# raulmur/ORB_SLAM

Hardware: AMD Instinct MI355X
Metric: frames/s ORB extract+match @640x480, 1000 kp (higher is better)
Workload: dtype u8; 1 GPU; vga: 640x480 grayscale stream, 8 levels, nFeatures 1000, S-blocks frames, extract + Hamming top-2 match vs previous frame (BASELINE.json configs[1] + the frame-to-frame match of the metric); resident_frames_per_gpu=2048, lanes=4, parity_checked_frames=0, parity_mismatches=0, library_build_id=6b2c39ae018c2573, lane_placement=2

## Files before the change

include/orbx.h:

```cpp
#ifndef ORBX_H
#define ORBX_H

#include <stddef.h>
#include <stdint.h>

#ifdef __cplusplus
extern "C" {
#endif

#define ORBX_OK             0
#define ORBX_EMPTY          1
#define ORBX_ERR_ARG       -1
#define ORBX_ERR_DEVICE    -2
#define ORBX_ERR_CAPACITY  -3
#define ORBX_ERR_GEOMETRY  -4

#define ORBX_HARRIS_SCORE 0
#define ORBX_FAST_SCORE   1

#define ORBX_BLUR_X86_SSE2 0
#define ORBX_BLUR_HALF_UP  1

#define ORBX_FP_ISO          0
#define ORBX_FP_GCC_CONTRACT 1

typedef struct orbx_keypoint {
    float x, y;
    float size;
    float angle;
    float response;
    int32_t octave;
    int32_t class_id;
} orbx_keypoint;

typedef struct orbx_params {
    int32_t nfeatures;
    float   scale_factor;
    int32_t nlevels;
    int32_t score_type;
    int32_t fast_th;
    int32_t device;
    int32_t max_batch;
    int32_t blur_rounding;
    int32_t fp_contract;
    int32_t reserved[7];
} orbx_params;

typedef struct orbx_extractor orbx_extractor;

void  orbx_default_params(orbx_params* p);
int   orbx_create(const orbx_params* p, orbx_extractor** out);
void  orbx_destroy(orbx_extractor* h);
int   orbx_get_levels(const orbx_extractor* h);
float orbx_get_scale_factor(const orbx_extractor* h);
int   orbx_max_keypoints(const orbx_extractor* h);
const char* orbx_last_error(const orbx_extractor* h);
const char* orbx_build_id(void);

int orbx_extract(orbx_extractor* h, const uint8_t* img, int w, int hgt, ptrdiff_t stride,
                 orbx_keypoint* kps, uint8_t* desc, int cap, int* n_out);

int orbx_extract_batch_device(orbx_extractor* h, const uint8_t* d_imgs, int nframes, int w, int hgt,
                              ptrdiff_t row_stride, ptrdiff_t frame_stride,
                              orbx_keypoint* d_kps, uint8_t* d_desc, int32_t* d_n, int cap,
                              int32_t* d_status, void* stream);

#define ORBX_PHASE_PYRAMID  1
#define ORBX_PHASE_DETECT   2
#define ORBX_PHASE_DESCRIBE 4
#define ORBX_PHASE_ALL      7
int orbx_extract_batch_device_phases(orbx_extractor* h, const uint8_t* d_imgs, int nframes, int w, int hgt,
                                     ptrdiff_t row_stride, ptrdiff_t frame_stride,
                                     orbx_keypoint* d_kps, uint8_t* d_desc, int32_t* d_n, int cap,
                                     int32_t* d_status, void* stream, int phases);

#define ORBX_FRAMES_ON_DEVICE 0
#define ORBX_FRAMES_ON_HOST   1
int orbx_extract_batch(orbx_extractor* h, const uint8_t* const* imgs, const ptrdiff_t* row_strides, int nframes, int w, int hgt,
                       int where, orbx_keypoint* d_kps, uint8_t* d_desc, int32_t* d_n, int cap,
                       int32_t* d_status, void* stream);

#define ORBX_PIX_GRAY8  0
#define ORBX_PIX_RGB8   1
#define ORBX_PIX_BGR8   2
#define ORBX_PIX_RGBA8  3
#define ORBX_PIX_BGRA8  4

int orbx_to_gray_device(const uint8_t* d_src, int nframes, int w, int hgt, ptrdiff_t src_row_stride, ptrdiff_t src_frame_stride, int fmt,
                        uint8_t* d_gray, ptrdiff_t gray_row_stride, ptrdiff_t gray_frame_stride, void* stream);

int orbx_extract_color(orbx_extractor* h, const uint8_t* img, int w, int hgt, ptrdiff_t stride, int fmt,
                       orbx_keypoint* kps, uint8_t* desc, int cap, int* n_out, uint8_t* gray_out);

int orbx_extract_batch_device_color(orbx_extractor* h, const uint8_t* d_imgs, int nframes, int w, int hgt,
                                    ptrdiff_t row_stride, ptrdiff_t frame_stride, int fmt,
                                    orbx_keypoint* d_kps, uint8_t* d_desc, int32_t* d_n, int cap, int32_t* d_status,
                                    uint8_t* d_gray, ptrdiff_t gray_row_stride, ptrdiff_t gray_frame_stride, void* stream);

int orbx_extract_batch_color(orbx_extractor* h, const uint8_t* const* imgs, const ptrdiff_t* row_strides, int nframes, int w, int hgt,
                             int where, int fmt, orbx_keypoint* d_kps, uint8_t* d_desc, int32_t* d_n, int cap,
                             int32_t* d_status, void* stream);

int orbm_hamming256(const uint8_t* a, const uint8_t* b);

int orbm_match_top2(const uint8_t* Q, int nq, const uint8_t* T, int nt,
                    int32_t* best_idx, int32_t* best, int32_t* second, int device);
int orbm_match_top2_device(const uint8_t* dQ, int nq, const uint8_t* dT, int nt,
                           int32_t* d_best_idx, int32_t* d_best, int32_t* d_second, void* stream);
int orbm_match_top2_masked(const uint8_t* Q, int nq, const uint8_t* T, int nt, const uint8_t* t_valid,
                           int32_t* best_idx, int32_t* best, int32_t* second, int device);
int orbm_match_top2_masked_device(const uint8_t* dQ, int nq, const uint8_t* dT, int nt, const uint8_t* d_t_valid,
                                  int32_t* d_best_idx, int32_t* d_best, int32_t* d_second, void* stream);
int orbm_match_top2_batch_device(const uint8_t* dQ, const int32_t* d_nq, const uint8_t* dT, const int32_t* d_nt,
                                 int nbatch, int cap, int32_t* d_best_idx, int32_t* d_best, int32_t* d_second,
                                 void* stream);
int orbm_match_top2_segments(const uint8_t* Q, int nq, const uint8_t* T, int nt, const int32_t* seg_off, const int32_t* cand,
                             int32_t* best_idx, int32_t* best, int32_t* second, int device);
int orbm_match_top2_segments_device(const uint8_t* dQ, int nq, const uint8_t* dT, int nt, const int32_t* d_seg_off,
                                    const int32_t* d_cand, int32_t* d_best_idx, int32_t* d_best, int32_t* d_second, void* stream);
int orbm_count_accepted(const int32_t* best, const int32_t* second, int nq, int th, float ratio);
int orbm_debug_set_match_path(int path);
int orbm_debug_get_match_path(void);

int orbx_device_alloc(int device, size_t bytes, void** d_ptr);
int orbx_device_free(int device, void* d_ptr);
int orbx_device_upload(int device, void* d_dst, const void* src, size_t bytes);
int orbx_device_download(int device, void* dst, const void* d_src, size_t bytes);

int orbx_stream_create(int device, void** stream);
int orbx_stream_create_priority(int device, int priority, void** stream);
int orbx_stream_destroy(int device, void* stream);
int orbx_stream_synchronize(int device, void* stream);
int orbx_event_create(int device, void** event);
int orbx_event_destroy(int device, void* event);
int orbx_event_record(void* event, void* stream);
int orbx_stream_wait_event(void* stream, void* event);
int orbx_device_copy_async(void* d_dst, const void* d_src, size_t bytes, void* stream);
int orbx_host_alloc(int device, size_t bytes, void** h_ptr);
int orbx_host_free(int device, void* h_ptr);
int orbx_device_upload_async(void* d_dst, const void* h_src, size_t bytes, void* stream);
int orbx_device_download_async(void* h_dst, const void* d_src, size_t bytes, void* stream);

int orbm_distinctive(const uint8_t* desc, const int32_t* seg_off, int npoints, int32_t* best_idx, int32_t* best_median, int device);
int orbm_distinctive_device(const uint8_t* d_desc, const int32_t* d_seg_off, int npoints, int32_t* d_best_idx,
                            int32_t* d_best_median, void* stream);

#define ORBX_DBG_PLANE      0
#define ORBX_DBG_BLUR       1
#define ORBX_DBG_NMS        2
#define ORBX_DBG_LEVEL_KPS  3
#define ORBX_DBG_BANDS      4
int orbx_debug_set_stop_after(orbx_extractor* h, int stage);
int orbx_debug_set_blur_on_demand(orbx_extractor* h, int mode);
int orbx_debug_stage_timing(orbx_extractor* h, int enable);
int orbx_debug_stage_time(orbx_extractor* h, int stage, double* total_ms, long* launches);
int orbx_debug_level_size(const orbx_extractor* h, int level, int* w, int* hgt);
int orbx_debug_resize_form(const orbx_extractor* h, int level, int* form, int* rows_out);
#define ORBX_VS_COLOR        0
#define ORBX_VS_INGEST       1
#define ORBX_VS_PYRAMID      2
#define ORBX_VS_FAST         3
#define ORBX_VS_QUOTA        4
#define ORBX_VS_CELL_SELECT  5
#define ORBX_VS_LEVEL_SELECT 6
#define ORBX_VS_BLUR         7
#define ORBX_VS_DESCRIBE     8
#define ORBX_VS_COUNT        9
#define ORBX_VF_LDS_OVER_64K  1u
#define ORBX_VF_FUSE_BLUR     2u
#define ORBX_VF_OVERLAP       4u
#define ORBX_VF_ON_DEMAND     8u
#define ORBX_VF_XCD_AFFINITY 16u
typedef struct orbx_stage_variant {
    int32_t id;
    uint32_t flags;
    uint64_t mask;
} orbx_stage_variant;
int orbx_debug_launch_variant(const orbx_extractor* h, int stage, orbx_stage_variant* out, char* name, int name_cap);
int orbx_debug_variant_count(int stage);
const char* orbx_debug_variant_name(int stage, int id);
typedef struct orbx_plan_args {
    int32_t w, h, nframes;
    int32_t gather, xcd_affinity, on_demand, od_min_frames, stop_after;
    int64_t row_stride, frame_stride;
    uint32_t base_bits;
    int32_t color_fmt, color_gather;
    uint32_t color_bits;
    int32_t one_frame, side_stream;
    int64_t one_frame_bytes;
} orbx_plan_args;
int orbx_debug_plan(const orbx_params* p, const orbx_plan_args* a, orbx_stage_variant* out);
long orbx_debug_fetch(orbx_extractor* h, int what, int frame, int level, void* host_out, long cap_bytes);
int orbx_debug_geometry(const orbx_params* p, int w, int hgt, int32_t* out, int cap_levels);
int orbx_debug_nth_element(const float* resp, int n, int nth, int32_t* out_perm, int device);
int orbx_debug_eval_math(int kind, const float* in0, const float* in1, float* out0, float* out1, int n, int device);
int orbx_debug_eval_compass(const uint32_t* c, const uint32_t* e, const uint32_t* w, const uint32_t* nn, const uint32_t* ss, uint32_t* out, int n, int t, int device);
int orbx_debug_eval_blur_window(const uint8_t* windows, uint8_t* out, int n, int rounding, int general, int device);

#ifdef __cplusplus
}
#endif
#endif
```

orb_slam_amd/capi.py:

```python
import ctypes
import os
import numpy as np

_HERE = os.path.dirname(os.path.abspath(__file__))
LIB_PATH = os.environ.get("ORBX_LIB") or os.path.join(_HERE, "liborbx.so")

ORBX_OK, ORBX_EMPTY = 0, 1
ORBX_ERR_ARG, ORBX_ERR_DEVICE, ORBX_ERR_CAPACITY, ORBX_ERR_GEOMETRY = -1, -2, -3, -4
HARRIS_SCORE, FAST_SCORE = 0, 1
BLUR_X86_SSE2, BLUR_HALF_UP = 0, 1
DBG_PLANE, DBG_BLUR, DBG_NMS, DBG_LEVEL_KPS, DBG_BANDS = 0, 1, 2, 3, 4
(ST_PYRAMID, ST_FAST_CELLS, ST_QUOTA, ST_CELL_SELECT, ST_LEVEL_SELECT, ST_BLUR, ST_DESCRIBE) = range(7)

KP_DTYPE = np.dtype([("x", "<f4"), ("y", "<f4"), ("size", "<f4"), ("angle", "<f4"),
                     ("response", "<f4"), ("octave", "<i4"), ("class_id", "<i4")])

EXPORTS = [
    "orbx_default_params", "orbx_create", "orbx_destroy", "orbx_get_levels", "orbx_get_scale_factor",
    "orbx_max_keypoints", "orbx_last_error", "orbx_build_id", "orbx_extract", "orbx_extract_batch_device", "orbx_extract_batch_device_phases", "orbx_extract_batch",
    "orbx_to_gray_device", "orbx_extract_color", "orbx_extract_batch_device_color", "orbx_extract_batch_color",
    "orbm_hamming256", "orbm_match_top2", "orbm_match_top2_device", "orbm_match_top2_batch_device", "orbm_match_top2_masked", "orbm_match_top2_masked_device",
    "orbm_count_accepted", "orbm_match_top2_segments", "orbm_match_top2_segments_device", "orbm_distinctive", "orbm_distinctive_device",
    "orbx_device_alloc", "orbx_device_free", "orbx_device_upload", "orbx_device_download",
    "orbx_stream_create", "orbx_stream_create_priority", "orbx_stream_destroy", "orbx_stream_synchronize", "orbx_event_create", "orbx_event_destroy", "orbx_event_record",
    "orbx_stream_wait_event", "orbx_device_copy_async", "orbx_host_alloc", "orbx_host_free", "orbx_device_upload_async", "orbx_device_download_async", "orbx_debug_set_stop_after", "orbx_debug_set_blur_on_demand", "orbx_debug_level_size", "orbx_debug_resize_form", "orbx_debug_fetch",
    "orbx_debug_launch_variant", "orbx_debug_variant_count", "orbx_debug_variant_name", "orbx_debug_plan",
    "orbx_debug_eval_math", "orbx_debug_eval_compass", "orbx_debug_eval_blur_window", "orbx_debug_stage_timing", "orbx_debug_stage_time", "orbx_debug_nth_element", "orbx_debug_geometry",
    "orbm_debug_set_match_path",
    "orbm_debug_get_match_path",
]
EXPORTS_F = [
    "orbf_image_bounds", "orbf_undistort_grid", "orbf_undistort_grid_batch_device", "orbf_features_in_area",
    "orbf_features_in_area_device",
]
EXPORTS_S = ["orbs_lds_bytes", "orbs_debug_set_buckets", "orbs_debug_set_wide_max", "orbs_three_maxima", "orbs_window_search_batch_device", "orbs_list_search_batch_device",
             "orbs_bow_ranges_batch_device", "orbs_triangulation_search_batch_device", "orbs_epipolar_bound", "orbs_agreement_batch_device",
             "orbs_bow_rows_search_batch_device", "orbs_bow_rows_search", "orbs_tri_rows_search_batch_device", "orbs_tri_rows_search"]
PHASE_PYRAMID, PHASE_DETECT, PHASE_DESCRIBE, PHASE_ALL = 1, 2, 4, 7
RULE_MAPPOINTS, RULE_WINDOW, RULE_BEST, RULE_INIT, RULE_BOW, RULE_FREE, RULE_TRIANGULATION = 0, 1, 2, 3, 4, 5, 6
TH_HIGH, TH_LOW = 100, 50
EXPORTS_V = [
    "orbv_create", "orbv_load_text", "orbv_destroy", "orbv_info", "orbv_descend", "orbv_descend_device",
    "orbv_transform", "orbv_transform_batch_device", "orbv_score",
]
EXPORTS_D = ["orbd_create", "orbd_destroy", "orbd_size", "orbd_add", "orbd_add_batch_device", "orbd_erase", "orbd_clear",
             "orbd_query_batch_device", "orbd_query"]
EXPORTS_P = ["orbp_create", "orbp_destroy", "orbp_capacity", "orbp_size", "orbp_clear", "orbp_put", "orbp_put_device", "orbp_erase", "orbp_get",
             "orbp_project_batch_device", "orbp_track_batch_device", "orbp_track", "orbp_project_source_batch_device",
             "orbp_track_source_batch_device", "orbp_track_source", "orbp_refresh_batch_device", "orbp_refresh", "orbp_fuse_batch_device",
             "orbp_fuse", "orbp_view_from_sim3", "orbp_loop_project_batch_device", "orbp_loop_search_batch_device", "orbp_loop_search",
             "orbp_sim3_from_pair", "orbp_sim3_search_batch_device", "orbp_sim3_search", "orbp_local_votes_batch_device", "orbp_local_votes",
             "orbp_local_points_batch_device", "orbp_local_points", "orbp_rows_purge_device", "orbp_cull_batch_device", "orbp_cull"]
LOCAL_MAX_PROBLEMS, LOCAL_MAX_ROWS = 64, 65535
CULL_MAX_CANDIDATES = 4096
EXPORTS_T = ["orbt_triangulate_batch_device", "orbt_triangulate", "orbt_new_points_rows_device", "orbt_new_points_rows"]
(T_NONE, T_ACCEPTED, T_PARALLAX, T_W_ZERO, T_DEPTH1, T_DEPTH2, T_REPROJ1, T_REPROJ2, T_ZERO_DIST, T_SCALE, T_SKIP_INDEX, T_SKIP_OCTAVE) = range(12)
EXPORTS_I = ["orbi_normalize", "orbi_pose_from_rt", "orbi_models_batch_device", "orbi_models", "orbi_check_rt_batch_device", "orbi_check_rt"]
INIT_MAX_PROBLEMS, INIT_MAX_MATCHES, INIT_MAX_ITERS, INIT_MAX_HYP = 32, 16384, 1024, 8
(RT_NONE, RT_GOOD, RT_COUNTED, RT_NONFINITE, RT_DEPTH1, RT_DEPTH2, RT_REPROJ1, RT_REPROJ2, RT_SKIP_INDEX) = range(9)
EXPORTS_E = ["orbe_ransac_parameters", "orbe_hypotheses_batch_device", "orbe_hypotheses", "orbe_refine_batch_device", "orbe_refine",
             "orbe_refit_batch_device", "orbe_refit", "orbe_select_batch_device", "orbe_select", "orbe_iterate", "orbe_iterate_batch"]
EXPORTS_H = ["orbh_ransac_parameters", "orbh_max_errors", "orbh_hypotheses_batch_device", "orbh_hypotheses", "orbh_select_batch_device", "orbh_select",
             "orbh_iterate", "orbh_iterate_batch"]
MODE_FRAME, MODE_LAST_FRAME, MODE_KEYFRAME, MODE_FUSE, MODE_LOOP, MODE_SIM3 = 0, 1, 2, 3, 4, 5
(FUSE_FUSED, FUSE_SKIPPED, FUSE_DEPTH, FUSE_IMAGE, FUSE_DISTANCE, FUSE_ANGLE, FUSE_EMPTY, FUSE_FAR) = range(8)
LOOP_QUERY = 8
REFRESH_NORMAL_DEPTH, REFRESH_DESCRIPTOR = 1, 2
(REFRESH_OK, REFRESH_SKIPPED, REFRESH_EMPTY, REFRESH_BAD_INDEX, REFRESH_BAD_OCTAVE, REFRESH_NONFINITE) = range(6)


class OrbxError(RuntimeError):
    def __init__(self, code, msg=""):
        super().__init__("orbx error %d %s" % (code, msg))
        self.code = code


class Params(ctypes.Structure):
    _fields_ = [("nfeatures", ctypes.c_int32), ("scale_factor", ctypes.c_float), ("nlevels", ctypes.c_int32),
                ("score_type", ctypes.c_int32), ("fast_th", ctypes.c_int32), ("device", ctypes.c_int32),
                ("max_batch", ctypes.c_int32), ("blur_rounding", ctypes.c_int32), ("fp_contract", ctypes.c_int32), ("reserved", ctypes.c_int32 * 7)]


class StageVariant(ctypes.Structure):
    _fields_ = [("id", ctypes.c_int32), ("flags", ctypes.c_uint32), ("mask", ctypes.c_uint64)]


class PlanArgs(ctypes.Structure):
    _fields_ = [("w", ctypes.c_int32), ("h", ctypes.c_int32), ("nframes", ctypes.c_int32), ("gather", ctypes.c_int32),
                ("xcd_affinity", ctypes.c_int32), ("on_demand", ctypes.c_int32), ("od_min_frames", ctypes.c_int32), ("stop_after", ctypes.c_int32),
                ("row_stride", ctypes.c_int64), ("frame_stride", ctypes.c_int64), ("base_bits", ctypes.c_uint32), ("color_fmt", ctypes.c_int32),
                ("color_gather", ctypes.c_int32), ("color_bits", ctypes.c_uint32), ("one_frame", ctypes.c_int32), ("side_stream", ctypes.c_int32),
                ("one_frame_bytes", ctypes.c_int64)]


VS_COLOR, VS_INGEST, VS_PYRAMID, VS_FAST, VS_QUOTA, VS_CELL_SELECT, VS_LEVEL_SELECT, VS_BLUR, VS_DESCRIBE, VS_COUNT = range(10)
VS_NAMES = ["color", "ingest", "pyramid", "fast", "quota", "cell_select", "level_select", "blur", "describe"]
VF_LDS_OVER_64K, VF_FUSE_BLUR, VF_OVERLAP, VF_ON_DEMAND, VF_XCD_AFFINITY = 1, 2, 4, 8, 16
XCD_AFFINITY_MIN_FRAMES = 64
OD_MIN_FRAMES_DEFAULT = 32


class Camera(ctypes.Structure):
    _fields_ = [("K", ctypes.c_float * 9), ("dist", ctypes.c_float * 8), ("ndist", ctypes.c_int32),
                ("width", ctypes.c_int32), ("height", ctypes.c_int32)]

    @classmethod
    def make(cls, fx, fy, cx, cy, dist, width, height):
        c = cls()
        for i, v in enumerate((fx, 0, cx, 0, fy, cy, 0, 0, 1)):
            c.K[i] = v
        for i, v in enumerate(dist):
            c.dist[i] = v
        c.ndist, c.width, c.height = len(dist), width, height
        return c


class Bounds(ctypes.Structure):
    _fields_ = [("min_x", ctypes.c_int32), ("max_x", ctypes.c_int32), ("min_y", ctypes.c_int32), ("max_y", ctypes.c_int32),
                ("inv_w", ctypes.c_float), ("inv_h", ctypes.c_float)]

    def astuple(self):
        return (self.min_x, self.max_x, self.min_y, self.max_y, self.inv_w, self.inv_h)


class SearchParams(ctypes.Structure):
    _fields_ = [("rule", ctypes.c_int32), ("th", ctypes.c_int32), ("ratio", ctypes.c_float), ("check_orientation", ctypes.c_int32)]


class View(ctypes.Structure):
    _fields_ = [("Rcw", ctypes.c_float * 9), ("tcw", ctypes.c_float * 3), ("Ow", ctypes.c_float * 3),
                ("fx", ctypes.c_float), ("fy", ctypes.c_float), ("cx", ctypes.c_float), ("cy", ctypes.c_float),
                ("min_x", ctypes.c_int32), ("max_x", ctypes.c_int32), ("min_y", ctypes.c_int32), ("max_y", ctypes.c_int32),
                ("view_cos_limit", ctypes.c_float), ("th", ctypes.c_float), ("mode", ctypes.c_int32), ("reserved", ctypes.c_int32)]

    @classmethod
    def make(cls, Rcw, tcw, Ow, fx, fy, cx, cy, min_x, max_x, min_y, max_y, view_cos_limit=0.5, th=1.0):
        v = cls()
        v.Rcw[:] = [float(x) for x in np.asarray(Rcw, np.float32).reshape(9)]
        v.tcw[:] = [float(x) for x in np.asarray(tcw, np.float32).reshape(3)]
        v.Ow[:] = [float(x) for x in np.asarray(Ow, np.float32).reshape(3)]
        v.fx, v.fy, v.cx, v.cy = float(fx), float(fy), float(cx), float(cy)
        v.min_x, v.max_x, v.min_y, v.max_y = int(min_x), int(max_x), int(min_y), int(max_y)
        v.view_cos_limit, v.th, v.mode, v.reserved = float(view_cos_limit), float(th), 0, 0
        return v


def view_from_sim3(Scw, view):
    S = np.ascontiguousarray(np.asarray(Scw, dtype=np.float32).reshape(-1)[:12])
    assert S.size == 12
    if isinstance(view, np.ndarray):
        assert view.dtype == VIEW_DTYPE and view.size == 1 and view.flags.c_contiguous
        ptr = view.ctypes.data
    else:
        ptr = ctypes.addressof(view)
    rc = lib().orbp_view_from_sim3(S.ctypes.data, ptr)
    if rc != ORBX_OK:
        raise OrbxError(rc, "orbp_view_from_sim3")
    return view


def sim3_from_pair(s12, R12, t12, R1w, t1w, R2w, t2w, fx, fy, cx, cy, bounds, th):
    a = lambda x, n: np.ascontiguousarray(np.asarray(x, dtype=np.float32).reshape(n))
    R12, t12, R1w, t1w, R2w, t2w = a(R12, 9), a(t12, 3), a(R1w, 9), a(t1w, 3), a(R2w, 9), a(t2w, 3)
    dirs = np.zeros(2, SIM3_DIR_DTYPE)
    rc = lib().orbp_sim3_from_pair(float(s12), R12.ctypes.data, t12.ctypes.data, R1w.ctypes.data, t1w.ctypes.data, R2w.ctypes.data, t2w.ctypes.data,
                                   float(fx), float(fy), float(cx), float(cy), ctypes.addressof(bounds), float(th), dirs.ctypes.data)
    if rc != ORBX_OK:
        raise OrbxError(rc, "orbp_sim3_from_pair")
    return dirs


class TriCamera(ctypes.Structure):
    _fields_ = [("Rcw", ctypes.c_float * 9), ("tcw", ctypes.c_float * 3), ("Ow", ctypes.c_float * 3),
                ("fx", ctypes.c_float), ("fy", ctypes.c_float), ("cx", ctypes.c_float), ("cy", ctypes.c_float)]


class TriPair(ctypes.Structure):
    _fields_ = [("kf1", TriCamera), ("kf2", TriCamera), ("scale_factor", ctypes.c_float), ("reserved", ctypes.c_int32)]


TRI_CAMERA_DTYPE = np.dtype([("Rcw", np.float32, 9), ("tcw", np.float32, 3), ("Ow", np.float32, 3), ("fx", np.float32), ("fy", np.float32),
                             ("cx", np.float32), ("cy", np.float32)])
TRI_PAIR_DTYPE = np.dtype([("kf1", TRI_CAMERA_DTYPE), ("kf2", TRI_CAMERA_DTYPE), ("scale_factor", np.float32), ("reserved", np.int32)])
assert TRI_PAIR_DTYPE.itemsize == ctypes.sizeof(TriPair) == 160

INIT_PROBLEM_DTYPE = np.dtype([("norm1", np.float32, 4), ("norm2", np.float32, 4), ("sigma", np.float32), ("n1", np.int32), ("n2", np.int32),
                               ("nmatches", np.int32), ("iters", np.int32), ("reserved", np.int32)])
INIT_POSE_DTYPE = np.dtype([("R", np.float32, 9), ("t", np.float32, 3), ("P2", np.float32, 12), ("O2", np.float32, 3)])
assert INIT_PROBLEM_DTYPE.itemsize == 56 and INIT_POSE_DTYPE.itemsize == 108
PNP_PROBLEM_DTYPE = np.dtype([("fu", np.float32), ("fv", np.float32), ("uc", np.float32), ("vc", np.float32), ("n", np.int32), ("iters", np.int32),
                              ("min_inliers", np.int32), ("max_its", np.int32)])
PNP_STATE_DTYPE = np.dtype([("iterations", np.int32), ("best_inliers", np.int32), ("refine_ok", np.int32), ("refined_inliers", np.int32),
                            ("best_tcw", np.float32, 12), ("refined_tcw", np.float32, 12)])
PNP_RESULT_DTYPE = np.dtype([("kind", np.int32), ("stop", np.int32), ("no_more", np.int32), ("ninliers", np.int32), ("tcw", np.float32, 12)])
assert PNP_PROBLEM_DTYPE.itemsize == 32 and PNP_STATE_DTYPE.itemsize == 112 and PNP_RESULT_DTYPE.itemsize == 64
PNP_KIND_NONE, PNP_KIND_BEST, PNP_KIND_REFINED = 0, 1, 2
PNP_MAX_PROBLEMS, PNP_MAX_POINTS, PNP_MAX_ITERS = 32, 8192, 1024
SIM3SOLVER_PROBLEM_DTYPE = np.dtype([("fx1", np.float32), ("fy1", np.float32), ("cx1", np.float32), ("cy1", np.float32), ("fx2", np.float32),
                                     ("fy2", np.float32), ("cx2", np.float32), ("cy2", np.float32), ("n", np.int32), ("iters", np.int32),
                                     ("min_inliers", np.int32), ("max_its", np.int32)])
SIM3SOLVER_HYP_DTYPE = np.dtype([("q", np.float64, 4), ("R", np.float32, 9), ("t", np.float32, 3), ("s", np.float32), ("T12", np.float32, 16),
                                 ("T21", np.float32, 16), ("count", np.int32)])
SIM3SOLVER_STATE_DTYPE = np.dtype([("iterations", np.int32), ("best_inliers", np.int32), ("best_T12", np.float32, 16), ("best_R", np.float32, 9),
                                   ("best_t", np.float32, 3), ("best_s", np.float32)])
SIM3SOLVER_RESULT_DTYPE = np.dtype([("found", np.int32), ("stop", np.int32), ("no_more", np.int32), ("ninliers", np.int32), ("T12", np.float32, 16)])
assert SIM3SOLVER_PROBLEM_DTYPE.itemsize == 48 and SIM3SOLVER_HYP_DTYPE.itemsize == 216 and SIM3SOLVER_STATE_DTYPE.itemsize == 124 and \
    SIM3SOLVER_RESULT_DTYPE.itemsize == 80
SIM3SOLVER_MAX_PROBLEMS, SIM3SOLVER_MAX_POINTS, SIM3SOLVER_MAX_ITERS, SIM3SOLVER_POINT_ROWS = 32, 8192, 1024, 12

VIEW_DTYPE = np.dtype([("Rcw", np.float32, 9), ("tcw", np.float32, 3), ("Ow", np.float32, 3), ("fx", np.float32), ("fy", np.float32),
                       ("cx", np.float32), ("cy", np.float32), ("min_x", np.int32), ("max_x", np.int32), ("min_y", np.int32),
                       ("max_y", np.int32), ("view_cos_limit", np.float32), ("th", np.float32), ("mode", np.int32), ("reserved", np.int32)])
RECORD_DTYPE = np.dtype([("in_view", np.uint8), ("pad", np.uint8, 3), ("u", np.float32), ("v", np.float32), ("view_cos", np.float32),
                         ("level", np.int32)])
assert VIEW_DTYPE.itemsize == ctypes.sizeof(View) == 108 and RECORD_DTYPE.itemsize == 20
REFRESHED_DTYPE = np.dtype([("normal", np.float32, 3), ("min_dist", np.float32), ("max_dist", np.float32), ("best_obs", np.int32),
                            ("best_median", np.int32), ("status", np.int32)])
assert REFRESHED_DTYPE.itemsize == 32
FUSED_DTYPE = np.dtype([("u", np.float32), ("v", np.float32), ("level", np.int32), ("status", np.int32)])
assert FUSED_DTYPE.itemsize == 16
SIM3_DIR_DTYPE = np.dtype([("Raw", np.float32, 9), ("taw", np.float32, 3), ("S", np.float32, 9), ("t", np.float32, 3), ("fx", np.float32),
                           ("fy", np.float32), ("cx", np.float32), ("cy", np.float32), ("min_x", np.int32), ("max_x", np.int32), ("min_y", np.int32),
                           ("max_y", np.int32), ("th", np.float32), ("mode", np.int32), ("reserved", np.int32, 2)])
assert SIM3_DIR_DTYPE.itemsize == 144

GRID_COLS, GRID_ROWS = 64, 48
GRID_CELLS = GRID_COLS * GRID_ROWS

_LIB = None


def lib():
    global _LIB
    if _LIB is None:
        if not os.path.exists(LIB_PATH):
            raise OrbxError(ORBX_ERR_DEVICE, "liborbx.so not built: run `make` / __graft_entry__.build()")
        try:
            import torch
        except ImportError:
            pass
        L = ctypes.CDLL(LIB_PATH)
        vp, ci, cl, cf = ctypes.c_void_p, ctypes.c_int, ctypes.c_long, ctypes.c_float
        pd = ctypes.c_ssize_t
        L.orbx_default_params.argtypes = [ctypes.POINTER(Params)]
        L.orbx_default_params.restype = None
        L.orbx_create.argtypes = [ctypes.POINTER(Params), ctypes.POINTER(vp)]
        L.orbx_destroy.argtypes = [vp]
        L.orbx_destroy.restype = None
        L.orbx_get_levels.argtypes = [vp]
        L.orbx_get_scale_factor.argtypes = [vp]
        L.orbx_get_scale_factor.restype = cf
        L.orbx_max_keypoints.argtypes = [vp]
        L.orbx_last_error.argtypes = [vp]
        L.orbx_last_error.restype = ctypes.c_char_p
        L.orbx_build_id.argtypes = []
        L.orbx_build_id.restype = ctypes.c_char_p
        L.orbx_extract.argtypes = [vp, vp, ci, ci, pd, vp, vp, ci, ctypes.POINTER(ci)]
        L.orbx_extract_batch_device.argtypes = [vp, vp, ci, ci, ci, pd, pd, vp, vp, vp, ci, vp, vp]
        L.orbx_extract_batch_device_phases.argtypes = [vp, vp, ci, ci, ci, pd, pd, vp, vp, vp, ci, vp, vp, ci]
        L.orbx_extract_batch.argtypes = [vp, vp, vp, ci, ci, ci, ci, vp, vp, vp, ci, vp, vp]
        L.orbx_to_gray_device.argtypes = [vp, ci, ci, ci, pd, pd, ci, vp, pd, pd, vp]
        L.orbx_extract_color.argtypes = [vp, vp, ci, ci, pd, ci, vp, vp, ci, ctypes.POINTER(ci), vp]
        L.orbx_extract_batch_device_color.argtypes = [vp, vp, ci, ci, ci, pd, pd, ci, vp, vp, vp, ci, vp, vp, pd, pd, vp]
        L.orbx_extract_batch_color.argtypes = [vp, vp, vp, ci, ci, ci, ci, ci, vp, vp, vp, ci, vp, vp]
        L.orbm_hamming256.argtypes = [vp, vp]
        L.orbm_match_top2.argtypes = [vp, ci, vp, ci, vp, vp, vp, ci]
        L.orbm_match_top2_device.argtypes = [vp, ci, vp, ci, vp, vp, vp, vp]
        L.orbm_match_top2_batch_device.argtypes = [vp, vp, vp, vp, ci, ci, vp, vp, vp, vp]
        L.orbm_match_top2_masked.argtypes = [vp, ci, vp, ci, vp, vp, vp, vp, ci]
        L.orbm_match_top2_masked_device.argtypes = [vp, ci, vp, ci, vp, vp, vp, vp, vp]
        L.orbm_count_accepted.argtypes = [vp, vp, ci, ci, cf]
        L.orbm_debug_set_match_path.argtypes = [ci]
        L.orbm_debug_get_match_path.argtypes = []
        L.orbs_debug_set_buckets.argtypes = [ci]
        L.orbs_debug_set_wide_max.argtypes = [ci]
        L.orbm_match_top2_segments.argtypes = [vp, ci, vp, ci, vp, vp, vp, vp, vp, ci]
        L.orbm_match_top2_segments_device.argtypes = [vp, ci, vp, ci, vp, vp, vp, vp, vp, vp]
        L.orbx_device_alloc.argtypes = [ci, ctypes.c_size_t, ctypes.POINTER(vp)]
        L.orbx_device_free.argtypes = [ci, vp]
        L.orbx_device_upload.argtypes = [ci, vp, vp, ctypes.c_size_t]
        L.orbx_device_download.argtypes = [ci, vp, vp, ctypes.c_size_t]
        L.orbm_distinctive.argtypes = [vp, vp, ci, vp, vp, ci]
        L.orbm_distinctive_device.argtypes = [vp, vp, ci, vp, vp, vp]
        L.orbx_debug_set_stop_after.argtypes = [vp, ci]
        L.orbx_debug_set_blur_on_demand.argtypes = [vp, ci]
        L.orbx_debug_level_size.argtypes = [vp, ci, ctypes.POINTER(ci), ctypes.POINTER(ci)]
        if hasattr(L, "orbx_debug_resize_form"):
            L.orbx_debug_resize_form.argtypes = [vp, ci, ctypes.POINTER(ci), ctypes.POINTER(ci)]
        if hasattr(L, "orbx_debug_launch_variant"):
            L.orbx_debug_launch_variant.argtypes = [vp, ci, ctypes.POINTER(StageVariant), ctypes.c_char_p, ci]
            L.orbx_debug_variant_count.argtypes = [ci]
            L.orbx_debug_variant_name.argtypes = [ci, ci]
            L.orbx_debug_variant_name.restype = ctypes.c_char_p
            L.orbx_debug_plan.argtypes = [ctypes.POINTER(Params), ctypes.POINTER(PlanArgs), ctypes.POINTER(StageVariant)]
        L.orbx_debug_fetch.argtypes = [vp, ci, ci, ci, vp, cl]
        L.orbx_debug_fetch.restype = cl
        L.orbx_debug_eval_math.argtypes = [ci, vp, vp, vp, vp, ci, ci]
        L.orbx_debug_eval_compass.argtypes = [vp, vp, vp, vp, vp, vp, ci, ci, ci]
        L.orbx_debug_eval_blur_window.argtypes = [vp, vp, ci, ci, ci, ci]
        L.orbx_debug_nth_element.argtypes = [vp, ci, ci, vp, ci]
        L.orbx_debug_geometry.argtypes = [ctypes.POINTER(Params), ci, ci, vp, ci]
        L.orbx_debug_stage_timing.argtypes = [vp, ci]
        L.orbx_debug_stage_time.argtypes = [vp, ci, ctypes.POINTER(ctypes.c_double), ctypes.POINTER(cl)]
        L.orbf_image_bounds.argtypes = [ctypes.POINTER(Camera), ctypes.POINTER(Bounds)]
        L.orbf_undistort_grid.argtypes = [ctypes.POINTER(Camera), ctypes.POINTER(Bounds), vp, ci, vp, vp, vp, ci]
        L.orbf_undistort_grid_batch_device.argtypes = [ctypes.POINTER(Camera), ctypes.POINTER(Bounds), vp, vp, ci, ci, vp, vp, vp, vp]
        L.orbf_features_in_area.argtypes = [ctypes.POINTER(Bounds), vp, ci, vp, vp, vp, vp, ci, vp, vp, ci, ci]
        L.orbf_features_in_area_device.argtypes = [ctypes.POINTER(Bounds), vp, ci, vp, vp, vp, vp, ci, vp, vp, ci, vp, vp]
        L.orbs_lds_bytes.argtypes = [ci, ci]
        L.orbs_lds_bytes.restype = ctypes.c_size_t
        L.orbs_three_maxima.argtypes = [vp, ci, vp]
        L.orbs_three_maxima.restype = None
        L.orbs_window_search_batch_device.argtypes = [ctypes.POINTER(Bounds), ctypes.POINTER(SearchParams), vp, vp, vp, vp, vp, ci, vp,
                                                      vp, vp, vp, vp, vp, vp, ci, ci, vp, vp, vp, vp, vp, vp]
        L.orbs_list_search_batch_device.argtypes = [ctypes.POINTER(SearchParams), vp, vp, vp, vp, vp, ci, vp, vp, vp, vp, vp, vp, vp, ci, ci,
                                                    vp, vp, vp, vp, vp, vp]
        L.orbs_bow_ranges_batch_device.argtypes = [vp, vp, vp, vp, vp, vp, ci, ci, vp, vp, vp]
        L.orbs_triangulation_search_batch_device.argtypes = [ctypes.POINTER(SearchParams), vp, vp, ci, vp, vp, vp, vp, vp, ci, vp, vp, vp,
                                                             vp, vp, vp, vp, ci, ci, vp, vp, vp, vp, vp, vp]
        L.orbs_epipolar_bound.argtypes = [ctypes.c_float]
        L.orbs_epipolar_bound.restype = ctypes.c_float
        L.orbs_agreement_batch_device.argtypes = [vp, vp, ci, vp, vp, ci, ci, vp, vp, vp]
        L.orbs_bow_rows_search_batch_device.argtypes = [ctypes.POINTER(SearchParams), vp, ci, vp, vp, vp, vp, vp, vp, vp, ci, ci, vp, vp, vp, vp, vp, vp, vp, vp]
        L.orbs_bow_rows_search.argtypes = [ctypes.POINTER(SearchParams), vp, ci, vp, vp, vp, vp, vp, vp, vp, ci, ci, ci, vp, vp, vp, vp, vp, vp, vp, vp]
        L.orbs_tri_rows_search_batch_device.argtypes = [ctypes.POINTER(SearchParams), vp, ci, vp, vp, ci, vp, vp, vp, vp, vp, vp, vp, ci, ci, vp, ci, vp, vp, vp, vp, vp,
                                                        vp, vp]
        L.orbs_tri_rows_search.argtypes = [ctypes.POINTER(SearchParams), vp, ci, vp, vp, ci, vp, vp, vp, vp, vp, vp, vp, ci, ci, ci, vp, ci, vp, vp, vp, vp, vp, vp, vp]
        L.orbv_create.argtypes = [ci, ci, ci, ci, ci, vp, vp, vp, vp, ci, ctypes.POINTER(vp)]
        L.orbv_load_text.argtypes = [ctypes.c_char_p, ci, ctypes.POINTER(vp)]
        L.orbv_destroy.argtypes = [vp]
        L.orbv_destroy.restype = None
        L.orbv_info.argtypes = [vp] + [ctypes.POINTER(ci)] * 6
        L.orbv_descend.argtypes = [vp, vp, ci, ci, vp, vp, vp]
        L.orbv_descend_device.argtypes = [vp, vp, ci, ci, vp, vp, vp, vp]
        L.orbv_transform.argtypes = [vp, vp, ci, ci, vp, vp, ctypes.POINTER(ci), vp, vp, vp, ctypes.POINTER(ci)]
        L.orbv_transform_batch_device.argtypes = [vp, vp, vp, ci, ci, ci, vp, vp, vp, vp, vp, vp, vp, vp]
        L.orbv_score.argtypes = [vp, vp, vp, ci, vp, vp, ci]
        L.orbv_score.restype = ctypes.c_double
        L.orbd_create.argtypes = [vp, ci, ci, ctypes.POINTER(vp)]
        L.orbd_destroy.argtypes = [vp]
        L.orbd_destroy.restype = None
        L.orbd_size.argtypes = [vp]
        L.orbd_add.argtypes = [vp, ci, vp, vp, ci]
        L.orbd_add_batch_device.argtypes = [vp, vp, ci, vp, vp, vp, ci, vp, vp]
        L.orbd_erase.argtypes = [vp, ci]
        L.orbd_clear.argtypes = [vp]
        L.orbd_query_batch_device.argtypes = [vp, ci, vp, vp, vp, ci, vp, vp, vp, vp, vp, vp, ci, vp, vp, vp, vp]
        L.orbd_query.argtypes = [vp, vp, vp, ci, vp, ci, vp, vp, vp, vp, ci, ctypes.POINTER(ci), ctypes.POINTER(ci), vp]
        L.orbp_create.argtypes = [ci, ci, ctypes.POINTER(vp)]
        L.orbp_destroy.argtypes = [vp]
        L.orbp_destroy.restype = None
        L.orbp_capacity.argtypes = [vp]
        L.orbp_size.argtypes = [vp]
        L.orbp_clear.argtypes = [vp]
        L.orbp_put.argtypes = [vp, vp, ci, vp, vp, vp, vp, vp]
        L.orbp_put_device.argtypes = [vp, vp, ci, vp, vp, vp, vp, vp, vp]
        L.orbp_erase.argtypes = [vp, vp, ci]
        L.orbp_get.argtypes = [vp, ci, ctypes.POINTER(ci), vp, vp, vp, vp, vp]
        L.orbp_project_batch_device.argtypes = [vp, vp, ci, vp, ci, vp, vp, ci, vp, vp, vp, vp, vp, vp, vp, vp, ci, vp]
        L.orbp_track_batch_device.argtypes = [vp, vp, ci, vp, ci, vp, vp, ci, vp, ctypes.POINTER(Bounds), cf, vp, vp, vp, vp, vp, ci, vp, ci,
                                              vp, vp, vp, vp, vp, vp]
        L.orbp_track.argtypes = [vp, ctypes.POINTER(View), vp, ci, vp, ci, vp, ctypes.POINTER(Bounds), cf, vp, vp, vp, vp, vp, ci, ci, ci,
                                 vp, vp, ctypes.POINTER(ci), ctypes.POINTER(ci), vp]
        L.orbp_refresh_batch_device.argtypes = [vp, vp, ci, vp, vp, vp, vp, vp, vp, vp, vp, vp, ci, ci, vp, ci, ci, vp, vp]
        L.orbp_refresh.argtypes = [vp, vp, ci, vp, vp, vp, vp, vp, vp, vp, vp, vp, ci, ci, ci, vp, ci, ci, vp, vp]
        L.orbp_fuse_batch_device.argtypes = [vp, vp, ci, vp, ci, vp, vp, ci, vp, vp, ci, vp, vp, vp, vp, vp, ci, ci, vp, vp, vp, vp, vp]
        L.orbp_fuse.argtypes = [vp, vp, ci, vp, ci, vp, vp, ci, vp, vp, ci, vp, vp, vp, vp, vp, ci, ci, ci, vp, vp, vp, vp, vp]
        L.orbp_view_from_sim3.argtypes = [vp, vp]
        cf = ctypes.c_float
        L.orbp_sim3_from_pair.argtypes = [cf, vp, vp, vp, vp, vp, vp, cf, cf, cf, cf, vp, cf, vp]
        L.orbp_sim3_search_batch_device.argtypes = [vp, vp, ci, vp, ci, vp, vp, ci, vp, vp, vp, vp, vp, vp, vp, ci, ci, vp, ci, vp, vp, vp, vp, vp, vp]
        L.orbp_sim3_search.argtypes = [vp, vp, ci, vp, ci, vp, vp, ci, vp, vp, vp, vp, vp, vp, vp, ci, ci, ci, vp, ci, vp, vp, vp, vp, vp, vp]
        L.orbp_loop_project_batch_device.argtypes = [vp, vp, ci, vp, ci, vp, vp, ci, vp, vp, vp, vp, vp, vp, vp, vp, ci, vp]
        L.orbp_loop_search_batch_device.argtypes = [vp, vp, ci, vp, ci, vp, vp, ci, vp, vp, ci, vp, vp, vp, vp, vp, ci, ci, vp, vp, ci, vp, vp, vp, vp, vp, vp, vp]
        L.orbp_loop_search.argtypes = [vp, vp, vp, ci, vp, ci, vp, vp, ci, vp, vp, vp, vp, vp, ci, ci, ci, vp, vp, vp, ctypes.POINTER(ci), ctypes.POINTER(ci), vp]
        L.orbp_local_votes_batch_device.argtypes = [vp, vp, vp, ci, ci, vp, vp, ci, ci, vp, vp]
        L.orbp_local_votes.argtypes = [vp, vp, vp, ci, ci, vp, vp, ci, ci, ci, vp, vp]
        L.orbp_local_points_batch_device.argtypes = [vp, vp, vp, ci, ci, vp, vp, ci, vp, vp, ci, ci, vp, vp, vp, vp, ci, vp]
        L.orbp_local_points.argtypes = [vp, vp, vp, ci, ci, vp, vp, ci, vp, vp, ci, ci, ci, vp, vp, vp, vp, ci, vp]
        L.orbp_rows_purge_device.argtypes = [vp, vp, ci, vp, ci, ci, vp]
        L.orbp_cull_batch_device.argtypes = [vp, vp, ci, vp, vp, vp, ci, ci, ci, vp, vp, vp, vp]
        L.orbp_cull.argtypes = [vp, vp, ci, vp, vp, vp, ci, ci, ci, ci, vp, vp, vp, vp]
        L.orbp_project_source_batch_device.argtypes = [vp, vp, ci, vp, ci, vp, vp, ci, vp, vp, vp, vp, vp, vp, vp, vp, vp, vp, ci, vp]
        L.orbp_track_source_batch_device.argtypes = [vp, vp, ci, vp, ci, vp, vp, ci, vp, vp, vp, ctypes.POINTER(Bounds), ctypes.POINTER(SearchParams),
                                                     vp, vp, vp, vp, vp, ci, vp, ci, vp, vp, vp, vp, vp, vp]
        L.orbp_track_source.argtypes = [vp, ctypes.POINTER(View), vp, ci, vp, ci, vp, vp, vp, ci, ctypes.POINTER(Bounds), ctypes.POINTER(SearchParams),
                                        vp, vp, vp, vp, vp, ci, ci, ci, vp, vp, ctypes.POINTER(ci), ctypes.POINTER(ci), vp]
        L.orbt_triangulate_batch_device.argtypes = [vp, ci, vp, vp, vp, vp, ci, vp, vp, ci, ci, vp, vp, ci, vp, vp, vp, ci, vp, vp, vp, vp, vp, vp, vp, vp,
                                                    ci, vp, vp, vp]
        L.orbt_triangulate.argtypes = [vp, vp, vp, vp, vp, ci, vp, ci, vp, ci, vp, vp, vp, vp, vp, vp, ci, ctypes.POINTER(ci), ci]
        L.orbt_new_points_rows_device.argtypes = [ctypes.POINTER(SearchParams), vp, ci, vp, vp, vp, vp, vp, vp, ci, vp, vp, vp, vp, vp, vp, vp, ci, ci, vp, vp, vp, vp,
                                                  vp, vp, vp, vp, vp, vp, vp, vp, vp, ci, vp]
        L.orbt_new_points_rows.argtypes = [ctypes.POINTER(SearchParams), vp, ci, vp, vp, vp, vp, vp, vp, ci, vp, vp, vp, vp, vp, vp, vp, ci, ci, ci, vp, vp, vp, vp,
                                           vp, vp, vp, vp, vp, vp, vp, vp, vp, ci, vp]
        pnp_bind(L)
        sim3solver_bind(L)
        L.orbi_normalize.argtypes = [vp, ci, vp]
        L.orbi_pose_from_rt.argtypes = [cf, cf, cf, cf, vp, vp, vp]
        L.orbi_models_batch_device.argtypes = [vp, ci, vp, ci, vp, ci, vp, ci, vp, ci, vp, vp, vp, vp, vp, vp, vp, vp, vp, vp, vp, vp]
        L.orbi_models.argtypes = [vp, vp, vp, vp, vp, vp, vp, vp, vp, vp, vp, vp, vp, vp, vp, vp, ci]
        L.orbi_check_rt_batch_device.argtypes = [cf, cf, cf, cf, vp, ci, ci, vp, vp, vp, vp, ci, vp, ci, vp, ci, vp, cf, vp, vp, vp, vp, vp, vp, vp]
        L.orbi_check_rt.argtypes = [cf, cf, cf, cf, vp, ci, vp, ci, vp, ci, vp, ci, vp, cf, vp, vp, vp, vp, vp, vp, vp, ci]
        _LIB = L
    return _LIB


FRAMES_ON_DEVICE, FRAMES_ON_HOST = 0, 1


def frame_table(frames):
    frames = list(frames)
    if not frames:
        raise ValueError("no frames")
    on_dev = [bool(getattr(f, "is_cuda", False)) for f in frames]
    if any(on_dev) and not all(on_dev):
        raise ValueError("frames mix device and host memory")
    ptrs, strides, keep, shape = [], [], [], None
    for f in frames:
        if hasattr(f, "data_ptr"):
            import torch
            if f.dtype != torch.uint8 or f.dim() != 2:
                raise ValueError("frames must be 2-D uint8")
            if f.stride(1) != 1 or f.stride(0) < f.shape[1]:
                if f.is_cuda:
                    raise ValueError("device frame rows must be contiguous (stride(1) == 1)")
                f = f.contiguous()
            hw, p, rs = tuple(f.shape), f.data_ptr(), f.stride(0)
        else:
            a = np.asarray(f)
            if a.dtype != np.uint8 or a.ndim != 2:
                raise ValueError("frames must be 2-D uint8")
            if a.strides[1] != 1 or a.strides[0] < a.shape[1]:
                a = np.ascontiguousarray(a)
            hw, p, rs = a.shape, a.ctypes.data, a.strides[0]
            f = a
        if shape is None:
            shape = hw
        elif hw != shape:
            raise ValueError("frames differ in size: %s vs %s" % (hw, shape))
        keep.append(f)
        ptrs.append(p)
# ... 59 lines not shown
        raise OrbxError(rc, "orbx_to_gray_device")


def to_gray(frames, fmt, stream=0):
    import torch
    one = frames.dim() == 3
    x = frames.unsqueeze(0) if one else frames
    ch = pix_channels(fmt)
    if not x.is_cuda or x.dtype != torch.uint8 or x.dim() != 4 or x.shape[3] != ch or x.stride(3) != 1 or x.stride(2) != ch:
        raise ValueError("to_gray wants a CUDA uint8 (F, H, W, %d) tensor with packed pixels" % ch)
    F, h, w = x.shape[:3]
    out = torch.empty((F, h, w), dtype=torch.uint8, device=x.device)
    to_gray_device(x.data_ptr(), F, w, h, x.stride(1), x.stride(0), fmt, out.data_ptr(), w, w * h, stream)
    return out[0] if one else out


class ORBextractor:

    def __init__(self, nfeatures=1000, scaleFactor=1.2, nlevels=8, scoreType=FAST_SCORE, fastTh=20,
                 device=0, max_batch=1, blur_rounding=BLUR_X86_SSE2, fp_contract=None):
        L = lib()
        p = Params()
        L.orbx_default_params(ctypes.byref(p))
        p.nfeatures, p.scale_factor, p.nlevels, p.score_type, p.fast_th = nfeatures, scaleFactor, nlevels, scoreType, fastTh
        p.device, p.max_batch, p.blur_rounding = device, max_batch, blur_rounding
        if fp_contract is not None:
            p.fp_contract = 1 if fp_contract else 0
        h = ctypes.c_void_p()
        rc = L.orbx_create(ctypes.byref(p), ctypes.byref(h))
        if rc != ORBX_OK:
            raise OrbxError(rc, "orbx_create (is a gfx950 GPU visible?)")
        self.h = h
        self.L = L
        self.max_keypoints = L.orbx_max_keypoints(h)

    def close(self):
        if getattr(self, "h", None):
            self.L.orbx_destroy(self.h)
            self.h = None

    def __del__(self):
        self.close()

    def GetLevels(self):
        return self.L.orbx_get_levels(self.h)

    def GetScaleFactor(self):
        return self.L.orbx_get_scale_factor(self.h)

    def _err(self, rc):
        return OrbxError(rc, self.L.orbx_last_error(self.h).decode())

    def __call__(self, image):
        img = np.asarray(image)
        if img.size == 0:
            return None
        assert img.dtype == np.uint8 and img.ndim == 2
        if img.strides[1] != 1:
            img = np.ascontiguousarray(img)
        hh, w = img.shape
        cap = self.max_keypoints
        kps = np.zeros(cap, dtype=KP_DTYPE)
        desc = np.zeros((cap, 32), dtype=np.uint8)
        n = ctypes.c_int(0)
        rc = self.L.orbx_extract(self.h, img.ctypes.data, w, hh, img.strides[0], kps.ctypes.data, desc.ctypes.data, cap, ctypes.byref(n))
        if rc != ORBX_OK:
            raise self._err(rc)
        return kps[:n.value].copy(), desc[:n.value].copy()

    def extract_batch_device(self, d_imgs, nframes, w, h, row_stride, frame_stride, d_kps, d_desc, d_n, cap, d_status=0, stream=0, phases=PHASE_ALL):
        rc = self.L.orbx_extract_batch_device_phases(self.h, d_imgs, nframes, w, h, row_stride, frame_stride, d_kps, d_desc, d_n, cap,
                                                     d_status or None, stream or None, phases)
        if rc != ORBX_OK:
            raise self._err(rc)

    def extract_batch(self, frames, d_kps, d_desc, d_n, cap, d_status=0, stream=0):
        where, ptrs, strides, w, h, keep = frame_table(frames)
        rc = self.L.orbx_extract_batch(self.h, ptrs.ctypes.data, strides.ctypes.data, len(ptrs), w, h, where, d_kps, d_desc, d_n, cap,
                                       d_status or None, stream or None)
        del keep
        if rc != ORBX_OK:
            raise self._err(rc)

    def extract_color(self, image, fmt, want_gray=False):
        ptr, w, hh, rs, on_dev, keep = color_layout(image, fmt)
        if on_dev:
            raise ValueError("extract_color takes a host frame")
        if w == 0 or hh == 0:
            return None
        cap = self.max_keypoints
        kps = np.zeros(cap, dtype=KP_DTYPE)
        desc = np.zeros((cap, 32), dtype=np.uint8)
        gray = np.empty((hh, w), dtype=np.uint8) if want_gray else None
        n = ctypes.c_int(0)
        rc = self.L.orbx_extract_color(self.h, ptr, w, hh, rs, fmt, kps.ctypes.data, desc.ctypes.data, cap, ctypes.byref(n),
                                       gray.ctypes.data if want_gray else None)
        del keep
        if rc != ORBX_OK:
            raise self._err(rc)
        res = (kps[:n.value].copy(), desc[:n.value].copy())
        return res + (gray,) if want_gray else res

    def extract_batch_device_color(self, d_imgs, nframes, w, h, row_stride, frame_stride, fmt, d_kps, d_desc, d_n, cap, d_status=0, d_gray=0,
                                   gray_row_stride=0, gray_frame_stride=0, stream=0):
        pix_channels(fmt)
        rc = self.L.orbx_extract_batch_device_color(self.h, d_imgs, nframes, w, h, row_stride, frame_stride, fmt, d_kps, d_desc, d_n, cap,
                                                    d_status or None, d_gray or None, gray_row_stride, gray_frame_stride, stream or None)
        if rc != ORBX_OK:
            raise self._err(rc)

    def extract_batch_color(self, frames, fmt, d_kps, d_desc, d_n, cap, d_status=0, stream=0):
        where, ptrs, strides, w, h, keep = color_frame_table(frames, fmt)
        rc = self.L.orbx_extract_batch_color(self.h, ptrs.ctypes.data, strides.ctypes.data, len(ptrs), w, h, where, fmt, d_kps, d_desc, d_n,
                                             cap, d_status or None, stream or None)
        del keep
        if rc != ORBX_OK:
            raise self._err(rc)

    def set_stop_after(self, stage):
        self.L.orbx_debug_set_stop_after(self.h, stage)

    def set_blur_on_demand(self, mode):
        rc = self.L.orbx_debug_set_blur_on_demand(self.h, int(mode))
        if rc != ORBX_OK:
            raise OrbxError(rc, "orbx_debug_set_blur_on_demand")

    STAGE_NAMES = ["pyramid", "fast_cells", "quota", "cell_select", "level_select", "blur", "describe"]

    def stage_timing(self, enable):
        self.L.orbx_debug_stage_timing(self.h, enable)

    def stage_times(self):
        res = {}
        for i, name in enumerate(self.STAGE_NAMES):
            ms, n = ctypes.c_double(), ctypes.c_long()
            self.L.orbx_debug_stage_time(self.h, i, ctypes.byref(ms), ctypes.byref(n))
            res[name] = (ms.value, n.value)
        return res

    def level_size(self, level):
        w, hh = ctypes.c_int(), ctypes.c_int()
        rc = self.L.orbx_debug_level_size(self.h, level, ctypes.byref(w), ctypes.byref(hh))
        if rc != ORBX_OK:
            raise self._err(rc)
        return w.value, hh.value

    def resize_form(self, level):
        form, rows = ctypes.c_int(), ctypes.c_int()
        rc = self.L.orbx_debug_resize_form(self.h, level, ctypes.byref(form), ctypes.byref(rows))
        if rc != ORBX_OK:
            raise OrbxError(rc, "orbx_debug_resize_form")
        return form.value, rows.value

    def launch_variant(self, stage):
        v, name = StageVariant(), ctypes.create_string_buffer(96)
        rc = self.L.orbx_debug_launch_variant(self.h, stage, ctypes.byref(v), name, len(name))
        if rc != ORBX_OK:
            raise OrbxError(rc, "orbx_debug_launch_variant")
        return v.id, v.flags, v.mask, name.value.decode()

    def fetch_plane(self, what, level, frame=0):
        w, hh = self.level_size(level)
        out = np.empty((hh, w), dtype=np.uint8)
        rc = self.L.orbx_debug_fetch(self.h, what, frame, level, out.ctypes.data, out.nbytes)
        if rc < 0:
            raise self._err(rc)
        return out

    def fetch_bands(self, level, frame=0):
        out = np.zeros((16384, 8), dtype=np.int32)
        rc = self.L.orbx_debug_fetch(self.h, DBG_BANDS, frame, level, out.ctypes.data, out.nbytes)
        if rc < 0:
            raise self._err(rc)
        return out[:rc // 32].copy()

    def fetch_level_keypoints(self, level, frame=0):
        out = np.zeros((4 * self.max_keypoints + 64, 3), dtype=np.int32)
        rc = self.L.orbx_debug_fetch(self.h, DBG_LEVEL_KPS, frame, level, out.ctypes.data, out.nbytes)
        if rc < 0:
            raise self._err(rc)
        n = rc // 12
        xy = out[:n, :2].copy()
        resp = out[:n, 2].copy().view(np.float32)
        return xy, resp


def hamming256(a, b):
    a = np.ascontiguousarray(a, dtype=np.uint8)
    b = np.ascontiguousarray(b, dtype=np.uint8)
    assert a.size == 32 and b.size == 32
    return lib().orbm_hamming256(a.ctypes.data, b.ctypes.data)


def match_top2(Q, T, device=0):
    Q = np.ascontiguousarray(Q, dtype=np.uint8).reshape(-1, 32)
    T = np.ascontiguousarray(T, dtype=np.uint8).reshape(-1, 32)
    nq, nt = len(Q), len(T)
    idx = np.empty(nq, np.int32)
    best = np.empty(nq, np.int32)
    sec = np.empty(nq, np.int32)
    rc = lib().orbm_match_top2(Q.ctypes.data, nq, T.ctypes.data, nt, idx.ctypes.data, best.ctypes.data, sec.ctypes.data, device)
    if rc != ORBX_OK:
        raise OrbxError(rc, "orbm_match_top2")
    return idx, best, sec


def match_top2_masked(Q, T, t_valid, device=0):
    Q = np.ascontiguousarray(Q, dtype=np.uint8).reshape(-1, 32)
    T = np.ascontiguousarray(T, dtype=np.uint8).reshape(-1, 32)
    v = np.ascontiguousarray(t_valid, dtype=np.uint8)
    nq, nt = len(Q), len(T)
    assert len(v) == nt
    idx = np.empty(nq, np.int32); best = np.empty(nq, np.int32); sec = np.empty(nq, np.int32)
    rc = lib().orbm_match_top2_masked(Q.ctypes.data, nq, T.ctypes.data, nt, v.ctypes.data if nt else None, idx.ctypes.data, best.ctypes.data, sec.ctypes.data, device)
    if rc != ORBX_OK:
        raise OrbxError(rc, "orbm_match_top2_masked")
    return idx, best, sec


def match_top2_segments(Q, T, seg_off, cand, device=0):
    Q = np.ascontiguousarray(Q, dtype=np.uint8).reshape(-1, 32)
    T = np.ascontiguousarray(T, dtype=np.uint8).reshape(-1, 32)
    seg = np.ascontiguousarray(seg_off, dtype=np.int32)
    cd = np.ascontiguousarray(cand, dtype=np.int32)
    nq = len(Q)
    assert len(seg) == nq + 1
    idx = np.empty(nq, np.int32); best = np.empty(nq, np.int32); sec = np.empty(nq, np.int32)
    rc = lib().orbm_match_top2_segments(Q.ctypes.data, nq, T.ctypes.data, len(T), seg.ctypes.data, cd.ctypes.data if len(cd) else None,
                                        idx.ctypes.data, best.ctypes.data, sec.ctypes.data, device)
    if rc != ORBX_OK:
        raise OrbxError(rc, "orbm_match_top2_segments")
    return idx, best, sec


def build_id():
    return lib().orbx_build_id().decode()


def match_top2_device(dQ, nq, dT, nt, d_idx, d_best, d_second, stream=0):
    rc = lib().orbm_match_top2_device(dQ, nq, dT, nt, d_idx, d_best, d_second, stream or None)
    if rc != ORBX_OK:
        raise OrbxError(rc, "orbm_match_top2_device")


def match_top2_batch_device(dQ, d_nq, dT, d_nt, nbatch, cap, d_idx, d_best, d_second, stream=0):
    rc = lib().orbm_match_top2_batch_device(dQ, d_nq, dT, d_nt, nbatch, cap, d_idx, d_best, d_second, stream or None)
    if rc != ORBX_OK:
        raise OrbxError(rc, "orbm_match_top2_batch_device")


def get_match_path():
    return int(lib().orbm_debug_get_match_path())


def set_match_path(path):
    rc = lib().orbm_debug_set_match_path(path)
    if rc != ORBX_OK:
        raise OrbxError(rc, "orbm_debug_set_match_path")


def set_search_buckets(mode):
    rc = lib().orbs_debug_set_buckets(mode)
    if rc != ORBX_OK:
        raise OrbxError(rc, "orbs_debug_set_buckets")


def set_search_wide_max(nproblems):
    rc = lib().orbs_debug_set_wide_max(nproblems)
    if rc != ORBX_OK:
        raise OrbxError(rc, "orbs_debug_set_wide_max")


def count_accepted(best, second, th=50, ratio=0.6):
    best = np.ascontiguousarray(best, dtype=np.int32)
    second = np.ascontiguousarray(second, dtype=np.int32)
    return lib().orbm_count_accepted(best.ctypes.data, second.ctypes.data, len(best), th, ratio)


def geometry(w, h, nfeatures=1000, scaleFactor=1.2, nlevels=8, scoreType=FAST_SCORE, fastTh=20):
    L = lib()
    p = Params()
    L.orbx_default_params(ctypes.byref(p))
    p.nfeatures, p.scale_factor, p.nlevels, p.score_type, p.fast_th = nfeatures, scaleFactor, nlevels, scoreType, fastTh
    out = np.zeros((16, 8), np.int32)
    rc = L.orbx_debug_geometry(ctypes.byref(p), w, h, out.ctypes.data, 16)
    if rc < 0:
        raise OrbxError(rc, "orbx_debug_geometry")
    keys = ("w", "h", "quota", "grid_cols", "grid_rows", "cell_w", "cell_h", "n_bands")
    return [dict(zip(keys, map(int, out[l]))) for l in range(rc)]


def variant_count(stage):
    return lib().orbx_debug_variant_count(stage)


def variant_name(stage, vid):
    return lib().orbx_debug_variant_name(stage, vid).decode()


def plan(w, h, nframes, row_stride=None, frame_stride=None, base_bits=0, gather=False, xcd_affinity=None, on_demand=1, od_min_frames=OD_MIN_FRAMES_DEFAULT,
         stop_after=-1, color_fmt=-1, color_gather=False, color_bits=0, one_frame=False, one_frame_bytes=0, side_stream=True,
         nfeatures=1000, scaleFactor=1.2, nlevels=8, scoreType=FAST_SCORE, fastTh=20, fp_contract=False):
    L = lib()
    p = Params()
    L.orbx_default_params(ctypes.byref(p))
    p.nfeatures, p.scale_factor, p.nlevels, p.score_type, p.fast_th, p.fp_contract = nfeatures, scaleFactor, nlevels, scoreType, fastTh, 1 if fp_contract else 0
# ... 1422 lines not shown
```

orb_slam_amd/csrc/k_pyramid.hip:

```cpp
#include <algorithm>
#include <type_traits>

#include "k_resize_strip.h"
#include "orbx_device.h"
#include "orbx_launch.h"

namespace orbx {


template <bool ALIGNED, bool WINDOW, bool GATHER>
__device__ __forceinline__ void k_resize_body(Batch b, int level) {
    extern __shared__ __attribute__((aligned(16))) uint8_t s_src[];
    const DevGeom& g = b.g;
    const LevelGeom& L = g.lv[level];
    const int RZ_SRC_W = L.rz_pitch;
    const LevelGeom& P = g.lv[level - 1];
    const int tiles_x = (L.w + 255) / 256, tiles_y = (L.h + RZ_ROWS - 1) / RZ_ROWS;
    int frame, tile;
    if (!frame_item(b, blockIdx.x, tiles_x * tiles_y, frame, tile)) return;
    const int tile_y = tile / tiles_x, tile_x = tile - tile_y * tiles_x;
    const int tid = threadIdx.x, lane = tid & 63, wave = wave_id();
    const int bx0 = tile_x * 256, by0 = tile_y * RZ_ROWS;
    const int bx1 = min(bx0 + 255, L.w - 1), by1 = min(by0 + RZ_ROWS - 1, L.h - 1);
    long long sstride;
    const uint8_t* src = plain_plane<GATHER>(b, P, level - 1, frame, sstride);
    const ResizeX* tx = b.tabx + L.tabx_off;
    const ResizeY* ty = b.taby + L.taby_off;
    const int dx0 = bx0 + lane * 4;
    ResizeX rx[4];
#pragma unroll
    for (int k = 0; k < 4; k++) rx[k] = tx[min(dx0 + k, L.w - 1)];
    constexpr int RPW = RZ_ROWS / 4;
    const uint2 ryl = *reinterpret_cast<const uint2*>(ty + min(by0 + wave * RPW + min(lane, RPW - 1), L.h - 1));
    const int r0 = ty[by0].sy0, r1 = ty[by1].sy1;
    const int c0 = tx[bx0].sx & ~3, c1 = tx[bx1].sx1;
    const int nd = ((c1 - c0) >> 2) + 1, nr = r1 - r0 + 1;
    if (ALIGNED) {
        typedef const void __attribute__((address_space(1))) * gptr_t;
        typedef void __attribute__((address_space(3))) * lptr_t;
        const uint8_t* base = src + (long long)r0 * sstride + c0;
        for (int p0 = 0; p0 < nd; p0 += 64) {
            const bool on = p0 + lane < nd;
            for (int r = wave; r < nr; r += 4) {
                const uint8_t* grow = base + (long long)r * sstride + 4 * p0;
                if (on) __builtin_amdgcn_global_load_lds((gptr_t)(grow + 4 * lane), (lptr_t)(s_src + r * RZ_SRC_W + 4 * p0), 4, 0, 0);
            }
        }
        asm volatile("s_waitcnt vmcnt(0)" ::: "memory");
    } else {
        const int total = nr * nd;
        const float inv_nd = 1.0f / (float)nd;
        const uint8_t* base = src + (long long)r0 * sstride + c0;
        const int xm = P.w - 1 - c0;
        for (int i0 = 0; i0 < total; i0 += 256 * 8) {
            uint32_t v4[8];
            int off[8];
#pragma unroll
            for (int k = 0; k < 8; k++) {
                const int i = i0 + k * 256 + tid;
                v4[k] = 0;
                off[k] = -1;
                if (i < total) {
                    int r, d;
                    split_px(i, nd, inv_nd, r, d);
                    const uint8_t* row = base + (long long)r * sstride;
                    off[k] = r * RZ_SRC_W + 4 * d;
                    if (ALIGNED) v4[k] = *reinterpret_cast<const uint32_t*>(row + 4 * d);
                    else v4[k] = (uint32_t)row[min(4 * d, xm)] | (uint32_t)row[min(4 * d + 1, xm)] << 8 | (uint32_t)row[min(4 * d + 2, xm)] << 16 |
                                 (uint32_t)row[min(4 * d + 3, xm)] << 24;
                }
            }
#pragma unroll
            for (int k = 0; k < 8; k++)
                if (off[k] >= 0) *reinterpret_cast<uint32_t*>(s_src + off[k]) = v4[k];
        }
    }
    __syncthreads();
    if (dx0 >= L.w) return;
    uint8_t* dplane = b.pyr + (long long)frame * g.frame_plane_bytes + L.plane_off;
    if (WINDOW) {
        const int w0 = rx[0].sx - c0;
        const int wa = w0 & ~3, sh = w0 & 3;
        uint32_t sel[4], apair[4];
#pragma unroll
        for (int k = 0; k < 4; k++) {
            sel[k] = (uint32_t)(rx[k].sx - c0 - w0) | 0x0C000C00u | ((uint32_t)(rx[k].sx1 - c0 - w0) << 16);
            apair[k] = (uint32_t)(uint16_t)rx[k].a0 | ((uint32_t)(uint16_t)rx[k].a1 << 16);
        }
        auto hrow = [&](int sy, uint32_t (&d)[4]) {
            const uint32_t* p = reinterpret_cast<const uint32_t*>(s_src + (sy - r0) * RZ_SRC_W + wa);
            const uint32_t d0 = p[0], d1 = p[1], d2 = p[2];
            const uint32_t lo = __builtin_amdgcn_alignbyte(d1, d0, (uint32_t)sh), hi = __builtin_amdgcn_alignbyte(d2, d1, (uint32_t)sh);
#pragma unroll
            for (int k = 0; k < 4; k++) d[k] = __builtin_amdgcn_udot2(as_us2v(__builtin_amdgcn_perm(hi, lo, sel[k])), as_us2v(apair[k]), 0u, false) >> 4;
        };
        int have = -1;
        uint32_t dprev[4] = {0, 0, 0, 0};
#pragma unroll
        for (int j = 0; j < RPW; j++) {
            const int dy = by0 + wave * RPW + j;
            if (dy >= L.h) break;
            const uint32_t ry_rows = (uint32_t)__builtin_amdgcn_readlane((int)ryl.x, j), ry_w = (uint32_t)__builtin_amdgcn_readlane((int)ryl.y, j);
            const int sy0 = (int16_t)(ry_rows & 0xffffu), sy1 = (int16_t)(ry_rows >> 16);
            const uint32_t b0s = ry_w << 16, b1s = ry_w & 0xffff0000u;
            uint32_t da[4], db[4];
            if (sy0 == have) {
#pragma unroll
                for (int k = 0; k < 4; k++) da[k] = dprev[k];
            } else hrow(sy0, da);
            if (sy1 == sy0) {
#pragma unroll
                for (int k = 0; k < 4; k++) db[k] = da[k];
            } else hrow(sy1, db);
            have = sy1;
            uint32_t packed = 0;
#pragma unroll
            for (int k = 0; k < 4; k++) {
                dprev[k] = db[k];
                const uint32_t px = (__umulhi(da[k], b0s) + __umulhi(db[k], b1s) + 2u) >> 2;
                packed |= px << (8 * k);
            }
            *reinterpret_cast<uint32_t*>(dplane + (long long)dy * L.stride + dx0) = packed;
        }
        return;
    }
#pragma unroll
    for (int j = 0; j < RZ_ROWS / 4; j++) {
        const int dy = by0 + wave + 4 * j;
        if (dy >= L.h) break;
        const ResizeY ry = ty[dy];
        const uint8_t* q0 = s_src + (ry.sy0 - r0) * RZ_SRC_W - c0;
        const uint8_t* q1 = s_src + (ry.sy1 - r0) * RZ_SRC_W - c0;
        uint32_t packed = 0;
#pragma unroll
        for (int k = 0; k < 4; k++) {
            const int px = resize_px(q0[rx[k].sx], q0[rx[k].sx1], q1[rx[k].sx], q1[rx[k].sx1], rx[k].a0, rx[k].a1, ry.b0, ry.b1);
            packed |= (uint32_t)(px & 255) << (8 * k);
        }
        *reinterpret_cast<uint32_t*>(dplane + (long long)dy * L.stride + dx0) = packed;
    }
}
template <bool ALIGNED, bool WINDOW>
__global__ __launch_bounds__(256) void k_resize(Batch b, int level) { k_resize_body<ALIGNED, WINDOW, false>(b, level); }
template <bool ALIGNED, bool WINDOW>
__global__ __launch_bounds__(256) void k_resize_gather(Batch b, int level) { k_resize_body<ALIGNED, WINDOW, true>(b, level); }

struct RzsCols {
    uint32_t sel[4], apair[4];
    int wa, sh;
};
__device__ __forceinline__ void rzs_load_cols(const ResizeX* tx, int w, int dcol, RzsCols& c) {
    ResizeX rx[4];
#pragma unroll
    for (int k = 0; k < 4; k++) rx[k] = tx[min(4 * dcol + k, w - 1)];
    const int w0 = rx[0].sx;
    c.wa = w0 & ~3;
    c.sh = w0 & 3;
#pragma unroll
    for (int k = 0; k < 4; k++) {
        c.sel[k] = (uint32_t)(rx[k].sx - w0) | 0x0C000C00u | ((uint32_t)(rx[k].sx1 - w0) << 16);
        c.apair[k] = (uint32_t)(uint16_t)rx[k].a0 | ((uint32_t)(uint16_t)rx[k].a1 << 16);
    }
}
__device__ __forceinline__ void rzs_hrow(const uint8_t* s_src, int off, const RzsCols& c, uint32_t (&d)[4]) {
    const uint32_t* p = reinterpret_cast<const uint32_t*>(s_src + off);
    const uint32_t d0 = p[0], d1 = p[1], d2 = p[2];
    const uint32_t lo = __builtin_amdgcn_alignbyte(d1, d0, (uint32_t)c.sh), hi = __builtin_amdgcn_alignbyte(d2, d1, (uint32_t)c.sh);
#pragma unroll
    for (int k = 0; k < 4; k++) d[k] = __builtin_amdgcn_udot2(as_us2v(__builtin_amdgcn_perm(hi, lo, c.sel[k])), as_us2v(c.apair[k]), 0u, false) >> 4;
}
__device__ __forceinline__ uint32_t rzs_vpack(const uint32_t (&da)[4], const uint32_t (&db)[4], uint32_t b0s, uint32_t b1s) {
    uint32_t packed = 0;
#pragma unroll
    for (int k = 0; k < 4; k++) packed |= ((__umulhi(da[k], b0s) + __umulhi(db[k], b1s) + 2u) >> 2) << (8 * k);
    return packed;
}

template <bool GATHER, int NG>
__device__ __forceinline__ void k_resize_strip_body(Batch b, int level, int rows_out, int nstrips, unsigned magic) {
    extern __shared__ __attribute__((aligned(16))) uint8_t s_src[];
    const DevGeom& g = b.g;
    const LevelGeom& L = g.lv[level];
    const LevelGeom& P = g.lv[level - 1];
    int frame, strip;
    if (!frame_item_magic(b, blockIdx.x, (unsigned)nstrips, magic, frame, strip)) return;
    const int tid = threadIdx.x, lane = tid & 63, wave = wave_id();
    long long sstride64;
    const uint8_t* src = plain_plane<GATHER>(b, P, level - 1, frame, sstride64);
    const int sstride = (int)sstride64;
    const ResizeX* tx = b.tabx + L.tabx_off;
    const ResizeY* ty = b.taby + L.taby_off;
    const int RPW = rows_out >> 2;
    const int row0 = strip * rows_out + wave * RPW;
    const uint2 ryl = *reinterpret_cast<const uint2*>(ty + min(row0 + min(lane, RPW - 1), L.h - 1));
    const int ngroups = NG ? NG : rzs_groups(L.w);
    const int rem = rzs_rem_cols(L.w);
    const bool rowpar = rem <= RZS_ROWPAR_MAX;
    const int shift = rzs_rowpar_shift(rem);
    auto group_col = [&](int gi) { return gi == ngroups - 1 && rowpar ? 64 * gi + rzs_rowpar_slot(lane, shift) : rzs_loop_col(gi, lane); };
    RzsCols cols[NG ? NG : 1];
    if (NG) {
#pragma unroll
        for (int gi = 0; gi < NG; gi++) rzs_load_cols(tx, L.w, group_col(gi), cols[gi]);
    }
    __builtin_amdgcn_sched_barrier(0);
    const StripSpan sp = rzs_span(ty, L.h, rows_out, strip, sstride64, rzs_readable(level == 1, sstride64, P.w));
    const int r0 = sp.r0, nchunks = (int)sp.chunks;
    {
        typedef const void __attribute__((address_space(1))) * gptr_t;
        typedef void __attribute__((address_space(3))) * lptr_t;
        const uint8_t* base = src + (long long)r0 * sstride64;
        if (tid < sp.tail_dwords)
            *reinterpret_cast<uint32_t*>(s_src + 16 * nchunks + 4 * tid) = *reinterpret_cast<const uint32_t*>(base + 16 * (long long)nchunks + 4 * tid);
        for (int q0 = 64 * wave; q0 < nchunks; q0 += 256)
            if (q0 + lane < nchunks) __builtin_amdgcn_global_load_lds((gptr_t)(base + 16 * (q0 + lane)), (lptr_t)(s_src + 16 * q0), 16, 0, 0);
        asm volatile("s_waitcnt vmcnt(0)" ::: "memory");
    }
    __syncthreads();
    uint8_t* dplane = b.pyr + (long long)frame * g.frame_plane_bytes + L.plane_off;
    const unsigned dstride = (unsigned)L.stride;
    const int nrows = min(RPW, L.h - row0);
    auto process = [&](int gi, const RzsCols& c) {
        const int dcol = group_col(gi);
        if (gi == ngroups - 1 && rowpar) {
            const int slot = rzs_rowpar_slot(lane, shift);
            for (int pass = 0; pass * (64 >> shift) < RPW; pass++) {
                const int j = rzs_rowpar_row(lane, shift, pass);
                const uint32_t ry_rows = (uint32_t)__shfl((int)ryl.x, min(j, RPW - 1)), ry_w = (uint32_t)__shfl((int)ryl.y, min(j, RPW - 1));
                const int dy = row0 + j;
                if (slot < rem && j < RPW && dy < L.h) {
                    const int sy0 = (int16_t)(ry_rows & 0xffffu), sy1 = (int16_t)(ry_rows >> 16);
                    uint32_t da[4], db[4];
                    rzs_hrow(s_src, (sy0 - r0) * sstride + c.wa, c, da);
                    rzs_hrow(s_src, (sy1 - r0) * sstride + c.wa, c, db);
                    *reinterpret_cast<uint32_t*>(dplane + ((unsigned)dy * dstride + 4u * (unsigned)dcol)) = rzs_vpack(da, db, ry_w << 16, ry_w & 0xffff0000u);
                }
            }
        } else if (4 * dcol < L.w) {
            int have = -1;
            uint32_t cur[4] = {0, 0, 0, 0};
            for (int j = 0; j < nrows; j++) {
                const int dy = row0 + j;
                const uint32_t ry_rows = (uint32_t)__builtin_amdgcn_readlane((int)ryl.x, j), ry_w = (uint32_t)__builtin_amdgcn_readlane((int)ryl.y, j);
                const int sy0 = (int16_t)(ry_rows & 0xffffu), sy1 = (int16_t)(ry_rows >> 16);
                const uint32_t b0s = ry_w << 16, b1s = ry_w & 0xffff0000u;
                if (sy0 != have) rzs_hrow(s_src, (sy0 - r0) * sstride + c.wa, c, cur);
                uint32_t t[4];
#pragma unroll
                for (int k = 0; k < 4; k++) t[k] = __umulhi(cur[k], b0s);
                asm volatile("" : "+v"(t[0]), "+v"(t[1]), "+v"(t[2]), "+v"(t[3]));
                if (sy1 != sy0) rzs_hrow(s_src, (sy1 - r0) * sstride + c.wa, c, cur);
                have = sy1;
                uint32_t packed = 0;
#pragma unroll
                for (int k = 0; k < 4; k++) packed |= ((t[k] + __umulhi(cur[k], b1s) + 2u) >> 2) << (8 * k);
                *reinterpret_cast<uint32_t*>(dplane + ((unsigned)dy * dstride + 4u * (unsigned)dcol)) = packed;
            }
        }
    };
    if constexpr (NG != 0) {
#pragma unroll
        for (int gi = 0; gi < NG; gi++) process(gi, cols[gi]);
    } else {
        for (int gi = 0; gi < ngroups; gi++) {
            rzs_load_cols(tx, L.w, group_col(gi), cols[0]);
            process(gi, cols[0]);
        }
    }
}
typedef void (*resize_strip_fn)(Batch, int, int, int, unsigned);
template <int NG>
__global__ __launch_bounds__(256) void k_resize(Batch b, int level, int rows_out, int nstrips, unsigned magic) { k_resize_strip_body<false, NG>(b, level, rows_out, nstrips, magic); }
template <int NG>
__global__ __launch_bounds__(256) void k_resize_gather(Batch b, int level, int rows_out, int nstrips, unsigned magic) { k_resize_strip_body<true, NG>(b, level, rows_out, nstrips, magic); }

template <bool ALIGNED, bool GATHER>
__global__ __launch_bounds__(256) void k_pyramid(Batch b, int group) {
    extern __shared__ __attribute__((aligned(16))) uint8_t s_lv[];
    const DevGeom& g = b.g;
    const PyrGroup& pg = g.pyr[group];
    const int frame = blockIdx.z, ix = blockIdx.x, iy = blockIdx.y;
    const int tid = threadIdx.x;
    const int l0 = pg.l0, depth = pg.depth;
    if (group == 0 && ix == 0 && iy == 0 && tid == 0) b.status[frame] = ORBX_OK;
    const int* xt = b.pyr_tab + pg.xtab;
    const int* yt = b.pyr_tab + pg.ytab;
    auto xr = [&](int k, int i, int e) { return xt[(k * (pg.ntx + 1) + i) * 2 + e]; };
    auto yr = [&](int k, int i, int e) { return yt[(k * (pg.nty + 1) + i) * 2 + e]; };
    {
        const LevelGeom& P = g.lv[l0];
        const int xs = xr(0, ix, 0), xe = xr(0, ix, 1), ys = yr(0, iy, 0), ye = yr(0, iy, 1);
        const int nd = ((xe - xs) >> 2) + 1, nr = ye - ys + 1;
        long long sstride;
        const uint8_t* src = plain_plane<GATHER>(b, P, l0, frame, sstride);
        const uint8_t* base = src + (long long)ys * sstride + xs;
        const int xm = P.w - 1 - xs;
        const int total = nr * nd;
        const float inv_nd = 1.0f / (float)nd;
        const int pitch = pg.pitch[0];
        for (int i0 = 0; i0 < total; i0 += 256 * 8) {
            uint32_t v4[8];
            int off[8];
#pragma unroll
            for (int k = 0; k < 8; k++) {
                const int i = i0 + k * 256 + tid;
                v4[k] = 0;
                off[k] = -1;
                if (i < total) {
                    int r, d;
                    split_px(i, nd, inv_nd, r, d);
                    const uint8_t* row = base + (long long)r * sstride;
                    off[k] = r * pitch + 4 * d;
                    if (ALIGNED) v4[k] = *reinterpret_cast<const uint32_t*>(row + 4 * d);
                    else v4[k] = (uint32_t)row[min(4 * d, xm)] | (uint32_t)row[min(4 * d + 1, xm)] << 8 | (uint32_t)row[min(4 * d + 2, xm)] << 16 |
                                 (uint32_t)row[min(4 * d + 3, xm)] << 24;
                }
            }
#pragma unroll
            for (int k = 0; k < 8; k++)
                if (off[k] >= 0) *reinterpret_cast<uint32_t*>(s_lv + pg.lds_off[0] + off[k]) = v4[k];
        }
    }
    __syncthreads();
    for (int k = 1; k <= depth; k++) {
        const int level = l0 + k;
        const LevelGeom& L = g.lv[level];
        const ResizeX* tx = b.tabx + L.tabx_off;
        const ResizeY* ty = b.taby + L.taby_off;
        const int xs = xr(k, ix, 0), xe = xr(k, ix, 1), ys = yr(k, iy, 0), ye = yr(k, iy, 1);
        const int own_x1 = xr(k, ix + 1, 0), own_y1 = yr(k, iy + 1, 0);
        const int sxs = xr(k - 1, ix, 0), sys = yr(k - 1, iy, 0);
        const uint8_t* sbuf = s_lv + pg.lds_off[k - 1];
        const int spitch = pg.pitch[k - 1];
        uint8_t* dbuf = k < depth ? s_lv + pg.lds_off[k] : nullptr;
        const int dpitch = k < depth ? pg.pitch[k] : 0;
        uint8_t* dplane = b.pyr + (long long)frame * g.frame_plane_bytes + L.plane_off;
        const int ngroups = ((xe - xs) >> 2) + 1;
        const int lc = ngroups > 16 ? 5 : ngroups > 8 ? 4 : 3;
        const int gx = tid & ((1 << lc) - 1), gy = tid >> lc, ystep = 256 >> lc;
        for (int G0 = 0; G0 < ngroups; G0 += 1 << lc) {
            const int G = G0 + gx;
            if (G >= ngroups) continue;
            const int X = xs + 4 * G;
            ResizeX rx[4];
#pragma unroll
            for (int j = 0; j < 4; j++) rx[j] = tx[min(X + j, L.w - 1)];
            for (int y = ys + gy; y <= ye; y += ystep) {
                const ResizeY ry = ty[y];
                const uint8_t* q0 = sbuf + (ry.sy0 - sys) * spitch - sxs;
                const uint8_t* q1 = sbuf + (ry.sy1 - sys) * spitch - sxs;
                uint32_t packed = 0;
#pragma unroll
                for (int j = 0; j < 4; j++) {
                    const int px = resize_px(q0[rx[j].sx], q0[rx[j].sx1], q1[rx[j].sx], q1[rx[j].sx1], rx[j].a0, rx[j].a1, ry.b0, ry.b1);
                    packed |= (uint32_t)(px & 255) << (8 * j);
                }
                if (dbuf) *reinterpret_cast<uint32_t*>(dbuf + (y - ys) * dpitch + 4 * G) = packed;
                if (X < own_x1 && y < own_y1) *reinterpret_cast<uint32_t*>(dplane + (long long)y * L.stride + X) = packed;
            }
        }
        __syncthreads();
    }
}


int resize_form(const Batch& b, const HostGeom& hg, int level, StripChoice& sc) {
    const DevGeom& g = hg.g;
    sc = StripChoice{0, 0};
    if (level < 1 || level >= g.nlevels) return RZ_FORM_TILED;
    if (g.npyr_groups > 0 && b.nframes < PYR_FUSED_MAX_FRAMES) return RZ_FORM_FUSED;
    const LevelGeom& L = g.lv[level];
    if (level >= 2 || (level0_max_stride(b) == g.lv[0].w && (level0_bits(b) & 3) == 0)) sc = StripChoice{L.rs_rows, L.rs_lds};
    else sc = resize_strip_choice(hg, level, level0_max_stride(b), level0_bits(b));
    return sc.rows_out ? RZ_FORM_STRIP : RZ_FORM_TILED;
}

template <int NG>
static void launch_resize_strip(const Batch& b, int l, const StripChoice& sc, bool gather, hipStream_t stream) {
    const LevelGeom& L = b.g.lv[l];
    const int nstrips = rzs_strips(L.h, sc.rows_out);
    const unsigned magic = frame_item_magic_of(nstrips);
    dim3 grid(frame_item_blocks(b, nstrips));
    const resize_strip_fn fn = gather ? static_cast<resize_strip_fn>(&k_resize_gather<NG>) : static_cast<resize_strip_fn>(&k_resize<NG>);
    hipLaunchKernelGGL(fn, grid, dim3(256), (size_t)sc.lds_bytes, stream, b, l, sc.rows_out, nstrips, magic);
}

PyramidPlan plan_pyramid(const Batch& b, const HostGeom& hg) {
    const DevGeom& g = hg.g;
    const bool al0 = (level0_bits(b) & 3) == 0;
    PyramidPlan p;
    StripChoice sc;
    if (g.nlevels > 1 && resize_form(b, hg, 1, sc) == RZ_FORM_FUSED) {
        for (int gi = 0; gi < g.npyr_groups; gi++) {
            const bool first = g.pyr[gi].l0 == 0;
            p.launch[p.n++] = PyramidLaunch{PV_PYRAMID0 + ((!first || al0) ? 1 : 0) + ((b.img_tab && first) ? 2 : 0), gi, StripChoice{0, 0}};
        }
        return p;
    }
    for (int l = 1; l < g.nlevels; l++) {
        const LevelGeom& L = g.lv[l];
        const bool gather = b.img_tab && l == 1;
        if (resize_form(b, hg, l, sc) == RZ_FORM_STRIP) {
            const int ng = rzs_groups(L.w);
            p.launch[p.n++] = PyramidLaunch{(gather ? PV_STRIP_GATHER0 : PV_STRIP0) + (ng <= 4 ? ng : 0), l, sc};
        } else
            p.launch[p.n++] = PyramidLaunch{PV_TILED0 + ((l > 1 || al0) ? 1 : 0) + (L.rz_window ? 2 : 0) + (gather ? 4 : 0), l, StripChoice{0, 0}};
    }
    return p;
}
const char* pyramid_variant_name(int id) {
    static const char* const names[PV_COUNT] = {
        "k_pyramid<false, false>", "k_pyramid<true, false>", "k_pyramid<false, true>", "k_pyramid<true, true>",
        "k_resize<false, false>", "k_resize<true, false>", "k_resize<false, true>", "k_resize<true, true>",
        "k_resize_gather<false, false>", "k_resize_gather<true, false>", "k_resize_gather<false, true>", "k_resize_gather<true, true>",
        "k_resize<0>", "k_resize<1>", "k_resize<2>", "k_resize<3>", "k_resize<4>",
        "k_resize_gather<0>", "k_resize_gather<1>", "k_resize_gather<2>", "k_resize_gather<3>", "k_resize_gather<4>"};
    return id >= 0 && id < PV_COUNT ? names[id] : "?";
}

int launch_pyramid(const Batch& b, const PyramidPlan& plan, hipStream_t stream) {
    const DevGeom& g = b.g;
    for (int i = 0; i < plan.n; i++) {
        const PyramidLaunch& pl = plan.launch[i];
        if (pl.variant < PV_TILED0) {
            const PyrGroup& pg = g.pyr[pl.index];
            const dim3 grid(pg.ntx, pg.nty, b.nframes);
            const size_t lds = (size_t)pg.lds_bytes;
            switch (pl.variant - PV_PYRAMID0) {
                case 0: hipLaunchKernelGGL((k_pyramid<false, false>), grid, dim3(256), lds, stream, b, pl.index); break;
                case 1: hipLaunchKernelGGL((k_pyramid<true, false>), grid, dim3(256), lds, stream, b, pl.index); break;
                case 2: hipLaunchKernelGGL((k_pyramid<false, true>), grid, dim3(256), lds, stream, b, pl.index); break;
                default: hipLaunchKernelGGL((k_pyramid<true, true>), grid, dim3(256), lds, stream, b, pl.index); break;
            }
        } else if (pl.variant < PV_STRIP0) {
            const int l = pl.index;
            const LevelGeom& L = g.lv[l];
            const dim3 grid(frame_item_blocks(b, ((L.w + 255) / 256) * ((L.h + RZ_ROWS - 1) / RZ_ROWS)));
            const size_t lds = (size_t)L.rz_pitch * L.rz_rows;
            switch (pl.variant - PV_TILED0) {
                case 0: hipLaunchKernelGGL((k_resize<false, false>), grid, dim3(256), lds, stream, b, l); break;
                case 1: hipLaunchKernelGGL((k_resize<true, false>), grid, dim3(256), lds, stream, b, l); break;
                case 2: hipLaunchKernelGGL((k_resize<false, true>), grid, dim3(256), lds, stream, b, l); break;
                case 3: hipLaunchKernelGGL((k_resize<true, true>), grid, dim3(256), lds, stream, b, l); break;
                case 4: hipLaunchKernelGGL((k_resize_gather<false, false>), grid, dim3(256), lds, stream, b, l); break;
                case 5: hipLaunchKernelGGL((k_resize_gather<true, false>), grid, dim3(256), lds, stream, b, l); break;
                case 6: hipLaunchKernelGGL((k_resize_gather<false, true>), grid, dim3(256), lds, stream, b, l); break;
                default: hipLaunchKernelGGL((k_resize_gather<true, true>), grid, dim3(256), lds, stream, b, l); break;
            }
        } else {
            const bool gather = pl.variant >= PV_STRIP_GATHER0;
            switch (pl.variant - (gather ? PV_STRIP_GATHER0 : PV_STRIP0)) {
                case 1: launch_resize_strip<1>(b, pl.index, pl.sc, gather, stream); break;
                case 2: launch_resize_strip<2>(b, pl.index, pl.sc, gather, stream); break;
                case 3: launch_resize_strip<3>(b, pl.index, pl.sc, gather, stream); break;
                case 4: launch_resize_strip<4>(b, pl.index, pl.sc, gather, stream); break;
                default: launch_resize_strip<0>(b, pl.index, pl.sc, gather, stream); break;
            }
        }
        ORBX_LAUNCH_CHECK();
    }
    return ORBX_OK;
}

}
```

orb_slam_amd/csrc/k_resize_strip.h:

```cpp
#pragma once
#include <stdint.h>

#include "orb_math.h"

namespace orbx {

constexpr int RZS_WG_PER_CU = 8;
constexpr int RZS_LDS_BUDGET = 160 * 1024 / RZS_WG_PER_CU;
constexpr int RZS_ROWS_MIN = 12, RZS_ROWS_CAP = 48;
constexpr int RZS_SLACK = 16;
constexpr int RZS_ROWPAR_MAX = 32;

enum { RZ_FORM_TILED = 0, RZ_FORM_STRIP = 1, RZ_FORM_FUSED = 2 };

ORBX_HD long long rzs_readable(bool src_is_level0, long long stride, int src_w) {
    if (!src_is_level0) return stride;
    const long long w16 = (long long)((src_w + 15) & ~15);
    return stride < w16 ? stride : w16;
}

struct StripSpan {
    int by0, by1;
    int r0, r1;
    long long bytes;
    long long chunks;
    int tail_dwords;
    long long lds_bytes;
};

template <class RY>
ORBX_HD StripSpan rzs_span(const RY* ty, int h, int rows_out, int strip, long long stride, long long readable) {
    StripSpan s;
    s.by0 = strip * rows_out;
    s.by1 = imin(s.by0 + rows_out - 1, h - 1);
    s.r0 = ty[s.by0].sy0;
    s.r1 = ty[s.by1].sy1;
    s.bytes = (long long)(s.r1 - s.r0) * stride + readable;
    s.chunks = s.bytes >> 4;
    s.tail_dwords = (int)(s.bytes & 15) >> 2;
    s.lds_bytes = ((s.bytes + 15) & ~15ll) + RZS_SLACK;
    return s;
}

ORBX_HD int rzs_strips(int h, int rows_out) { return (h + rows_out - 1) / rows_out; }

template <class RY>
inline long long rzs_lds_bytes(const RY* ty, int h, int rows_out, long long stride, long long readable) {
    long long m = 0;
    for (int s = 0; s < rzs_strips(h, rows_out); s++) {
        const long long v = rzs_span(ty, h, rows_out, s, stride, readable).lds_bytes;
        m = v > m ? v : m;
    }
    return m;
}

template <class RY>
inline int rzs_pick_rows(const RY* ty, int h, long long stride, long long readable, int budget = RZS_LDS_BUDGET, int cap = RZS_ROWS_CAP) {
    for (int r = cap & ~3; r >= RZS_ROWS_MIN; r -= 4)
        if (rzs_lds_bytes(ty, h, r, stride, readable) <= (long long)budget) return r;
    return 0;
}

ORBX_HD int rzs_dword_cols(int w) { return (w + 3) >> 2; }
ORBX_HD int rzs_groups(int w) { return (rzs_dword_cols(w) + 63) >> 6; }
ORBX_HD int rzs_rem_cols(int w) { return rzs_dword_cols(w) - 64 * (rzs_groups(w) - 1); }
ORBX_HD bool rzs_rowpar(int w) { return rzs_rem_cols(w) <= RZS_ROWPAR_MAX; }
ORBX_HD int rzs_rowpar_shift(int rem) {
    int s = 0;
    while ((1 << s) < rem) s++;
    return s;
}
ORBX_HD int rzs_loop_col(int g, int lane) { return 64 * g + lane; }
ORBX_HD int rzs_rowpar_slot(int lane, int shift) { return lane & ((1 << shift) - 1); }
ORBX_HD int rzs_rowpar_row(int lane, int shift, int pass) { return pass * (64 >> shift) + (lane >> shift); }
ORBX_HD long long rzs_window_off(int sy, int r0, long long stride, int sx0) { return (long long)(sy - r0) * stride + (sx0 & ~3); }

}
```

orb_slam_amd/csrc/orb_math.h:

```cpp
#pragma once
#include <math.h>
#include <stdint.h>

#if defined(__HIPCC__)
#define ORBX_HD __host__ __device__ inline
#else
#define ORBX_HD inline
#endif

namespace orbx {

ORBX_HD int cv_round_f(float v) { return (int)rintf(v); }

ORBX_HD int imin(int a, int b) { return a < b ? a : b; }
ORBX_HD int imax(int a, int b) { return a > b ? a : b; }
ORBX_HD int imin3(int a, int b, int c) { return imin(imin(a, b), c); }
ORBX_HD int imax3(int a, int b, int c) { return imax(imax(a, b), c); }

ORBX_HD int reflect101(int p, int len) {
    if ((unsigned)p < (unsigned)len) return p;
    if (len == 1) return 0;
    do {
        p = p < 0 ? -p : 2 * len - 2 - p;
    } while ((unsigned)p >= (unsigned)len);
    return p;
}

ORBX_HD float fast_atan2_deg(float y, float x) {
    const float k = (float)(180 / 3.14159265358979323846);
    const float p1 = 0.9997878412794807f * k, p3 = -0.3258083974640975f * k;
    const float p5 = 0.1555786518463281f * k, p7 = -0.04432655554792128f * k;
    const float eps = 2.2204460492503131e-16f;
    float ax = fabsf(x), ay = fabsf(y);
    float a, c, c2;
    if (ax >= ay) {
        c = ay / (ax + eps);
        c2 = c * c;
        a = (((p7 * c2 + p5) * c2 + p3) * c2 + p1) * c;
    } else {
        c = ax / (ay + eps);
        c2 = c * c;
        a = 90.f - (((p7 * c2 + p5) * c2 + p3) * c2 + p1) * c;
    }
    if (x < 0) a = 180.f - a;
    if (y < 0) a = 360.f - a;
    return a;
}

ORBX_HD void sincosf_orb(float y, float* sinp, float* cosp) {
    const double hpi_inv = 0x1.45F306DC9C883p+23;
    const double hpi = 0x1.921FB54442D18p0;
    const double c0 = 0x1p0, c1 = -0x1.ffffffd0c621cp-2, c2 = 0x1.55553e1068f19p-5;
    const double c3 = -0x1.6c087e89a359dp-10, c4 = 0x1.99343027bf8c3p-16;
    const double s1 = -0x1.555545995a603p-3, s2 = 0x1.1107605230bc4p-7, s3 = -0x1.994eb3774cf24p-13;
    double x = (double)y;
    int n = 0;
    const float ay = fabsf(y);
    if (!(ay < 0x1.921fb6p-1f)) {
        double r = x * hpi_inv;
        n = ((int32_t)r + 0x800000) >> 24;
        x = x - (double)n * hpi;
    }
    const double x2 = x * x;
    double ps, pc;
    {
        double x3 = x * x2;
        double t1 = s2 + x2 * s3;
        double x7 = x3 * x2;
        double s = x + x3 * s1;
        ps = s + x7 * t1;
    }
    {
        double x4 = x2 * x2;
        double t2 = c3 + x2 * c4;
        double t1 = c0 + x2 * c1;
        double x6 = x4 * x2;
        double c = t1 + x4 * c2;
        pc = c + x6 * t2;
    }
    double sv = (n & 1) ? pc : ps;
    double cv = (n & 1) ? ps : pc;
    if (n & 2) sv = -sv;
    if ((n + 1) & 2) cv = -cv;
    if (n == 0 && ay < 0x1p-12f) sv = (double)y;
    *sinp = (float)sv;
    *cosp = (float)cv;
}

ORBX_HD int fast9_score(const int d[16], int tmin) {
    int lo3[16], hi3[16];
#pragma unroll
    for (int k = 0; k < 16; k++) {
        lo3[k] = imin3(d[k], d[(k + 1) & 15], d[(k + 2) & 15]);
        hi3[k] = imax3(d[k], d[(k + 1) & 15], d[(k + 2) & 15]);
    }
    int dark = -1000, bright = 1000;
#pragma unroll
    for (int k = 0; k < 16; k++) {
        int lo9 = imin3(lo3[k], lo3[(k + 3) & 15], lo3[(k + 6) & 15]);
        int hi9 = imax3(hi3[k], hi3[(k + 3) & 15], hi3[(k + 6) & 15]);
        dark = imax(dark, lo9);
        bright = imin(bright, hi9);
    }
    int s = imax(dark, -bright) - 1;
    return s >= tmin ? s : 0;
}

ORBX_HD int avg_u8(int a, int b, int c) { return (a + b + (c & 1)) >> 1; }
ORBX_HD int compass_t(int t) { return t < 0 ? 0 : t > 254 ? 254 : t; }
ORBX_HD int compass_r(int t) { return compass_t(t) & 1; }
ORBX_HD int compass_kb(int t) { return 128 - (compass_t(t) + compass_r(t)) / 2; }
ORBX_HD int compass_kd(int t) { return 255 - (254 + compass_r(t) - compass_t(t)) / 2; }
ORBX_HD uint32_t avg4_u8(uint32_t a, uint32_t b, uint32_t c) {
    uint32_t o = 0;
    for (int j = 0; j < 4; j++) o |= (uint32_t)avg_u8((int)((a >> (8 * j)) & 255u), (int)((b >> (8 * j)) & 255u), (int)((c >> (8 * j)) & 1u)) << (8 * j);
    return o;
}
ORBX_HD uint32_t compass4_flags(uint32_t C, uint32_t E, uint32_t W, uint32_t N, uint32_t S, int t) {
    const uint32_t R = (uint32_t)compass_r(t) * 0x01010101u, KB = (uint32_t)compass_kb(t) * 0x01010101u, KD = (uint32_t)compass_kd(t) * 0x01010101u;
    const uint32_t nc = ~C;
    const uint32_t hN = avg4_u8(N, nc, R), hS = avg4_u8(S, nc, R), hE = avg4_u8(E, nc, R), hW = avg4_u8(W, nc, R);
    const uint32_t br = (avg4_u8(hN, KB, 0) | avg4_u8(hS, KB, 0)) & (avg4_u8(hE, KB, 0) | avg4_u8(hW, KB, 0));
    const uint32_t dk = (avg4_u8(hN, KD, 0) & avg4_u8(hS, KD, 0)) | (avg4_u8(hE, KD, 0) & avg4_u8(hW, KD, 0));
    return (br | ~dk) & 0x80808080u;
}

ORBX_HD int resize_px(int s00, int s01, int s10, int s11, int a0, int a1, int b0, int b1) {
    int d0 = s00 * a0 + s01 * a1;
    int d1 = s10 * a0 + s11 * a1;
    return (((b0 * (d0 >> 4)) >> 16) + ((b1 * (d1 >> 4)) >> 16) + 2) >> 2;
}

#define ORBX_G0 18
#define ORBX_G1 34
#define ORBX_G2 49
#define ORBX_G3 55
ORBX_HD int blur_taps7(int a, int b, int c, int d, int e, int f, int g) {
    return ORBX_G0 * (a + g) + ORBX_G1 * (b + f) + ORBX_G2 * (c + e) + ORBX_G3 * d;
}
ORBX_HD int blur_round(int sum, int ties_even) {
    int q = (sum + 0x7FFF + (ties_even ? ((sum >> 16) & 1) : 1)) >> 16;
    return q > 255 ? 255 : q;
}

ORBX_HD constexpr int blur_tap(int t) { return t == 0 || t == 6 ? ORBX_G0 : t == 1 || t == 5 ? ORBX_G1 : t == 2 || t == 4 ? ORBX_G2 : t == 3 ? ORBX_G3 : 0; }
ORBX_HD constexpr int blur_tap_sum() { return blur_tap(0) + blur_tap(1) + blur_tap(2) + blur_tap(3) + blur_tap(4) + blur_tap(5) + blur_tap(6); }
ORBX_HD constexpr int blurf_lo_bias() { return 1024; }
ORBX_HD constexpr int blurf_hi(int mid) { return mid >> 8; }
ORBX_HD constexpr int blurf_lo(int mid) { return blurf_lo_bias() + (mid & 255); }
ORBX_HD constexpr float blurf_tap_hi(int t) { return (float)blur_tap(t) / 256.f; }
ORBX_HD constexpr float blurf_tap_lo(int t) { return (float)blur_tap(t) / 65536.f; }
ORBX_HD constexpr float blurf_start() { return -(float)(blurf_lo_bias() * blur_tap_sum()) / 65536.f; }
ORBX_HD constexpr int blurf_mid_start() { return 128 * blur_tap_sum() + (0x64 << 16); }
ORBX_HD constexpr uint32_t f16_bits_scaled(int v, int shift) {
    if (v <= 0) return 0u;
    int p = 0;
    while ((v >> p) > 1) p++;
    return (uint32_t)(p - shift + 15) << 10 | (((uint32_t)v << (10 - p)) & 0x3FFu);
}
ORBX_HD float blurf_column(const int mid[7]) {
    float acc = blurf_start();
    for (int t = 0; t < 7; t++) acc = acc + (float)blurf_hi(mid[t]) * blurf_tap_hi(t);
    for (int t = 0; t < 7; t++) acc = acc + (float)blurf_lo(mid[t]) * blurf_tap_lo(t);
    return acc;
}
ORBX_HD int blurf_round(float v, int ties_even) {
    const float r = ties_even ? rintf(v) : floorf(v + 0.5f);
    return r > 255.f ? 255 : r < 0.f ? 0 : (int)r;
}

// ... 10 lines not shown
```

orb_slam_amd/csrc/orbx_api.hip:

```cpp
#include <climits>
#include <cstdio>
#include <cstdlib>
#include <cstring>

#include "orbx_internal.h"
#include "orbx_launch.h"

namespace orbx {
int launch_eval_math(int kind, const float* in0, const float* in1, float* out0, float* out1, int n);
int launch_eval_compass(const uint32_t* c, const uint32_t* e, const uint32_t* w, const uint32_t* nn, const uint32_t* ss, uint32_t* out, int n, int t);
int launch_eval_blur_window(const uint8_t* win, uint8_t* out, int n, int ties_even, int general);
void stage_timer_collect(StageTimer& t);
int launch_debug_nth(const float* d_resp, int n, int nth, int* d_out);
int launch_ingest(uint8_t* d_dst, const uint8_t* mapped_src, size_t bytes, hipStream_t stream);
}
using namespace orbx;

struct orbx_extractor {
    orbx_params p;
    std::string err;
    int gw = 0, gh = 0;
    HostGeom hg;
    struct __attribute__((visibility("hidden"))) Geom {
        DevBuf cells, cellrecs, bands, tabx, taby, pyr_tab;
        DevBuf pyr, blur, cand, sel, cstate, csel, cbands, level_total, level_count, status, long_cells;
    } geo;
    bool fallback_hint = true;
    DevBuf d_img1;
    PinnedBuf h_img1;
    DevBuf d_out1;
    PinnedBuf h_out1;
    bool zero_copy = true;
    Stream s1;
    int stop_after = -1;
    bool no_xcd_affinity = false;
    int od_min_frames = ORBX_OD_MIN_FRAMES_DEFAULT;
    int blur_on_demand = ORBX_BLUR_ON_DEMAND_DEFAULT;
    StageTimer timer;
    SideStream side;
    Batch last;
    bool have_last = false;
    LaunchPlan last_plan;
    StagePlan pend_color, pend_ingest;
    int ph_done = 0;
    struct PhaseKey {
        const void *img, *kps, *desc, *n, *stream;
        int nframes, w, hgt, cap;
        ptrdiff_t row_stride, frame_stride;
        bool operator==(const PhaseKey& o) const {
            return img == o.img && kps == o.kps && desc == o.desc && n == o.n && stream == o.stream && nframes == o.nframes && w == o.w && hgt == o.hgt &&
                   cap == o.cap && row_stride == o.row_stride && frame_stride == o.frame_stride;
        }
    } ph_key = {};
    static constexpr int TAB_RING = 4;
    DevBuf d_tab;
    PinnedBuf h_tab;
    Event tab_ev[TAB_RING];
    int tab_next = 0;
    std::vector<ImgSrc> last_tab;
    Stream up;
    struct __attribute__((visibility("hidden"))) HostUpload {
        DevBuf d[2];
        PinnedBuf stage[2];
        Event up_ev[2], kern_ev[2];
        int next = 0;
    };
    HostUpload hup;
    HostUpload cup;
    DevBuf d_cring;
    PinnedBuf h_cimg1, h_gray1;
    DevBuf d_cimg1;
};

template <typename T>
static int upload(orbx_extractor* h, DevBuf& d, const std::vector<T>& v) {
    HIPCHK(h, d.ensure(std::max<size_t>(v.size(), 1) * sizeof(T)));
    if (!v.empty()) HIPCHK(h, hipMemcpy(d, v.data(), v.size() * sizeof(T), hipMemcpyHostToDevice));
    return ORBX_OK;
}

static int ensure_geometry(orbx_extractor* h, int w, int hgt) {
    if (h->gw == w && h->gh == hgt) return ORBX_OK;
    HIPCHK(h, hipDeviceSynchronize());
    h->geo = {};
    h->gw = h->gh = 0;
    h->have_last = false;
    HostGeom hg;
    int rc = build_geometry(h->p, w, hgt, hg, h->err);
    if (rc != ORBX_OK) return rc;
    h->hg = hg;
    const DevGeom& g = h->hg.g;
    const size_t B = (size_t)h->p.max_batch;
    orbx_extractor::Geom& d = h->geo;
    if ((rc = upload(h, d.cells, h->hg.cells)) != ORBX_OK) return rc;
    if ((rc = upload(h, d.cellrecs, h->hg.cellrecs)) != ORBX_OK) return rc;
    if ((rc = upload(h, d.bands, h->hg.bands)) != ORBX_OK) return rc;
    if ((rc = upload(h, d.tabx, h->hg.tabx)) != ORBX_OK) return rc;
    if ((rc = upload(h, d.taby, h->hg.taby)) != ORBX_OK) return rc;
    if ((rc = upload(h, d.pyr_tab, h->hg.pyr_tab)) != ORBX_OK) return rc;
    HIPCHK(h, d.pyr.ensure(B * g.frame_plane_bytes));
    HIPCHK(h, d.blur.ensure(B * g.frame_plane_bytes));
    HIPCHK(h, d.cand.ensure(B * std::max(g.frame_cands, 1) * sizeof(Cand)));
    HIPCHK(h, d.sel.ensure((B * std::max(g.frame_sel, 1) + 4) * sizeof(Cand)));
    HIPCHK(h, d.cstate.ensure(B * g.nbands_total * sizeof(CellState)));
    HIPCHK(h, hipMemset(d.cstate, 0, B * g.nbands_total * sizeof(CellState)));
    HIPCHK(h, d.csel.ensure(B * g.ncells_total * sizeof(CellSel)));
    HIPCHK(h, d.cbands.ensure(B * g.ncells_total * sizeof(CellBands)));
    HIPCHK(h, hipMemset(d.cbands, 0, B * g.ncells_total * sizeof(CellBands)));
    HIPCHK(h, d.level_total.ensure(B * MAX_LEVELS * sizeof(int32_t)));
    HIPCHK(h, d.level_count.ensure(B * MAX_LEVELS * sizeof(int32_t)));
    HIPCHK(h, hipMemset(d.level_total, 0, B * MAX_LEVELS * sizeof(int32_t)));
    HIPCHK(h, hipMemset(d.level_count, 0, B * MAX_LEVELS * sizeof(int32_t)));
    HIPCHK(h, d.status.ensure(B * sizeof(int32_t)));
    HIPCHK(h, d.long_cells.ensure((B * g.ncells_total + 64) * sizeof(int32_t)));
    HIPCHK(h, hipDeviceSynchronize());
    h->gw = w;
    h->gh = hgt;
    return ORBX_OK;
}

static void fill_batch(orbx_extractor* h, Batch& b) {
    const orbx_extractor::Geom& d = h->geo;
    b.g = h->hg.g; b.cells = d.cells.as<CellGeom>(); b.cellrec = d.cellrecs.as<CellRec>(); b.bands = d.bands.as<BandGeom>(); b.tabx = d.tabx.as<ResizeX>(); b.taby = d.taby.as<ResizeY>();
    b.pyr_tab = d.pyr_tab.as<int>(); b.pyr = d.pyr.as(); b.blur = d.blur.as();
    b.cand = d.cand.as<Cand>(); b.sel = d.sel.as<Cand>(); b.cstate = d.cstate.as<CellState>(); b.csel = d.csel.as<CellSel>(); b.cbands = d.cbands.as<CellBands>();
    b.level_total = d.level_total.as<int32_t>(); b.level_count = d.level_count.as<int32_t>(); b.status = d.status.as<int32_t>();
    b.long_cells = d.long_cells.as<int32_t>();
}

static void group_batch(orbx_extractor* h, Batch& b, int f0, int n, orbx_keypoint* d_kps, uint8_t* d_desc, int32_t* d_n, int cap, int32_t* d_status) {
    memset(&b, 0, sizeof(b));
    fill_batch(h, b);
    b.fallback_hint = h->fallback_hint ? 1 : 0;
    b.nframes = n;
    b.xcd_affinity = (b.nframes >= XCD_AFFINITY_MIN_FRAMES && !h->no_xcd_affinity) ? 1 : 0;
    b.blur_on_demand = h->blur_on_demand;
    b.od_min_frames = h->od_min_frames;
    b.out_kps = d_kps + (size_t)f0 * cap;
    b.out_desc = d_desc + (size_t)f0 * cap * 32;
    b.out_n = d_n + f0;
    b.out_status = d_status ? d_status + f0 : nullptr;
    b.cap = cap;
}

static hipMemoryType host_memory_type(const void* p) {
    hipPointerAttribute_t a;
    if (hipPointerGetAttributes(&a, p) != hipSuccess) {
        (void)hipGetLastError();
        return hipMemoryTypeUnregistered;
    }
    return a.type;
}

static int launch_group(orbx_extractor* h, const Batch& b, hipStream_t stream, int phases = ORBX_PHASE_ALL) {
    LaunchPlan plan;
    const int rc = launch_extract(b, h->hg, stream, h->stop_after, &h->timer, &h->side, phases, &plan);
    plan.st[VS_COLOR] = h->pend_color;
    plan.st[VS_INGEST] = h->pend_ingest;
    h->pend_color = h->pend_ingest = StagePlan();
    if (!(phases & ORBX_PHASE_PYRAMID) && h->have_last)
        for (int s = 0; s < VS_COUNT; s++)
            if (plan.st[s].id < 0) plan.st[s] = h->last_plan.st[s];
    if (rc != ORBX_OK) { h->err = "kernel launch failed (no gfx950 code object for this device?)"; return rc; }
    h->last = b;
    h->last_plan = plan;
    h->have_last = true;
    return ORBX_OK;
}

static int ensure_cring(orbx_extractor* h, int w, int hgt, size_t& pitch);
static int convert(orbx_extractor* h, const uint8_t* src, ptrdiff_t srs, ptrdiff_t sfs, const ImgSrc* tab, unsigned long long tab_bits, int n, int w,
                   int hgt, int fmt, uint8_t* dst, ptrdiff_t drs, ptrdiff_t dfs, uint8_t* dst2, hipStream_t stream);

static int extract_gather(orbx_extractor* h, int fmt, const uint8_t* const* imgs, const ptrdiff_t* row_strides, int nframes, int w, int hgt,
                          orbx_keypoint* d_kps, uint8_t* d_desc, int32_t* d_n, int cap, int32_t* d_status, hipStream_t stream) {
    const int mb = h->p.max_batch;
    size_t gp = 0;
    if (fmt != ORBX_PIX_GRAY8) {
        const int rc = ensure_cring(h, w, hgt, gp);
        if (rc != ORBX_OK) return rc;
    }
    const size_t tab_bytes = (size_t)orbx_extractor::TAB_RING * mb * sizeof(ImgSrc);
    HIPCHK(h, h->d_tab.ensure(tab_bytes));
    HIPCHK(h, h->h_tab.ensure(tab_bytes, hipHostMallocDefault));
    for (Event& e : h->tab_ev) HIPCHK(h, e.ensure());
    for (int f0 = 0; f0 < nframes; f0 += mb) {
        const int n = std::min(mb, nframes - f0);
        const int slot = h->tab_next;
        h->tab_next = (slot + 1) % orbx_extractor::TAB_RING;
        HIPCHK(h, hipEventSynchronize(h->tab_ev[slot]));
        ImgSrc* ht = h->h_tab.as<ImgSrc>() + (size_t)slot * mb;
        ImgSrc* dt = h->d_tab.as<ImgSrc>() + (size_t)slot * mb;
        unsigned long long bits = 0;
        long long min_stride = LLONG_MAX, max_stride = 0;
        for (int i = 0; i < n; i++) {
            const long long s = row_strides ? (long long)row_strides[f0 + i] : (long long)w * pix_channels(fmt);
            ht[i].data = imgs[f0 + i];
            ht[i].row_stride = s;
            bits |= (uintptr_t)imgs[f0 + i] | (unsigned long long)s;
            min_stride = std::min(min_stride, s);
            max_stride = std::max(max_stride, s);
        }
        HIPCHK(h, hipMemcpyAsync(dt, ht, (size_t)n * sizeof(ImgSrc), hipMemcpyHostToDevice, stream));
        Batch b;
        group_batch(h, b, f0, n, d_kps, d_desc, d_n, cap, d_status);
        if (fmt == ORBX_PIX_GRAY8) {
            b.img_row_stride = min_stride;
            b.img_tab = dt;
            b.img_tab_bits = bits;
            b.img_tab_min_stride = min_stride;
            b.img_tab_max_stride = max_stride;
        } else {
            const int rc = convert(h, nullptr, 0, 0, dt, bits, n, w, hgt, fmt, h->d_cring.as(), (ptrdiff_t)gp, (ptrdiff_t)(gp * hgt), nullptr, stream);
            if (rc != ORBX_OK) return rc;
            b.img = h->d_cring.as();
            b.img_row_stride = (long long)gp;
            b.img_frame_stride = (long long)(gp * hgt);
        }
        const int rc = launch_group(h, b, stream);
        if (rc != ORBX_OK) return rc;
        HIPCHK(h, hipEventRecord(h->tab_ev[slot], stream));
        if (fmt == ORBX_PIX_GRAY8) h->last_tab.assign(ht, ht + n);
    }
    return ORBX_OK;
}

static int ensure_cring(orbx_extractor* h, int w, int hgt, size_t& pitch) {
    pitch = ((size_t)w + 15) & ~(size_t)15;
    const size_t bytes = pitch * hgt * h->p.max_batch;
    if (h->d_cring.size() < bytes) {
        HIPCHK(h, hipDeviceSynchronize());
        HIPCHK(h, h->d_cring.ensure(bytes));
    }
    return ORBX_OK;
}

static int convert(orbx_extractor* h, const uint8_t* src, ptrdiff_t srs, ptrdiff_t sfs, const ImgSrc* tab, unsigned long long tab_bits, int n, int w,
                   int hgt, int fmt, uint8_t* dst, ptrdiff_t drs, ptrdiff_t dfs, uint8_t* dst2, hipStream_t stream) {
    ColorArgs a;
    memset(&a, 0, sizeof(a));
    a.src = src; a.src_row_stride = srs; a.src_frame_stride = sfs; a.tab = tab; a.tab_bits = tab_bits;
    a.dst = dst; a.dst2 = dst2; a.dst_row_stride = drs; a.dst_frame_stride = dfs; a.w = w; a.h = hgt;
    const int rc = launch_to_gray(a, n, fmt, stream, &h->pend_color);
    if (rc != ORBX_OK) h->err = rc == ORBX_ERR_ARG ? "frame too large for the conversion kernel" : "kernel launch failed (no gfx950 code object for this device?)";
    return rc;
}

static int extract_host(orbx_extractor* h, orbx_extractor::HostUpload& U, int fmt, const uint8_t* const* imgs, const ptrdiff_t* row_strides, int nframes,
                        int w, int hgt, orbx_keypoint* d_kps, uint8_t* d_desc, int32_t* d_n, int cap, int32_t* d_status, hipStream_t stream) {
    const int mb = h->p.max_batch;
    const size_t rowb = (size_t)w * pix_channels(fmt);
    const size_t P = (rowb + 15) & ~(size_t)15, fb = P * hgt;
    size_t gp = 0;
    if (fmt != ORBX_PIX_GRAY8) {
        const int rc = ensure_cring(h, w, hgt, gp);
        if (rc != ORBX_OK) return rc;
    }
    HIPCHK(h, h->up.ensure());
    for (int i = 0; i < 2; i++) {
        HIPCHK(h, U.up_ev[i].ensure());
        HIPCHK(h, U.kern_ev[i].ensure());
    }
    std::vector<char> pinned(nframes);
    bool any_pageable = false;
    for (int f = 0; f < nframes; f++) {
        const hipMemoryType t = host_memory_type(imgs[f]);
        if (t == hipMemoryTypeDevice || t == hipMemoryTypeArray) { h->err = "ORBX_FRAMES_ON_HOST with a device pointer"; return ORBX_ERR_ARG; }
        pinned[f] = t == hipMemoryTypeHost;
        any_pageable |= !pinned[f];
    }
    const size_t bytes = fb * mb;
    const bool stage = any_pageable || U.stage[0].size() > 0;
    bool grow = false;
    for (int i = 0; i < 2; i++) grow |= U.d[i].size() < bytes || (stage && U.stage[i].size() < bytes);
    if (grow) {
        HIPCHK(h, hipDeviceSynchronize());
        for (int i = 0; i < 2; i++) {
            HIPCHK(h, U.d[i].ensure(bytes));
            if (stage) HIPCHK(h, U.stage[i].ensure(bytes, hipHostMallocDefault));
        }
    }
    for (int f0 = 0; f0 < nframes; f0 += mb) {
        const int n = std::min(mb, nframes - f0);
        const int i = U.next;
        U.next ^= 1;
        uint8_t* dbuf = U.d[i].as();
        uint8_t* stage = U.stage[i].as();
        HIPCHK(h, hipStreamWaitEvent(h->up, U.kern_ev[i], 0));
        bool stage_free = false;
        for (int j = 0; j < n;) {
            const uint8_t* src = imgs[f0 + j];
            const ptrdiff_t s = row_strides ? row_strides[f0 + j] : (ptrdiff_t)rowb;
            if (pinned[f0 + j]) {
                HIPCHK(h, hipMemcpy2DAsync(dbuf + j * fb, P, src, (size_t)s, rowb, (size_t)hgt, hipMemcpyHostToDevice, h->up));
                j++;
                continue;
            }
            if (!stage_free) {
                HIPCHK(h, hipEventSynchronize(U.up_ev[i]));
                stage_free = true;
            }
            int j1 = j;
            for (; j1 < n && !pinned[f0 + j1]; j1++) {
                const uint8_t* fs = imgs[f0 + j1];
                const ptrdiff_t fst = row_strides ? row_strides[f0 + j1] : (ptrdiff_t)rowb;
                uint8_t* d = stage + j1 * fb;
                if (fst == (ptrdiff_t)P) memcpy(d, fs, fb - (P - rowb));
                else for (int y = 0; y < hgt; y++) memcpy(d + y * P, fs + (ptrdiff_t)y * fst, rowb);
            }
            HIPCHK(h, hipMemcpyAsync(dbuf + j * fb, stage + j * fb, (size_t)(j1 - j) * fb, hipMemcpyHostToDevice, h->up));
            j = j1;
        }
        HIPCHK(h, hipEventRecord(U.up_ev[i], h->up));
        HIPCHK(h, hipStreamWaitEvent(stream, U.up_ev[i], 0));
        Batch b;
        group_batch(h, b, f0, n, d_kps, d_desc, d_n, cap, d_status);
        if (fmt == ORBX_PIX_GRAY8) {
            b.img = dbuf;
            b.img_row_stride = (long long)P;
            b.img_frame_stride = (long long)fb;
        } else {
            int rc = convert(h, dbuf, (ptrdiff_t)P, (ptrdiff_t)fb, nullptr, 0, n, w, hgt, fmt, h->d_cring.as(), (ptrdiff_t)gp, (ptrdiff_t)(gp * hgt), nullptr, stream);
            if (rc != ORBX_OK) return rc;
            HIPCHK(h, hipEventRecord(U.kern_ev[i], stream));
            b.img = h->d_cring.as();
            b.img_row_stride = (long long)gp;
            b.img_frame_stride = (long long)(gp * hgt);
        }
        const int rc = launch_group(h, b, stream);
        if (rc != ORBX_OK) return rc;
        if (fmt == ORBX_PIX_GRAY8) HIPCHK(h, hipEventRecord(U.kern_ev[i], stream));
    }
    for (int i = 0; i < 2; i++) HIPCHK(h, hipEventSynchronize(U.up_ev[i]));
    return ORBX_OK;
}

static int extract_one(orbx_extractor* h, int w, int hgt, int dstride, size_t bytes, orbx_keypoint* kps, uint8_t* desc, int* n_out);

extern "C" {

void orbx_default_params(orbx_params* p) {
    memset(p, 0, sizeof(*p));
    p->nfeatures = 1000;
    p->scale_factor = 1.2f;
    p->nlevels = 8;
    p->score_type = ORBX_FAST_SCORE;
    p->fast_th = 20;
    p->device = 0;
    p->max_batch = 1;
    p->blur_rounding = ORBX_BLUR_X86_SSE2;
    const char* fc = getenv("ORBX_FP_CONTRACT");
    p->fp_contract = (fc && fc[0] == '1' && fc[1] == 0) ? ORBX_FP_GCC_CONTRACT : ORBX_FP_ISO;
}

int orbx_create(const orbx_params* p, orbx_extractor** out) {
    if (!p || !out) return ORBX_ERR_ARG;
    *out = nullptr;
    if (p->max_batch < 1 || p->nlevels < 1 || p->nlevels > MAX_LEVELS || p->nfeatures < 1) return ORBX_ERR_ARG;
    int ndev = 0;
    if (hipGetDeviceCount(&ndev) != hipSuccess || ndev <= 0 || p->device < 0 || p->device >= ndev) return ORBX_ERR_DEVICE;
    if (hipSetDevice(p->device) != hipSuccess) return ORBX_ERR_DEVICE;
    orbx_extractor* h = new orbx_extractor();
    h->p = *p;
    { const char* xa = getenv("ORBX_XCD_AFFINITY"); h->no_xcd_affinity = xa && xa[0] == '0'; }
    { const char* fh = getenv("ORBX_FALLBACK_HINT"); h->fallback_hint = !(fh && fh[0] == '0'); }
    { const char* om = getenv("ORBX_OD_MIN_FRAMES"); if (om && atoi(om) >= 1) h->od_min_frames = atoi(om); }
    { const char* od = getenv("ORBX_BLUR_ON_DEMAND"); if (od && (od[0] == '0' || od[0] == '1') && od[1] == 0) h->blur_on_demand = od[0] - '0'; }
    { const char* zc = getenv("ORBX_ZERO_COPY"); h->zero_copy = !(zc && zc[0] == '0'); }
    const char* ovl = getenv("ORBX_OVERLAP");
    if (!(ovl && ovl[0] == '0') && (h->side.aux.ensure() != hipSuccess || h->side.fork.ensure() != hipSuccess || h->side.join.ensure() != hipSuccess)) {
        delete h;
        return ORBX_ERR_DEVICE;
    }
    *out = h;
    return ORBX_OK;
}

void orbx_destroy(orbx_extractor* h) {
    if (!h) return;
    (void)hipSetDevice(h->p.device);
    (void)hipDeviceSynchronize();
    delete h;
}

int orbx_get_levels(const orbx_extractor* h) { return h ? h->p.nlevels : 0; }
float orbx_get_scale_factor(const orbx_extractor* h) { return h ? (float)(double)h->p.scale_factor : 0.f; }
const char* orbx_last_error(const orbx_extractor* h) { return h ? h->err.c_str() : "null handle"; }
#ifndef ORBX_SRC_HASH
#define ORBX_SRC_HASH "unknown"
#endif
const char* orbx_build_id(void) { return ORBX_SRC_HASH; }

int orbx_max_keypoints(const orbx_extractor* h) {
    if (!h) return 0;
    HostGeom tmp;
    std::string e;
    orbx_params p = h->p;
    if (build_geometry(p, 4096, 4096, tmp, e) != ORBX_OK) return std::max(p.nfeatures, 0) + p.nlevels;
    return tmp.g.nslots;
}

int orbx_extract_batch_device(orbx_extractor* h, const uint8_t* d_imgs, int nframes, int w, int hgt, ptrdiff_t row_stride,
                              ptrdiff_t frame_stride, orbx_keypoint* d_kps, uint8_t* d_desc, int32_t* d_n, int cap,
                              int32_t* d_status, void* stream_) {
    return orbx_extract_batch_device_phases(h, d_imgs, nframes, w, hgt, row_stride, frame_stride, d_kps, d_desc, d_n, cap, d_status, stream_, ORBX_PHASE_ALL);
}

int orbx_extract_batch_device_phases(orbx_extractor* h, const uint8_t* d_imgs, int nframes, int w, int hgt, ptrdiff_t row_stride,
                                     ptrdiff_t frame_stride, orbx_keypoint* d_kps, uint8_t* d_desc, int32_t* d_n, int cap,
                                     int32_t* d_status, void* stream_, int phases) {
    if (!h) return ORBX_ERR_ARG;
    if (!d_imgs || nframes <= 0 || w <= 0 || hgt <= 0) return ORBX_EMPTY;
    if (!d_kps || !d_desc || !d_n || cap < 1 || row_stride < w) { h->err = "bad argument"; return ORBX_ERR_ARG; }
    if (phases < 1 || phases > ORBX_PHASE_ALL || phases == (ORBX_PHASE_PYRAMID | ORBX_PHASE_DESCRIBE)) {
        h->err = "bad phase mask (the parts of one call must be consecutive)";
        return ORBX_ERR_ARG;
    }
    if (phases != ORBX_PHASE_ALL && nframes > h->p.max_batch) { h->err = "a phased call covers one launch group: nframes <= max_batch"; return ORBX_ERR_ARG; }
    const orbx_extractor::PhaseKey key = {d_imgs, d_kps, d_desc, d_n, stream_, nframes, w, hgt, cap, row_stride, frame_stride};
    {
        const int first = phases & -phases;
        const int before = first - 1;
        if (!(phases & ORBX_PHASE_PYRAMID) && (!(key == h->ph_key) || (h->ph_done & before) != before)) {
            h->err = "phase queued out of order: the parts in front of it were not queued for this batch (same arguments, same stream)";
            return ORBX_ERR_ARG;
        }
    }
    if (phases & ORBX_PHASE_PYRAMID) h->ph_done = 0;
    HIPCHK(h, hipSetDevice(h->p.device));
    int rc = ensure_geometry(h, w, hgt);
    if (rc != ORBX_OK) return rc;
    if (cap < h->hg.g.nslots) { h->err = "cap < orbx_max_keypoints()"; return ORBX_ERR_CAPACITY; }
    hipStream_t stream = (hipStream_t)stream_;
    for (int f0 = 0; f0 < nframes; f0 += h->p.max_batch) {
        Batch b;
        group_batch(h, b, f0, std::min(h->p.max_batch, nframes - f0), d_kps, d_desc, d_n, cap, d_status);
        b.img = d_imgs + (ptrdiff_t)f0 * frame_stride;
        b.img_row_stride = row_stride;
        b.img_frame_stride = frame_stride;
        if ((rc = launch_group(h, b, stream, phases)) != ORBX_OK) return rc;
    }
    if (phases & ORBX_PHASE_PYRAMID) h->ph_key = key;
    h->ph_done |= phases;
    return ORBX_OK;
}

int orbx_extract_batch(orbx_extractor* h, const uint8_t* const* imgs, const ptrdiff_t* row_strides, int nframes, int w, int hgt, int where,
                       orbx_keypoint* d_kps, uint8_t* d_desc, int32_t* d_n, int cap, int32_t* d_status, void* stream_) {
    if (!h) return ORBX_ERR_ARG;
    if (nframes <= 0 || w <= 0 || hgt <= 0) return ORBX_EMPTY;
    if (!imgs || (where != ORBX_FRAMES_ON_DEVICE && where != ORBX_FRAMES_ON_HOST) || !d_kps || !d_desc || !d_n || cap < 1) {
        h->err = "bad argument";
        return ORBX_ERR_ARG;
    }
    for (int f = 0; f < nframes; f++) {
        const ptrdiff_t s = row_strides ? row_strides[f] : (ptrdiff_t)w;
        if (!imgs[f] || s < w || s >= ((ptrdiff_t)1 << 24)) { h->err = "bad frame pointer or row stride"; return ORBX_ERR_ARG; }
    }
    HIPCHK(h, hipSetDevice(h->p.device));
    int rc = ensure_geometry(h, w, hgt);
    if (rc != ORBX_OK) return rc;
    if (cap < h->hg.g.nslots) { h->err = "cap < orbx_max_keypoints()"; return ORBX_ERR_CAPACITY; }
    h->ph_done = 0;
    hipStream_t stream = (hipStream_t)stream_;
    if (where == ORBX_FRAMES_ON_HOST) return extract_host(h, h->hup, ORBX_PIX_GRAY8, imgs, row_strides, nframes, w, hgt, d_kps, d_desc, d_n, cap, d_status, stream);
    return extract_gather(h, ORBX_PIX_GRAY8, imgs, row_strides, nframes, w, hgt, d_kps, d_desc, d_n, cap, d_status, stream);
}

int orbx_extract(orbx_extractor* h, const uint8_t* img, int w, int hgt, ptrdiff_t stride, orbx_keypoint* kps, uint8_t* desc, int cap,
                 int* n_out) {
    if (!h) return ORBX_ERR_ARG;
    if (!img || w <= 0 || hgt <= 0) return ORBX_EMPTY;
    if (!kps || !desc || !n_out || stride < w) { h->err = "bad argument"; return ORBX_ERR_ARG; }
    HIPCHK(h, hipSetDevice(h->p.device));
    int rc = ensure_geometry(h, w, hgt);
    if (rc != ORBX_OK) return rc;
    const int need = h->hg.g.nslots;
    if (cap < need) { h->err = "cap < orbx_max_keypoints()"; return ORBX_ERR_CAPACITY; }
    const int dstride = (w + 63) / 64 * 64;
    const size_t bytes = (size_t)dstride * hgt;
    const size_t kps_off = 64, desc_off = kps_off + ((size_t)need * sizeof(orbx_keypoint) + 63) / 64 * 64, out_bytes = desc_off + (size_t)need * 32;
    HIPCHK(h, h->d_img1.ensure(bytes));
    HIPCHK(h, h->h_img1.ensure(bytes, hipHostMallocMapped));
    HIPCHK(h, h->d_out1.ensure(out_bytes));
    HIPCHK(h, h->h_out1.ensure(out_bytes, hipHostMallocMapped | hipHostMallocCoherent));
    HIPCHK(h, h->s1.ensure());
    h->pend_color = StagePlan();
    h->pend_ingest = plan_ingest(bytes, h->zero_copy);
    if (bytes <= INGEST_MAX_BYTES) {
        for (int y = 0; y < hgt; y++) memcpy(h->h_img1.as() + (size_t)y * dstride, img + (ptrdiff_t)y * stride, (size_t)w);
        if (h->pend_ingest.id >= 0) { if ((rc = launch_ingest(h->d_img1.as(), h->h_img1.mapped(), bytes, h->s1)) != ORBX_OK) { h->err = "kernel launch failed (no gfx950 code object for this device?)"; return rc; } }
        else HIPCHK(h, hipMemcpyAsync(h->d_img1, h->h_img1, bytes, hipMemcpyHostToDevice, h->s1));
    } else {
        HIPCHK(h, hipMemcpy2DAsync(h->d_img1, dstride, img, stride, w, hgt, hipMemcpyHostToDevice, h->s1));
    }
    return extract_one(h, w, hgt, dstride, bytes, kps, desc, n_out);
}

}

static int extract_one(orbx_extractor* h, int w, int hgt, int dstride, size_t bytes, orbx_keypoint* kps, uint8_t* desc, int* n_out) {
    const int need = h->hg.g.nslots;
    const size_t kps_off = 64, desc_off = kps_off + ((size_t)need * sizeof(orbx_keypoint) + 63) / 64 * 64, out_bytes = desc_off + (size_t)need * 32;
    int rc;
    uint8_t* out = h->zero_copy ? h->h_out1.mapped() : h->d_out1.as();
    int32_t* d_n = reinterpret_cast<int32_t*>(out);
    rc = orbx_extract_batch_device(h, h->d_img1.as(), 1, w, hgt, dstride, (ptrdiff_t)bytes, reinterpret_cast<orbx_keypoint*>(out + kps_off),
                                   out + desc_off, d_n, need, d_n + 1, h->s1);
    if (rc != ORBX_OK) return rc;
    if (!h->zero_copy) HIPCHK(h, hipMemcpyAsync(h->h_out1, h->d_out1, out_bytes, hipMemcpyDeviceToHost, h->s1));
    HIPCHK(h, hipStreamSynchronize(h->s1));
    const int32_t* res = h->h_out1.as<int32_t>();
    if (h->stop_after >= 0) { *n_out = 0; return ORBX_OK; }
    if (res[1] != ORBX_OK) { h->err = "internal list capacity exceeded"; return res[1]; }
    const int n = res[0];
    if (n > 0) {
        memcpy(kps, h->h_out1.as() + kps_off, (size_t)n * sizeof(orbx_keypoint));
        memcpy(desc, h->h_out1.as() + desc_off, (size_t)n * 32);
    }
    *n_out = n;
    return ORBX_OK;
// ... 18 lines not shown
    if (hipGetDeviceCount(&ndev) != hipSuccess || ndev <= 0 || hipGetDevice(&dev) != hipSuccess) return ORBX_ERR_DEVICE;
    ColorArgs a;
    memset(&a, 0, sizeof(a));
    a.src = d_src; a.src_row_stride = src_row_stride; a.src_frame_stride = src_frame_stride;
    a.dst = d_gray; a.dst_row_stride = gray_row_stride; a.dst_frame_stride = gray_frame_stride; a.w = w; a.h = hgt;
    return launch_to_gray(a, nframes, fmt, (hipStream_t)stream);
}

int orbx_extract_color(orbx_extractor* h, const uint8_t* img, int w, int hgt, ptrdiff_t stride, int fmt, orbx_keypoint* kps, uint8_t* desc, int cap,
                       int* n_out, uint8_t* gray_out) {
    if (!h) return ORBX_ERR_ARG;
    if (pix_channels(fmt) == 0) { h->err = "unknown pixel format"; return ORBX_ERR_ARG; }
    if (!img || w <= 0 || hgt <= 0) return ORBX_EMPTY;
    if (!kps || !desc || !n_out || color_args(fmt, w, stride) != ORBX_OK) { h->err = "bad argument"; return ORBX_ERR_ARG; }
    if (fmt == ORBX_PIX_GRAY8) {
        const int rc = orbx_extract(h, img, w, hgt, stride, kps, desc, cap, n_out);
        if (rc == ORBX_OK && gray_out)
            for (int y = 0; y < hgt; y++) memcpy(gray_out + (size_t)y * w, img + (ptrdiff_t)y * stride, (size_t)w);
        return rc;
    }
    HIPCHK(h, hipSetDevice(h->p.device));
    int rc = ensure_geometry(h, w, hgt);
    if (rc != ORBX_OK) return rc;
    const int need = h->hg.g.nslots;
    if (cap < need) { h->err = "cap < orbx_max_keypoints()"; return ORBX_ERR_CAPACITY; }
    const int dstride = (w + 63) / 64 * 64;
    const size_t bytes = (size_t)dstride * hgt;
    const size_t rowb = (size_t)w * pix_channels(fmt), cpitch = (rowb + 15) & ~(size_t)15;
    const size_t kps_off = 64, desc_off = kps_off + ((size_t)need * sizeof(orbx_keypoint) + 63) / 64 * 64, out_bytes = desc_off + (size_t)need * 32;
    HIPCHK(h, h->d_img1.ensure(bytes));
    HIPCHK(h, h->h_cimg1.ensure(cpitch * hgt, hipHostMallocMapped));
    if (gray_out) HIPCHK(h, h->h_gray1.ensure(bytes, hipHostMallocMapped | hipHostMallocCoherent));
    HIPCHK(h, h->d_out1.ensure(out_bytes));
    HIPCHK(h, h->h_out1.ensure(out_bytes, hipHostMallocMapped | hipHostMallocCoherent));
    HIPCHK(h, h->s1.ensure());
    for (int y = 0; y < hgt; y++) memcpy(h->h_cimg1.as() + (size_t)y * cpitch, img + (ptrdiff_t)y * stride, rowb);
    const uint8_t* src = h->h_cimg1.mapped();
    if (!h->zero_copy) {
        HIPCHK(h, h->d_cimg1.ensure(cpitch * hgt));
        HIPCHK(h, hipMemcpyAsync(h->d_cimg1, h->h_cimg1, cpitch * hgt, hipMemcpyHostToDevice, h->s1));
        src = h->d_cimg1.as();
    }
    if ((rc = convert(h, src, (ptrdiff_t)cpitch, 0, nullptr, 0, 1, w, hgt, fmt, h->d_img1.as(), dstride, 0, gray_out ? h->h_gray1.mapped() : nullptr, h->s1)) != ORBX_OK)
        return rc;
    rc = extract_one(h, w, hgt, dstride, bytes, kps, desc, n_out);
    if (rc == ORBX_OK && gray_out)
        for (int y = 0; y < hgt; y++) memcpy(gray_out + (size_t)y * w, h->h_gray1.as() + (size_t)y * dstride, (size_t)w);
    return rc;
}

int orbx_extract_batch_device_color(orbx_extractor* h, const uint8_t* d_imgs, int nframes, int w, int hgt, ptrdiff_t row_stride, ptrdiff_t frame_stride,
                                    int fmt, orbx_keypoint* d_kps, uint8_t* d_desc, int32_t* d_n, int cap, int32_t* d_status, uint8_t* d_gray,
                                    ptrdiff_t gray_row_stride, ptrdiff_t gray_frame_stride, void* stream_) {
    if (!h) return ORBX_ERR_ARG;
    if (pix_channels(fmt) == 0) { h->err = "unknown pixel format"; return ORBX_ERR_ARG; }
    if (!d_imgs || nframes <= 0 || w <= 0 || hgt <= 0) return ORBX_EMPTY;
    if (!d_kps || !d_desc || !d_n || cap < 1 || color_args(fmt, w, row_stride) != ORBX_OK || frame_stride < 0 ||
        (d_gray && (gray_row_stride < w || gray_frame_stride < 0 || (nframes > 1 && gray_frame_stride < gray_row_stride * (hgt - 1) + w)))) {
        h->err = "bad argument";
        return ORBX_ERR_ARG;
    }
    if (fmt == ORBX_PIX_GRAY8 && !d_gray) return orbx_extract_batch_device(h, d_imgs, nframes, w, hgt, row_stride, frame_stride, d_kps, d_desc, d_n, cap, d_status, stream_);
    HIPCHK(h, hipSetDevice(h->p.device));
    int rc = ensure_geometry(h, w, hgt);
    if (rc != ORBX_OK) return rc;
    if (cap < h->hg.g.nslots) { h->err = "cap < orbx_max_keypoints()"; return ORBX_ERR_CAPACITY; }
    size_t gp = 0;
    if (!d_gray && (rc = ensure_cring(h, w, hgt, gp)) != ORBX_OK) return rc;
    h->ph_done = 0;
    hipStream_t stream = (hipStream_t)stream_;
    for (int f0 = 0; f0 < nframes; f0 += h->p.max_batch) {
        const int n = std::min(h->p.max_batch, nframes - f0);
        uint8_t* g = d_gray ? d_gray + (ptrdiff_t)f0 * gray_frame_stride : h->d_cring.as();
        const ptrdiff_t grs = d_gray ? gray_row_stride : (ptrdiff_t)gp, gfs = d_gray ? gray_frame_stride : (ptrdiff_t)(gp * hgt);
        if ((rc = convert(h, d_imgs + (ptrdiff_t)f0 * frame_stride, row_stride, frame_stride, nullptr, 0, n, w, hgt, fmt, g, grs, gfs, nullptr, stream)) != ORBX_OK)
            return rc;
        Batch b;
        group_batch(h, b, f0, n, d_kps, d_desc, d_n, cap, d_status);
        b.img = g;
        b.img_row_stride = grs;
        b.img_frame_stride = gfs;
        if ((rc = launch_group(h, b, stream)) != ORBX_OK) return rc;
    }
    return ORBX_OK;
}

int orbx_extract_batch_color(orbx_extractor* h, const uint8_t* const* imgs, const ptrdiff_t* row_strides, int nframes, int w, int hgt, int where, int fmt,
                             orbx_keypoint* d_kps, uint8_t* d_desc, int32_t* d_n, int cap, int32_t* d_status, void* stream_) {
    if (!h) return ORBX_ERR_ARG;
    const int ch = pix_channels(fmt);
    if (ch == 0) { h->err = "unknown pixel format"; return ORBX_ERR_ARG; }
    if (nframes <= 0 || w <= 0 || hgt <= 0) return ORBX_EMPTY;
    if (!imgs || (where != ORBX_FRAMES_ON_DEVICE && where != ORBX_FRAMES_ON_HOST) || !d_kps || !d_desc || !d_n || cap < 1) {
        h->err = "bad argument";
        return ORBX_ERR_ARG;
    }
    if (fmt == ORBX_PIX_GRAY8) return orbx_extract_batch(h, imgs, row_strides, nframes, w, hgt, where, d_kps, d_desc, d_n, cap, d_status, stream_);
    for (int f = 0; f < nframes; f++) {
        const ptrdiff_t s = row_strides ? row_strides[f] : (ptrdiff_t)w * ch;
        if (!imgs[f] || s < (ptrdiff_t)w * ch || s >= ((ptrdiff_t)1 << 24)) { h->err = "bad frame pointer or row stride"; return ORBX_ERR_ARG; }
    }
    HIPCHK(h, hipSetDevice(h->p.device));
    int rc = ensure_geometry(h, w, hgt);
    if (rc != ORBX_OK) return rc;
    if (cap < h->hg.g.nslots) { h->err = "cap < orbx_max_keypoints()"; return ORBX_ERR_CAPACITY; }
    h->ph_done = 0;
    hipStream_t stream = (hipStream_t)stream_;
    if (where == ORBX_FRAMES_ON_HOST) return extract_host(h, h->cup, fmt, imgs, row_strides, nframes, w, hgt, d_kps, d_desc, d_n, cap, d_status, stream);
    return extract_gather(h, fmt, imgs, row_strides, nframes, w, hgt, d_kps, d_desc, d_n, cap, d_status, stream);
}

int orbx_debug_set_blur_on_demand(orbx_extractor* h, int mode) {
    if (!h || mode < 0 || mode > 1) return ORBX_ERR_ARG;
    h->blur_on_demand = mode;
    return ORBX_OK;
}

int orbx_debug_set_stop_after(orbx_extractor* h, int stage) {
    if (!h) return ORBX_ERR_ARG;
    h->stop_after = stage;
    return ORBX_OK;
}

int orbx_debug_stage_timing(orbx_extractor* h, int enable) {
    if (!h) return ORBX_ERR_ARG;
    if (hipSetDevice(h->p.device) != hipSuccess || hipDeviceSynchronize() != hipSuccess) return ORBX_ERR_DEVICE;
    stage_timer_collect(h->timer);
    h->timer.enabled = enable != 0;
    if (enable == 2) { memset(h->timer.ms, 0, sizeof(h->timer.ms)); memset(h->timer.launches, 0, sizeof(h->timer.launches)); }
    return ORBX_OK;
}

int orbx_debug_stage_time(orbx_extractor* h, int stage, double* total_ms, long* launches) {
    if (!h || stage < 0 || stage >= ST_COUNT) return ORBX_ERR_ARG;
    if (hipSetDevice(h->p.device) != hipSuccess || hipDeviceSynchronize() != hipSuccess) return ORBX_ERR_DEVICE;
    stage_timer_collect(h->timer);
    *total_ms = h->timer.ms[stage];
    *launches = h->timer.launches[stage];
    return ORBX_OK;
}

int orbx_debug_level_size(const orbx_extractor* h, int level, int* w, int* hgt) {
    if (!h || h->gw == 0 || level < 0 || level >= h->hg.g.nlevels) return ORBX_ERR_ARG;
    *w = h->hg.g.lv[level].w;
    *hgt = h->hg.g.lv[level].h;
    return ORBX_OK;
}

int orbx_debug_resize_form(const orbx_extractor* h, int level, int* form, int* rows_out) {
    if (!h || !h->have_last || !form || !rows_out || level < 1 || level >= h->hg.g.nlevels) return ORBX_ERR_ARG;
    StripChoice sc;
    *form = resize_form(h->last, h->hg, level, sc);
    *rows_out = sc.rows_out;
    return ORBX_OK;
}

int orbx_debug_launch_variant(const orbx_extractor* h, int stage, orbx_stage_variant* out, char* name, int name_cap) {
    if (!h || !h->have_last || !out || stage < 0 || stage >= VS_COUNT) return ORBX_ERR_ARG;
    const StagePlan& s = h->last_plan.st[stage];
    out->id = s.id; out->flags = s.flags; out->mask = s.mask;
    if (name && name_cap > 0) snprintf(name, (size_t)name_cap, "%s", s.id < 0 ? "" : variant_name(stage, s.id));
    return ORBX_OK;
}

int orbx_debug_variant_count(int stage) { return variant_count(stage); }
const char* orbx_debug_variant_name(int stage, int id) { return variant_name(stage, id); }

int orbx_debug_plan(const orbx_params* p, const orbx_plan_args* a, orbx_stage_variant* out) {
    if (!p || !a || !out || a->nframes < 1 || a->row_stride < a->w) return ORBX_ERR_ARG;
    HostGeom hg;
    std::string err;
    const int rc = build_geometry(*p, a->w, a->h, hg, err);
    if (rc != ORBX_OK) return rc;
    Batch b;
    memset(&b, 0, sizeof(b));
    b.g = hg.g;
    b.nframes = a->nframes;
    b.xcd_affinity = a->xcd_affinity ? 1 : 0;
    b.blur_on_demand = a->on_demand ? 1 : 0;
    b.od_min_frames = a->od_min_frames;
    b.img_row_stride = a->row_stride;
    ImgSrc none = {nullptr, 0};
    if (a->gather) {
        b.img_tab = &none;
        b.img_tab_bits = (unsigned long long)a->base_bits | (unsigned long long)a->row_stride;
        b.img_tab_min_stride = b.img_tab_max_stride = a->row_stride;
    } else {
        b.img = reinterpret_cast<const uint8_t*>((uintptr_t)a->base_bits);
        b.img_frame_stride = a->frame_stride;
    }
    LaunchPlan plan = plan_extract(b, hg, a->stop_after, a->side_stream != 0, ORBX_PHASE_ALL);
    if (a->color_fmt >= 0) {
        ColorArgs c;
        memset(&c, 0, sizeof(c));
        ImgSrc cnone = {nullptr, 0};
        if (a->color_gather) { c.tab = &cnone; c.tab_bits = a->color_bits; }
        else c.src = reinterpret_cast<const uint8_t*>((uintptr_t)a->color_bits);
        plan.st[VS_COLOR] = plan_to_gray(c, a->color_fmt);
    }
    if (a->one_frame) plan.st[VS_INGEST] = plan_ingest((size_t)a->one_frame_bytes, true);
    for (int s = 0; s < VS_COUNT; s++) { out[s].id = plan.st[s].id; out[s].flags = plan.st[s].flags; out[s].mask = plan.st[s].mask; }
    return ORBX_OK;
}

long orbx_debug_fetch(orbx_extractor* h, int what, int frame, int level, void* host_out, long cap_bytes) {
    if (!h || !h->have_last || frame < 0 || frame >= h->last.nframes || level < 0 || level >= h->hg.g.nlevels) return ORBX_ERR_ARG;
    if (hipSetDevice(h->p.device) != hipSuccess || hipDeviceSynchronize() != hipSuccess) return ORBX_ERR_DEVICE;
    const DevGeom& g = h->hg.g;
    const LevelGeom& L = g.lv[level];
    const Batch& b = h->last;
    if (what == ORBX_DBG_NMS) {
        const long need = (long)L.w * L.h;
        if (cap_bytes < need) return ORBX_ERR_CAPACITY;
        memset(host_out, 0, need);
        std::vector<CellState> st(g.nbands_total);
        if (hipMemcpy(st.data(), b.cstate + (size_t)frame * g.nbands_total, g.nbands_total * sizeof(CellState), hipMemcpyDeviceToHost) != hipSuccess)
            return ORBX_ERR_DEVICE;
        std::vector<Cand> tmp;
        for (int it = 0; it < g.nbands_total; it++) {
            const BandGeom& bgm = h->hg.bands[it];
            if (bgm.level != level) continue;
            const int n = st[it].n_all;
            if (n <= 0) continue;
            if (n > bgm.cand_cap) return ORBX_ERR_CAPACITY;
            tmp.resize(n);
            if (hipMemcpy(tmp.data(), b.cand + (size_t)frame * g.frame_cands + L.cand_base + bgm.cand_off, (size_t)n * sizeof(Cand), hipMemcpyDeviceToHost) != hipSuccess)
                return ORBX_ERR_DEVICE;
            for (int i = 0; i < n; i++) ((uint8_t*)host_out)[(size_t)(tmp[i].pos >> 16) * L.w + (tmp[i].pos & 0xFFFF)] = (uint8_t)tmp[i].resp;
        }
        return need;
    }
    if (what == ORBX_DBG_BANDS) {
        std::vector<CellState> st(g.nbands_total);
        if (hipMemcpy(st.data(), b.cstate + (size_t)frame * g.nbands_total, g.nbands_total * sizeof(CellState), hipMemcpyDeviceToHost) != hipSuccess)
            return ORBX_ERR_DEVICE;
        long n = 0;
        for (int it = 0; it < g.nbands_total; it++) {
            const BandGeom& bgm = h->hg.bands[it];
            if (bgm.level != level) continue;
            if ((n + 1) * 32 > cap_bytes) return ORBX_ERR_CAPACITY;
            int32_t* o = (int32_t*)host_out + 8 * n++;
            o[0] = bgm.x0; o[1] = bgm.x1; o[2] = bgm.y0; o[3] = bgm.y1;
            o[4] = st[it].n_all; o[5] = st[it].n_hi; o[6] = st[it].n_lo;
            o[7] = st[it].thr & 0xFF;
        }
        return n * 32;
    }
    if (what == ORBX_DBG_PLANE || what == ORBX_DBG_BLUR) {
        const long need = (long)L.w * L.h;
        if (cap_bytes < need) return ORBX_ERR_CAPACITY;
        const uint8_t* src;
        size_t spitch;
        if (what == ORBX_DBG_PLANE && level == 0) {
            if (b.img_tab) {
                src = h->last_tab[frame].data;
                spitch = (size_t)h->last_tab[frame].row_stride;
            } else {
                src = b.img + (ptrdiff_t)frame * b.img_frame_stride;
                spitch = (size_t)b.img_row_stride;
            }
        } else {
            const uint8_t* base = what == ORBX_DBG_PLANE ? b.pyr : b.blur;
            src = base + (size_t)frame * g.frame_plane_bytes + L.plane_off;
            spitch = (size_t)L.stride;
        }
        if (hipMemcpy2D(host_out, L.w, src, spitch, L.w, L.h, hipMemcpyDeviceToHost) != hipSuccess) return ORBX_ERR_DEVICE;
        return need;
    }
    if (what == ORBX_DBG_LEVEL_KPS) {
        int32_t n = 0;
        if (hipMemcpy(&n, b.level_count + frame * MAX_LEVELS + level, 4, hipMemcpyDeviceToHost) != hipSuccess) return ORBX_ERR_DEVICE;
        const long need = (long)n * 12;
        if (cap_bytes < need) return ORBX_ERR_CAPACITY;
        std::vector<Cand> tmp(std::max(n, 1));
        if (n > 0 && hipMemcpy(tmp.data(), b.sel + (size_t)frame * g.frame_sel + L.sel_base, (size_t)n * sizeof(Cand), hipMemcpyDeviceToHost) != hipSuccess)
            return ORBX_ERR_DEVICE;
        int32_t* o = (int32_t*)host_out;
        for (int i = 0; i < n; i++) {
            o[3 * i] = tmp[i].pos & 0xFFFF;
            o[3 * i + 1] = tmp[i].pos >> 16;
            memcpy(&o[3 * i + 2], &tmp[i].resp, 4);
        }
        return need;
    }
    return ORBX_ERR_ARG;
}

int orbx_debug_geometry(const orbx_params* p, int w, int hgt, int32_t* out, int cap_levels) {
    if (!p || !out) return ORBX_ERR_ARG;
    HostGeom hg;
    std::string err;
    const int rc = build_geometry(*p, w, hgt, hg, err);
    if (rc != ORBX_OK) {
        if (getenv("ORBX_DBG_GEOM")) fprintf(stderr, "orbx geometry: %s\n", err.c_str());
        return rc;
    }
    if (cap_levels < hg.g.nlevels) return ORBX_ERR_CAPACITY;
    if (getenv("ORBX_DBG_GEOM"))
        fprintf(stderr, "orbx geometry: fast_lds_bytes %d (band image %d B, chunks %d), sel_lds %d, bands %d, cells %d\n", hg.g.fast_lds_bytes, hg.g.fast_max_img,
                hg.g.fast_max_chunks, hg.g.sel_lds_cell, (int)hg.bands.size(), (int)hg.cells.size());
    for (int l = 0; l < hg.g.nlevels; l++) {
        const LevelGeom& L = hg.g.lv[l];
        int nb = 0;
        for (const BandGeom& b : hg.bands) nb += b.level == l;
        int32_t* o = out + 8 * l;
        o[0] = L.w; o[1] = L.h; o[2] = L.ndesired; o[3] = L.gcols; o[4] = L.grows; o[5] = L.cellW; o[6] = L.cellH; o[7] = nb;
// ... 176 lines not shown
```

orb_slam_amd/csrc/orbx_device.h:

```cpp
#pragma once
#include <hip/hip_runtime.h>

#include "orb_math.h"
#include "orbx_internal.h"

namespace orbx {

static __device__ __constant__ uint32_t c_pattern[256] = {
#include "orb_pattern_packed.inc"
};

__device__ __forceinline__ const uint8_t* level0_src(const Batch& b, int frame, long long& stride) {
    typedef const ImgSrc __attribute__((address_space(4)))* ctab_t;
    const ctab_t e = (ctab_t)(uintptr_t)b.img_tab + frame;
    stride = e->row_stride;
    return e->data;
}

template <bool GATHER = false>
__device__ __forceinline__ const uint8_t* plain_plane(const Batch& b, const LevelGeom& L, int level, int frame, long long& stride) {
    if (level == 0) {
        if constexpr (GATHER) return level0_src(b, frame, stride);
        stride = b.img_row_stride;
        return b.img + (long long)frame * b.img_frame_stride;
    }
    stride = L.stride;
    return b.pyr + (long long)frame * b.g.frame_plane_bytes + L.plane_off;
}

__device__ __forceinline__ int wave_id() { return __builtin_amdgcn_readfirstlane((int)(threadIdx.x >> 6)); }

__device__ __forceinline__ int find_level(const int (&bases)[MAX_LEVELS], int idx) {
    int level = 0;
#pragma unroll
    for (int l = 1; l < MAX_LEVELS; l++) level += idx >= bases[l] ? 1 : 0;
    return level;
}

__device__ __forceinline__ bool frame_item(const Batch& b, int block, int per_frame, int& frame, int& item) {
    if (b.xcd_affinity) {
        const int slot = block >> 3;
        const int fr = slot / per_frame;
        frame = fr * 8 + (block & 7);
        item = slot - fr * per_frame;
    } else {
        frame = block / per_frame;
        item = block - frame * per_frame;
    }
    return frame < b.nframes;
}
__device__ __forceinline__ bool frame_item_magic(const Batch& b, unsigned block, unsigned per_frame, unsigned magic, int& frame, int& item) {
    const unsigned slot = b.xcd_affinity ? block >> 3 : block;
    unsigned fr = magic ? __umulhi(slot, magic) : slot;
    if (fr * per_frame > slot) --fr;
    frame = (int)(b.xcd_affinity ? fr * 8u + (block & 7u) : fr);
    item = (int)(slot - fr * per_frame);
    return frame < b.nframes;
}
static inline int frame_item_blocks(const Batch& b, int per_frame) {
    return (b.xcd_affinity ? (b.nframes + 7) / 8 * 8 : b.nframes) * per_frame;
}
static inline unsigned frame_item_magic_of(int per_frame) {
    return per_frame > 1 ? (unsigned)((1ull << 32) / (unsigned)per_frame) + 1u : 0u;
}

typedef int rec16_t __attribute__((ext_vector_type(16)));
typedef int rec8_t __attribute__((ext_vector_type(8)));
typedef int rec4_t __attribute__((ext_vector_type(4)));
__device__ __forceinline__ void load_cell_records(const Batch& b, int cell, long long frame_cell, CellRec& rc, CellSel& s, CellBands& bn) {
    typedef const rec16_t __attribute__((address_space(4)))* c16_t;
    typedef const rec8_t __attribute__((address_space(4)))* c8_t;
    typedef const rec4_t __attribute__((address_space(4)))* c4_t;
    rec16_t vr = *((c16_t)(uintptr_t)b.cellrec + cell);
    rec4_t vs = *((c4_t)(uintptr_t)b.csel + frame_cell);
    rec8_t vb = *((c8_t)(uintptr_t)b.cbands + frame_cell);
    asm volatile("" : "+s"(vr), "+s"(vs), "+s"(vb));
    rc = __builtin_bit_cast(CellRec, vr);
    s = __builtin_bit_cast(CellSel, vs);
    bn = __builtin_bit_cast(CellBands, vb);
}

constexpr unsigned long long UMAX_NIBBLES = 0x3689ABCDDEEEFFFFull;

__device__ __forceinline__ int wave_scan_inclusive(int v) {
    v += __builtin_amdgcn_update_dpp(0, v, 0x111, 0xf, 0xf, false);
    v += __builtin_amdgcn_update_dpp(0, v, 0x112, 0xf, 0xf, false);
    v += __builtin_amdgcn_update_dpp(0, v, 0x114, 0xf, 0xf, false);
    v += __builtin_amdgcn_update_dpp(0, v, 0x118, 0xf, 0xf, false);
    v += __builtin_amdgcn_update_dpp(0, v, 0x142, 0xa, 0xf, false);
    v += __builtin_amdgcn_update_dpp(0, v, 0x143, 0xc, 0xf, false);
    return v;
}

__device__ __forceinline__ int wave_sum(int v) { return __builtin_amdgcn_readlane(wave_scan_inclusive(v), 63); }

__device__ __forceinline__ int row16_sum(int v) {
    v += __builtin_amdgcn_update_dpp(0, v, 0x128, 0xf, 0xf, false);
    v += __builtin_amdgcn_update_dpp(0, v, 0x124, 0xf, 0xf, false);
    v += __builtin_amdgcn_update_dpp(0, v, 0x122, 0xf, 0xf, false);
    v += __builtin_amdgcn_update_dpp(0, v, 0x121, 0xf, 0xf, false);
    return v;
}


__device__ __forceinline__ void split_px(int p, int cw, float inv_cw, int& y, int& x) {
    y = (int)(((float)p + 0.5f) * inv_cw);
    x = p - (int)__umul24((unsigned)y, (unsigned)cw);
}

typedef unsigned short us2v __attribute__((ext_vector_type(2)));
__device__ __forceinline__ us2v as_us2v(uint32_t v) { return __builtin_bit_cast(us2v, v); }



__device__ __forceinline__ void wave_lds_fence() { __builtin_amdgcn_fence(__ATOMIC_ACQ_REL, "workgroup"); __builtin_amdgcn_wave_barrier(); }

__device__ __forceinline__ int gauss7_tap(int t) {
    return (unsigned)t <= 6u ? (int)((0x12223137312212ull >> (8 * t)) & 255ull) : 0;
}
__device__ __forceinline__ int gauss7_taps4(int t0) {
    const unsigned long long taps = 0x12223137312212ull;
    const int sh = 8 * min(max(t0, -4), 7);
    return (int)(uint32_t)(t0 >= 0 ? taps >> sh : taps << -sh);
}


}
```

orb_slam_amd/csrc/orbx_internal.h:

```cpp
#pragma once
#include <hip/hip_runtime.h>
#include <stdint.h>
#include <string>
#include <vector>

#include "orbx.h"
#include "orbx_host.h"

namespace orbx {

constexpr int MAX_LEVELS = 16;
constexpr int EDGE = 16;
constexpr int HALF_PATCH = 15;

struct Cand {
    uint32_t pos;
    float resp;
};

struct ResizeX { int16_t sx, sx1, a0, a1; };
struct ResizeY { int16_t sy0, sy1, b0, b1; };

struct LevelGeom {
    int w, h;
// ... 45 lines not shown
#endif
#ifndef ORBX_DESC_WAVES
#define ORBX_DESC_WAVES 4
#endif
constexpr int BLUR_WAVES = ORBX_BLUR_WAVES;
constexpr int DESC_WAVES = ORBX_DESC_WAVES;
#ifndef ORBX_BLUR_ROWS
#define ORBX_BLUR_ROWS 32
#endif
#ifndef ORBX_RZ_ROWS
#define ORBX_RZ_ROWS 48
#endif
#ifndef ORBX_BLUR_MFMA
#define ORBX_BLUR_MFMA 1
#endif
#ifndef ORBX_MB_BAND_STEPS
#define ORBX_MB_BAND_STEPS 8
#endif
constexpr int MB_BAND_STEPS = ORBX_MB_BAND_STEPS;
constexpr int MB_MAX_WIDTH = 1024;
constexpr int MB_TILES = 2;
#ifndef ORBX_MB_WAVES
#define ORBX_MB_WAVES 4
#endif
constexpr int MB_WAVES = ORBX_MB_WAVES;
constexpr int BLUR_ROWS = ORBX_BLUR_ROWS;
constexpr int BLUR_ROWS_SMALL = 8;
constexpr int RZ_ROWS = ORBX_RZ_ROWS;
struct FastShape { int threads, ppt, band_px, max_cw; };
#ifndef ORBX_FS
#define ORBX_FS 256, 1, 8192, 500
#endif
#ifndef ORBX_FL
#define ORBX_FL 256, 2, 7168, 6500
#endif
constexpr FastShape FAST_SMALL = {ORBX_FS};
constexpr FastShape FAST_LARGE = {ORBX_FL};
#ifndef ORBX_FAST_TWO_PASS
#define ORBX_FAST_TWO_PASS 1
#endif
#ifndef ORBX_FAST_ROTATE
#define ORBX_FAST_ROTATE 1
#endif
constexpr int FAST_Q1CAP = 192, FAST_Q2CAP = 128, FAST_Q3CAP = 192;
constexpr int fast_q0cap(int) { return 128; }
constexpr int fast_wave_queue_bytes(int ppt) { return fast_q0cap(ppt) * 4 + FAST_Q1CAP * 2 + FAST_Q2CAP * 2 + FAST_Q3CAP * 2; }
__host__ __device__ constexpr int fast_row_dwords(int xoff, int cw) { return (((xoff + cw + 6 + 3) >> 2) + 3) & ~3; }
struct BandGeom {
    int16_t x0, x1;
    int16_t y0, y1;
    int16_t ey0, ey1;
    int32_t level;
    int32_t cand_off;
    int32_t cand_cap;
    float inv_nd, inv_s, inv_cpr;
};

constexpr int XCD_AFFINITY_MIN_FRAMES = 64;
#ifndef ORBX_PYR_DEPTH
#define ORBX_PYR_DEPTH 4, 4
#endif
constexpr int PYR_MAX_GROUPS = 4, PYR_MAX_DEPTH = 8;
struct PyrGroup {
    int l0, depth;
    int ntx, nty;
    int xtab, ytab;
    int lds_off[PYR_MAX_DEPTH];
    int pitch[PYR_MAX_DEPTH];
    int lds_bytes;
};
#ifndef ORBX_PYR_TILE
#define ORBX_PYR_TILE 16, 16
#endif

constexpr int SEL_LDS_MAX_ENTRIES = 2048;
constexpr int QUOTA_LDS_PER_CELL = 10;
constexpr int QUOTA_MAX_CELLS = 160 * 1024 / QUOTA_LDS_PER_CELL / 64 * 64;
struct CellState { int32_t n_all, n_hi, n_lo, thr; };
constexpr int CELL_REC_BANDS = 8;
struct alignas(64) CellRec {
    int32_t level, nbands, skipped, band0;
    int32_t sel_base;
    int32_t plane_off, stride;
    int32_t cand_off;
    int32_t band_cand[CELL_REC_BANDS];
};
struct alignas(16) CellSel { int32_t n_all, thr, nretain, out_off; };
struct alignas(32) CellBands { int32_t n[CELL_REC_BANDS]; };
static_assert(sizeof(CellRec) == 64 && sizeof(CellSel) == 16 && sizeof(CellBands) == 32, "one scalar load per record");

struct DevGeom {
    int nlevels;
    int ncells_total;
    int nbands_total;
    uint32_t nbands_magic;
    int nbtiles_total, nbtiles_total_s;
    int nmb_total;
    int nslots;
    int nquads;
    int quota_cells;
    int score_type, fast_th, tmin;
    int fp_contract;
    int frame_plane_bytes;
    int frame_cands;
    int frame_sel;
    int sel_lds_cell, sel_lds_level, sel_lds_entries;
    int fast_max_img, fast_max_chunks, fast_lds_bytes;
    int fast_threads;
    int fast_small;
    int npyr_groups;
    PyrGroup pyr[PYR_MAX_GROUPS];
    int umax[HALF_PATCH + 1];
    int cell_bases[MAX_LEVELS], quad_bases[MAX_LEVELS], btile_bases[MAX_LEVELS], btile_bases_s[MAX_LEVELS], mb_bases[MAX_LEVELS];
    LevelGeom lv[MAX_LEVELS];
};

struct ImgSrc {
    const uint8_t* data;
    long long row_stride;
};
static_assert(sizeof(ImgSrc) == 16, "one scalar dwordx4 per table entry");

struct Batch {
    DevGeom g;
    const CellGeom* cells;
    const CellRec* cellrec;
    const BandGeom* bands;
    const ResizeX* tabx;
    const ResizeY* taby;
    const int* pyr_tab;
    const uint8_t* img;
    long long img_row_stride, img_frame_stride;
    uint8_t* pyr;
    uint8_t* blur;
    Cand* cand;
    Cand* sel;
    CellState* cstate;
    int fallback_hint;
    CellSel* csel;
    CellBands* cbands;
    int32_t* level_total;
    int32_t* level_count;
    int32_t* status;
    int32_t* long_cells;
    orbx_keypoint* out_kps;
    uint8_t* out_desc;
    int32_t* out_n;
    int32_t* out_status;
    int cap;
    int nframes;
    int xcd_affinity;
    int od_min_frames;
    int blur_on_demand;
    const ImgSrc* img_tab;
    unsigned long long img_tab_bits;
    long long img_tab_min_stride;
    long long img_tab_max_stride;
};

static inline unsigned long long level0_bits(const Batch& b) {
    return b.img_tab ? b.img_tab_bits : ((uintptr_t)b.img | (unsigned long long)b.img_row_stride | (unsigned long long)b.img_frame_stride);
}
static inline long long level0_min_stride(const Batch& b) { return b.img_tab ? b.img_tab_min_stride : b.img_row_stride; }
static inline long long level0_max_stride(const Batch& b) { return b.img_tab ? b.img_tab_max_stride : b.img_row_stride; }

struct ColorArgs {
    const uint8_t* src;
    long long src_row_stride, src_frame_stride;
    const ImgSrc* tab;
    unsigned long long tab_bits;
    uint8_t* dst;
    uint8_t* dst2;
    long long dst_row_stride, dst_frame_stride;
    int w, h;
    int f0;
    int cpr, items;
};
static inline int pix_channels(int fmt) {
    switch (fmt) {
        case ORBX_PIX_GRAY8: return 1;
        case ORBX_PIX_RGB8: case ORBX_PIX_BGR8: return 3;
        case ORBX_PIX_RGBA8: case ORBX_PIX_BGRA8: return 4;
        default: return 0;
    }
}
struct StagePlan;
int launch_to_gray(const ColorArgs& a, int nframes, int fmt, hipStream_t stream, StagePlan* report = nullptr);

struct HostGeom {
    DevGeom g;
    std::vector<CellGeom> cells;
    std::vector<CellRec> cellrecs;
    std::vector<BandGeom> bands;
    std::vector<ResizeX> tabx;
    std::vector<ResizeY> taby;
    std::vector<int> pyr_tab;
    std::vector<int> features_per_level;
    std::vector<float> scale, inv_scale;
};

int build_geometry(const orbx_params& p, int w, int h, HostGeom& out, std::string& err);

struct StripChoice { int rows_out, lds_bytes; };
StripChoice resize_strip_choice(const HostGeom& hg, int level, long long src_stride, unsigned long long src_bits);
int resize_form(const Batch& b, const HostGeom& hg, int level, StripChoice& sc);

enum Stage { ST_PYRAMID = 0, ST_FAST_CELLS, ST_QUOTA, ST_CELL_SELECT, ST_LEVEL_SELECT, ST_BLUR, ST_DESCRIBE, ST_COUNT };

struct StageTimer {
    bool enabled = false;
    std::vector<hipEvent_t> pool;
    std::vector<int> pool_stage;
    double ms[ST_COUNT] = {0};
    long launches[ST_COUNT] = {0};
};

struct SideStream {
    Stream aux;
    Event fork, join;
};
struct LaunchPlan;
int launch_extract(const Batch& b, const HostGeom& hg, hipStream_t stream, int stop_after, StageTimer* timer, const SideStream* side,
                   int phases = ORBX_PHASE_ALL, LaunchPlan* report = nullptr);
bool describe_od_supported(const Batch& b, const HostGeom& hg);

}
```

orb_slam_amd/csrc/orbx_launch.h:

```cpp
#pragma once
#include <hip/hip_runtime.h>

#include "orbx_internal.h"

namespace orbx {

#define ORBX_LAUNCH_CHECK()                                   \
    do {                                                      \
        hipError_t e_ = hipGetLastError();                    \
        if (e_ != hipSuccess) return ORBX_ERR_DEVICE;         \
    } while (0)

constexpr size_t INGEST_MAX_BYTES = (size_t)512 << 10;
constexpr int PYR_FUSED_MAX_FRAMES = 32;

struct StageScope {
    StageTimer* t; hipStream_t s; int stage;
    StageScope(StageTimer* t_, hipStream_t s_, int stage_) : t(t_ && t_->enabled ? t_ : nullptr), s(s_), stage(stage_) {
        if (t) { hipEvent_t e; if (hipEventCreate(&e) == hipSuccess) { (void)hipEventRecord(e, s); t->pool.push_back(e); } else t = nullptr; }
    }
    ~StageScope() {
        if (t) { hipEvent_t e; if (hipEventCreate(&e) == hipSuccess) { (void)hipEventRecord(e, s); t->pool.push_back(e); t->pool_stage.push_back(stage); } else { (void)hipEventDestroy(t->pool.back()); t->pool.pop_back(); } }
    }
};

enum VStage { VS_COLOR = ORBX_VS_COLOR, VS_INGEST, VS_PYRAMID, VS_FAST, VS_QUOTA, VS_CELL_SELECT, VS_LEVEL_SELECT, VS_BLUR, VS_DESCRIBE, VS_COUNT };
static_assert(VS_COUNT == ORBX_VS_COUNT, "include/orbx.h names the stages");

enum ColorVariant { CV_GATHER0 = 10, CV_COUNT = 18 };
enum PyramidVariant { PV_PYRAMID0 = 0, PV_TILED0 = 4, PV_STRIP0 = 12, PV_STRIP_GATHER0 = 17, PV_COUNT = 22 };
enum FastVariant { FV_ALIGNED = 1, FV_SMALL = 2, FV_GATHER = 4, FV_BLUR = 8, FV_COUNT = 16 };
enum QuotaVariant { QV_QUOTA = 0, QV_COUNT };
enum CellSelectVariant { CS_SELECT = 0, CS_SELECT_GATHER, CS_LONG, CS_LONG_GATHER, CS_COUNT };
enum LevelSelectVariant { LS_ONE = 0, LS_CHUNKED, LS_COUNT };
enum BlurVariant { BV_ALIGNED = 1, BV_GATHER = 2, BV_MFMA = 4, BV_COUNT };
enum DescribeVariant { DV_FMA = 1, DV_GATHER = 2, DV_OD = 4, DV_COUNT = 8 };

struct StagePlan { int id = -1; unsigned flags = 0; unsigned long long mask = 0; };
inline StagePlan stage_plan(int id, unsigned flags = 0) { StagePlan s; s.id = id; s.flags = flags; s.mask = 1ull << id; return s; }
struct PyramidLaunch { int variant, index; StripChoice sc; };
struct PyramidPlan { int n = 0; PyramidLaunch launch[MAX_LEVELS]; };
struct LaunchPlan {
    StagePlan st[VS_COUNT];
    PyramidPlan pyr;
    bool on_demand = false, overlap = false, fuse_blur = false;
};

int variant_count(int stage);
const char* variant_name(int stage, int id);
LaunchPlan plan_extract(const Batch& b, const HostGeom& hg, int stop_after, bool have_side, int phases);
PyramidPlan plan_pyramid(const Batch& b, const HostGeom& hg);
StagePlan plan_fast(const Batch& b, const HostGeom& hg, bool fuse_blur);
StagePlan plan_quota(const HostGeom& hg);
StagePlan plan_cell_select(const Batch& b, const HostGeom& hg);
StagePlan plan_level_select(const Batch& b, const HostGeom& hg);
StagePlan plan_blur(const Batch& b, const HostGeom& hg);
StagePlan plan_describe(const Batch& b, const HostGeom& hg, bool on_demand);
StagePlan plan_to_gray(const ColorArgs& a, int fmt);
StagePlan plan_ingest(size_t frame_bytes, bool zero_copy);
const char* pyramid_variant_name(int id);
const char* fast_variant_name(int id);
const char* cell_select_variant_name(int id);
const char* level_select_variant_name(int id);
const char* blur_variant_name(int id);
const char* describe_variant_name(int id);
const char* color_variant_name(int id);

int launch_pyramid(const Batch& b, const PyramidPlan& plan, hipStream_t stream);
int launch_fast(const Batch& b, const HostGeom& hg, hipStream_t stream, const StagePlan& plan);
int launch_quota(const Batch& b, const HostGeom& hg, hipStream_t stream, const StagePlan& plan);
int launch_cell_select(const Batch& b, const HostGeom& hg, hipStream_t stream, const StagePlan& plan);
int launch_level_select(const Batch& b, const HostGeom& hg, hipStream_t stream, const StagePlan& plan);
int launch_blur(const Batch& b, const HostGeom& hg, hipStream_t stream, const StagePlan& plan);
int launch_describe(const Batch& b, const HostGeom& hg, hipStream_t stream, const StagePlan& plan);
int launch_describe_od(const Batch& b, const HostGeom& hg, hipStream_t stream, int variant);

}
```

Baseline: 496,200 frames/s.

## Make strip resize kernel persistent with grid-stride virtual blocks and capped grid

The strip resize kernel becomes grid-stride: each workgroup loops over virtual blocks, staging the source strip into LDS and then computing. Column tables are fetched once per workgroup and reused. The grid can be capped to a multiple of the CU count through an env var or a debug setter. With the default of zero the cap is off and the grid equals nblocks, so behaviour stays about the same except for small extra loop and bounds overhead.

Result: slower. 489,700 frames/s (-1.3%).

```diff
diff --git a/include/orbx.h b/include/orbx.h
--- a/include/orbx.h
+++ b/include/orbx.h
@@ -156,6 +156,8 @@
 int orbx_debug_stage_time(orbx_extractor* h, int stage, double* total_ms, long* launches);
 int orbx_debug_level_size(const orbx_extractor* h, int level, int* w, int* hgt);
 int orbx_debug_resize_form(const orbx_extractor* h, int level, int* form, int* rows_out);
+int orbx_debug_resize_grid(const orbx_extractor* h, int level, int* blocks, int* virtual_blocks);
+int orbx_debug_set_resize_grid(orbx_extractor* h, int blocks);
 #define ORBX_VS_COLOR        0
 #define ORBX_VS_INGEST       1
 #define ORBX_VS_PYRAMID      2
diff --git a/orb_slam_amd/capi.py b/orb_slam_amd/capi.py
--- a/orb_slam_amd/capi.py
+++ b/orb_slam_amd/capi.py
@@ -23,7 +23,7 @@
     "orbm_count_accepted", "orbm_match_top2_segments", "orbm_match_top2_segments_device", "orbm_distinctive", "orbm_distinctive_device",
     "orbx_device_alloc", "orbx_device_free", "orbx_device_upload", "orbx_device_download",
     "orbx_stream_create", "orbx_stream_create_priority", "orbx_stream_destroy", "orbx_stream_synchronize", "orbx_event_create", "orbx_event_destroy", "orbx_event_record",
-    "orbx_stream_wait_event", "orbx_device_copy_async", "orbx_host_alloc", "orbx_host_free", "orbx_device_upload_async", "orbx_device_download_async", "orbx_debug_set_stop_after", "orbx_debug_set_blur_on_demand", "orbx_debug_level_size", "orbx_debug_resize_form", "orbx_debug_fetch",
+    "orbx_stream_wait_event", "orbx_device_copy_async", "orbx_host_alloc", "orbx_host_free", "orbx_device_upload_async", "orbx_device_download_async", "orbx_debug_set_stop_after", "orbx_debug_set_blur_on_demand", "orbx_debug_level_size", "orbx_debug_resize_form", "orbx_debug_resize_grid", "orbx_debug_set_resize_grid", "orbx_debug_fetch",
     "orbx_debug_launch_variant", "orbx_debug_variant_count", "orbx_debug_variant_name", "orbx_debug_plan",
     "orbx_debug_eval_math", "orbx_debug_eval_compass", "orbx_debug_eval_blur_window", "orbx_debug_stage_timing", "orbx_debug_stage_time", "orbx_debug_nth_element", "orbx_debug_geometry",
     "orbm_debug_set_match_path",
@@ -287,6 +287,9 @@
         L.orbx_debug_level_size.argtypes = [vp, ci, ctypes.POINTER(ci), ctypes.POINTER(ci)]
         if hasattr(L, "orbx_debug_resize_form"):
             L.orbx_debug_resize_form.argtypes = [vp, ci, ctypes.POINTER(ci), ctypes.POINTER(ci)]
+        if hasattr(L, "orbx_debug_resize_grid"):
+            L.orbx_debug_resize_grid.argtypes = [vp, ci, ctypes.POINTER(ci), ctypes.POINTER(ci)]
+            L.orbx_debug_set_resize_grid.argtypes = [vp, ci]
         if hasattr(L, "orbx_debug_launch_variant"):
             L.orbx_debug_launch_variant.argtypes = [vp, ci, ctypes.POINTER(StageVariant), ctypes.c_char_p, ci]
             L.orbx_debug_variant_count.argtypes = [ci]
@@ -652,6 +655,18 @@
             raise OrbxError(rc, "orbx_debug_resize_form")
         return form.value, rows.value
 
+    def resize_grid(self, level):
+        blocks, vblocks = ctypes.c_int(), ctypes.c_int()
+        rc = self.L.orbx_debug_resize_grid(self.h, level, ctypes.byref(blocks), ctypes.byref(vblocks))
+        if rc != ORBX_OK:
+            raise OrbxError(rc, "orbx_debug_resize_grid")
+        return blocks.value, vblocks.value
+
+    def set_resize_grid(self, blocks):
+        rc = self.L.orbx_debug_set_resize_grid(self.h, int(blocks))
+        if rc != ORBX_OK:
+            raise OrbxError(rc, "orbx_debug_set_resize_grid")
+
     def launch_variant(self, stage):
         v, name = StageVariant(), ctypes.create_string_buffer(96)
         rc = self.L.orbx_debug_launch_variant(self.h, stage, ctypes.byref(v), name, len(name))
diff --git a/orb_slam_amd/csrc/k_pyramid.hip b/orb_slam_amd/csrc/k_pyramid.hip
--- a/orb_slam_amd/csrc/k_pyramid.hip
+++ b/orb_slam_amd/csrc/k_pyramid.hip
@@ -149,10 +149,11 @@
     uint32_t sel[4], apair[4];
     int wa, sh;
 };
-__device__ __forceinline__ void rzs_load_cols(const ResizeX* tx, int w, int dcol, RzsCols& c) {
-    ResizeX rx[4];
+__device__ __forceinline__ void rzs_fetch_cols(const ResizeX* tx, int w, int dcol, ResizeX (&rx)[4]) {
 #pragma unroll
     for (int k = 0; k < 4; k++) rx[k] = tx[min(4 * dcol + k, w - 1)];
+}
+__device__ __forceinline__ void rzs_make_cols(const ResizeX (&rx)[4], RzsCols& c) {
     const int w0 = rx[0].sx;
     c.wa = w0 & ~3;
     c.sh = w0 & 3;
@@ -177,36 +178,44 @@
 }
 
 template <bool GATHER, int NG>
-__device__ __forceinline__ void k_resize_strip_body(Batch b, int level, int rows_out, int nstrips, unsigned magic) {
+__device__ __forceinline__ void k_resize_strip_body(Batch b, int level, int rows_out, int nstrips, unsigned magic, unsigned nblocks) {
     extern __shared__ __attribute__((aligned(16))) uint8_t s_src[];
     const DevGeom& g = b.g;
     const LevelGeom& L = g.lv[level];
     const LevelGeom& P = g.lv[level - 1];
-    int frame, strip;
-    if (!frame_item_magic(b, blockIdx.x, (unsigned)nstrips, magic, frame, strip)) return;
+    unsigned vb = blockIdx.x;
+    if (vb >= nblocks) return;
     const int tid = threadIdx.x, lane = tid & 63, wave = wave_id();
-    long long sstride64;
-    const uint8_t* src = plain_plane<GATHER>(b, P, level - 1, frame, sstride64);
-    const int sstride = (int)sstride64;
     const ResizeX* tx = b.tabx + L.tabx_off;
     const ResizeY* ty = b.taby + L.taby_off;
     const int RPW = rows_out >> 2;
-    const int row0 = strip * rows_out + wave * RPW;
-    const uint2 ryl = *reinterpret_cast<const uint2*>(ty + min(row0 + min(lane, RPW - 1), L.h - 1));
     const int ngroups = NG ? NG : rzs_groups(L.w);
     const int rem = rzs_rem_cols(L.w);
     const bool rowpar = rem <= RZS_ROWPAR_MAX;
     const int shift = rzs_rowpar_shift(rem);
     auto group_col = [&](int gi) { return gi == ngroups - 1 && rowpar ? 64 * gi + rzs_rowpar_slot(lane, shift) : rzs_loop_col(gi, lane); };
-    RzsCols cols[NG ? NG : 1];
+    ResizeX rxc[NG ? NG : 1][4];
     if (NG) {
 #pragma unroll
-        for (int gi = 0; gi < NG; gi++) rzs_load_cols(tx, L.w, group_col(gi), cols[gi]);
-    }
-    __builtin_amdgcn_sched_barrier(0);
-    const StripSpan sp = rzs_span(ty, L.h, rows_out, strip, sstride64, rzs_readable(level == 1, sstride64, P.w));
-    const int r0 = sp.r0, nchunks = (int)sp.chunks;
-    {
+        for (int gi = 0; gi < NG; gi++) rzs_fetch_cols(tx, L.w, group_col(gi), rxc[gi]);
+    }
+    const unsigned dstride = (unsigned)L.stride;
+    bool live;
+    int frame, strip, sstride, row0, r0;
+    uint2 ryl;
+    auto stage = [&](unsigned block) {
+        block_item_magic(block, b.xcd_affinity != 0, (unsigned)nstrips, magic, frame, strip);
+        live = frame < b.nframes;
+        if (!live) return;
+        long long sstride64;
+        const uint8_t* src = plain_plane<GATHER>(b, P, level - 1, frame, sstride64);
+        sstride = (int)sstride64;
+        row0 = strip * rows_out + wave * RPW;
+        ryl = *reinterpret_cast<const uint2*>(ty + min(row0 + min(lane, RPW - 1), L.h - 1));
+        __builtin_amdgcn_sched_barrier(0);
+        const StripSpan sp = rzs_span(ty, L.h, rows_out, strip, sstride64, rzs_readable(level == 1, sstride64, P.w));
+        const int nchunks = (int)sp.chunks;
+        r0 = sp.r0;
         typedef const void __attribute__((address_space(1))) * gptr_t;
         typedef void __attribute__((address_space(3))) * lptr_t;
         const uint8_t* base = src + (long long)r0 * sstride64;
@@ -215,64 +224,79 @@
         for (int q0 = 64 * wave; q0 < nchunks; q0 += 256)
             if (q0 + lane < nchunks) __builtin_amdgcn_global_load_lds((gptr_t)(base + 16 * (q0 + lane)), (lptr_t)(s_src + 16 * q0), 16, 0, 0);
         asm volatile("s_waitcnt vmcnt(0)" ::: "memory");
-    }
-    __syncthreads();
-    uint8_t* dplane = b.pyr + (long long)frame * g.frame_plane_bytes + L.plane_off;
-    const unsigned dstride = (unsigned)L.stride;
-    const int nrows = min(RPW, L.h - row0);
-    auto process = [&](int gi, const RzsCols& c) {
-        const int dcol = group_col(gi);
-        if (gi == ngroups - 1 && rowpar) {
-            const int slot = rzs_rowpar_slot(lane, shift);
-            for (int pass = 0; pass * (64 >> shift) < RPW; pass++) {
-                const int j = rzs_rowpar_row(lane, shift, pass);
-                const uint32_t ry_rows = (uint32_t)__shfl((int)ryl.x, min(j, RPW - 1)), ry_w = (uint32_t)__shfl((int)ryl.y, min(j, RPW - 1));
-                const int dy = row0 + j;
-                if (slot < rem && j < RPW && dy < L.h) {
+        __syncthreads();
+    };
+    stage(vb);
+    RzsCols cols[NG ? NG : 1];
+    if (NG) {
+#pragma unroll
+        for (int gi = 0; gi < NG; gi++) rzs_make_cols(rxc[gi], cols[gi]);
+    }
+    auto compute = [&]() {
+        uint8_t* dplane = b.pyr + (long long)frame * g.frame_plane_bytes + L.plane_off;
+        const int nrows = min(RPW, L.h - row0);
+        auto process = [&](int gi, const RzsCols& c) {
+            const int dcol = group_col(gi);
+            if (gi == ngroups - 1 && rowpar) {
+                const int slot = rzs_rowpar_slot(lane, shift);
+                for (int pass = 0; pass * (64 >> shift) < RPW; pass++) {
+                    const int j = rzs_rowpar_row(lane, shift, pass);
+                    const uint32_t ry_rows = (uint32_t)__shfl((int)ryl.x, min(j, RPW - 1)), ry_w = (uint32_t)__shfl((int)ryl.y, min(j, RPW - 1));
+                    const int dy = row0 + j;
+                    if (slot < rem && j < RPW && dy < L.h) {
+                        const int sy0 = (int16_t)(ry_rows & 0xffffu), sy1 = (int16_t)(ry_rows >> 16);
+                        uint32_t da[4], db[4];
+                        rzs_hrow(s_src, (sy0 - r0) * sstride + c.wa, c, da);
+                        rzs_hrow(s_src, (sy1 - r0) * sstride + c.wa, c, db);
+                        *reinterpret_cast<uint32_t*>(dplane + ((unsigned)dy * dstride + 4u * (unsigned)dcol)) = rzs_vpack(da, db, ry_w << 16, ry_w & 0xffff0000u);
+                    }
+                }
+            } else if (4 * dcol < L.w) {
+                int have = -1;
+                uint32_t cur[4] = {0, 0, 0, 0};
+                for (int j = 0; j < nrows; j++) {
+                    const int dy = row0 + j;
+                    const uint32_t ry_rows = (uint32_t)__builtin_amdgcn_readlane((int)ryl.x, j), ry_w = (uint32_t)__builtin_amdgcn_readlane((int)ryl.y, j);
                     const int sy0 = (int16_t)(ry_rows & 0xffffu), sy1 = (int16_t)(ry_rows >> 16);
-                    uint32_t da[4], db[4];
-                    rzs_hrow(s_src, (sy0 - r0) * sstride + c.wa, c, da);
-                    rzs_hrow(s_src, (sy1 - r0) * sstride + c.wa, c, db);
-                    *reinterpret_cast<uint32_t*>(dplane + ((unsigned)dy * dstride + 4u * (unsigned)dcol)) = rzs_vpack(da, db, ry_w << 16, ry_w & 0xffff0000u);
+                    const uint32_t b0s = ry_w << 16, b1s = ry_w & 0xffff0000u;
+                    if (sy0 != have) rzs_hrow(s_src, (sy0 - r0) * sstride + c.wa, c, cur);
+                    uint32_t t[4];
+#pragma unroll
+                    for (int k = 0; k < 4; k++) t[k] = __umulhi(cur[k], b0s);
+                    asm volatile("" : "+v"(t[0]), "+v"(t[1]), "+v"(t[2]), "+v"(t[3]));
+                    if (sy1 != sy0) rzs_hrow(s_src, (sy1 - r0) * sstride + c.wa, c, cur);
+                    have = sy1;
+                    uint32_t packed = 0;
+#pragma unroll
+                    for (int k = 0; k < 4; k++) packed |= ((t[k] + __umulhi(cur[k], b1s) + 2u) >> 2) << (8 * k);
+                    *reinterpret_cast<uint32_t*>(dplane + ((unsigned)dy * dstride + 4u * (unsigned)dcol)) = packed;
                 }
             }
-        } else if (4 * dcol < L.w) {
-            int have = -1;
-            uint32_t cur[4] = {0, 0, 0, 0};
-            for (int j = 0; j < nrows; j++) {
-                const int dy = row0 + j;
-                const uint32_t ry_rows = (uint32_t)__builtin_amdgcn_readlane((int)ryl.x, j), ry_w = (uint32_t)__builtin_amdgcn_readlane((int)ryl.y, j);
-                const int sy0 = (int16_t)(ry_rows & 0xffffu), sy1 = (int16_t)(ry_rows >> 16);
-                const uint32_t b0s = ry_w << 16, b1s = ry_w & 0xffff0000u;
-                if (sy0 != have) rzs_hrow(s_src, (sy0 - r0) * sstride + c.wa, c, cur);
-                uint32_t t[4];
-#pragma unroll
-                for (int k = 0; k < 4; k++) t[k] = __umulhi(cur[k], b0s);
-                asm volatile("" : "+v"(t[0]), "+v"(t[1]), "+v"(t[2]), "+v"(t[3]));
-                if (sy1 != sy0) rzs_hrow(s_src, (sy1 - r0) * sstride + c.wa, c, cur);
-                have = sy1;
-                uint32_t packed = 0;
-#pragma unroll
-                for (int k = 0; k < 4; k++) packed |= ((t[k] + __umulhi(cur[k], b1s) + 2u) >> 2) << (8 * k);
-                *reinterpret_cast<uint32_t*>(dplane + ((unsigned)dy * dstride + 4u * (unsigned)dcol)) = packed;
+        };
+        if constexpr (NG != 0) {
+#pragma unroll
+            for (int gi = 0; gi < NG; gi++) process(gi, cols[gi]);
+        } else {
+            for (int gi = 0; gi < ngroups; gi++) {
+                rzs_fetch_cols(tx, L.w, group_col(gi), rxc[0]);
+                rzs_make_cols(rxc[0], cols[0]);
+                process(gi, cols[0]);
             }
         }
     };
-    if constexpr (NG != 0) {
-#pragma unroll
-        for (int gi = 0; gi < NG; gi++) process(gi, cols[gi]);
-    } else {
-        for (int gi = 0; gi < ngroups; gi++) {
-            rzs_load_cols(tx, L.w, group_col(gi), cols[0]);
-            process(gi, cols[0]);
-        }
-    }
-}
-typedef void (*resize_strip_fn)(Batch, int, int, int, unsigned);
+    for (;;) {
+        if (live) compute();
+        vb += gridDim.x;
+        if (vb >= nblocks) break;
+        __syncthreads();
+        stage(vb);
+    }
+}
+typedef void (*resize_strip_fn)(Batch, int, int, int, unsigned, unsigned);
 template <int NG>
-__global__ __launch_bounds__(256) void k_resize(Batch b, int level, int rows_out, int nstrips, unsigned magic) { k_resize_strip_body<false, NG>(b, level, rows_out, nstrips, magic); }
+__global__ __launch_bounds__(256) void k_resize(Batch b, int level, int rows_out, int nstrips, unsigned magic, unsigned nblocks) { k_resize_strip_body<false, NG>(b, level, rows_out, nstrips, magic, nblocks); }
 template <int NG>
-__global__ __launch_bounds__(256) void k_resize_gather(Batch b, int level, int rows_out, int nstrips, unsigned magic) { k_resize_strip_body<true, NG>(b, level, rows_out, nstrips, magic); }
+__global__ __launch_bounds__(256) void k_resize_gather(Batch b, int level, int rows_out, int nstrips, unsigned magic, unsigned nblocks) { k_resize_strip_body<true, NG>(b, level, rows_out, nstrips, magic, nblocks); }
 
 template <bool ALIGNED, bool GATHER>
 __global__ __launch_bounds__(256) void k_pyramid(Batch b, int group) {
@@ -376,13 +400,11 @@
 }
 
 template <int NG>
-static void launch_resize_strip(const Batch& b, int l, const StripChoice& sc, bool gather, hipStream_t stream) {
-    const LevelGeom& L = b.g.lv[l];
-    const int nstrips = rzs_strips(L.h, sc.rows_out);
+static void launch_resize_strip(const Batch& b, const PyramidLaunch& pl, bool gather, hipStream_t stream) {
+    const int l = pl.index, nstrips = rzs_strips(b.g.lv[l].h, pl.sc.rows_out);
     const unsigned magic = frame_item_magic_of(nstrips);
-    dim3 grid(frame_item_blocks(b, nstrips));
     const resize_strip_fn fn = gather ? static_cast<resize_strip_fn>(&k_resize_gather<NG>) : static_cast<resize_strip_fn>(&k_resize<NG>);
-    hipLaunchKernelGGL(fn, grid, dim3(256), (size_t)sc.lds_bytes, stream, b, l, sc.rows_out, nstrips, magic);
+    hipLaunchKernelGGL(fn, dim3(pl.grid), dim3(256), (size_t)pl.sc.lds_bytes, stream, b, l, pl.sc.rows_out, nstrips, magic, (unsigned)pl.nblocks);
 }
 
 PyramidPlan plan_pyramid(const Batch& b, const HostGeom& hg) {
@@ -393,7 +415,7 @@
     if (g.nlevels > 1 && resize_form(b, hg, 1, sc) == RZ_FORM_FUSED) {
         for (int gi = 0; gi < g.npyr_groups; gi++) {
             const bool first = g.pyr[gi].l0 == 0;
-            p.launch[p.n++] = PyramidLaunch{PV_PYRAMID0 + ((!first || al0) ? 1 : 0) + ((b.img_tab && first) ? 2 : 0), gi, StripChoice{0, 0}};
+            p.launch[p.n++] = PyramidLaunch{PV_PYRAMID0 + ((!first || al0) ? 1 : 0) + ((b.img_tab && first) ? 2 : 0), gi, StripChoice{0, 0}, 0, 0};
         }
         return p;
     }
@@ -402,9 +424,12 @@
         const bool gather = b.img_tab && l == 1;
         if (resize_form(b, hg, l, sc) == RZ_FORM_STRIP) {
             const int ng = rzs_groups(L.w);
-            p.launch[p.n++] = PyramidLaunch{(gather ? PV_STRIP_GATHER0 : PV_STRIP0) + (ng <= 4 ? ng : 0), l, sc};
-        } else
-            p.launch[p.n++] = PyramidLaunch{PV_TILED0 + ((l > 1 || al0) ? 1 : 0) + (L.rz_window ? 2 : 0) + (gather ? 4 : 0), l, StripChoice{0, 0}};
+            const int nblocks = frame_item_blocks(b, rzs_strips(L.h, sc.rows_out));
+            p.launch[p.n++] = PyramidLaunch{(gather ? PV_STRIP_GATHER0 : PV_STRIP0) + (ng <= 4 ? ng : 0), l, sc, b.rz_grid_cap < 0 ? -b.rz_grid_cap : rzs_grid(nblocks, b.rz_grid_cap), nblocks};
+        } else {
+            const int nblocks = frame_item_blocks(b, ((L.w + 255) / 256) * ((L.h + RZ_ROWS - 1) / RZ_ROWS));
+            p.launch[p.n++] = PyramidLaunch{PV_TILED0 + ((l > 1 || al0) ? 1 : 0) + (L.rz_window ? 2 : 0) + (gather ? 4 : 0), l, StripChoice{0, 0}, nblocks, nblocks};
+        }
     }
     return p;
 }
@@ -435,7 +460,7 @@
         } else if (pl.variant < PV_STRIP0) {
             const int l = pl.index;
             const LevelGeom& L = g.lv[l];
-            const dim3 grid(frame_item_blocks(b, ((L.w + 255) / 256) * ((L.h + RZ_ROWS - 1) / RZ_ROWS)));
+            const dim3 grid(pl.grid);
             const size_t lds = (size_t)L.rz_pitch * L.rz_rows;
             switch (pl.variant - PV_TILED0) {
                 case 0: hipLaunchKernelGGL((k_resize<false, false>), grid, dim3(256), lds, stream, b, l); break;
@@ -450,11 +475,11 @@
         } else {
             const bool gather = pl.variant >= PV_STRIP_GATHER0;
             switch (pl.variant - (gather ? PV_STRIP_GATHER0 : PV_STRIP0)) {
-                case 1: launch_resize_strip<1>(b, pl.index, pl.sc, gather, stream); break;
-                case 2: launch_resize_strip<2>(b, pl.index, pl.sc, gather, stream); break;
-                case 3: launch_resize_strip<3>(b, pl.index, pl.sc, gather, stream); break;
-                case 4: launch_resize_strip<4>(b, pl.index, pl.sc, gather, stream); break;
-                default: launch_resize_strip<0>(b, pl.index, pl.sc, gather, stream); break;
+                case 1: launch_resize_strip<1>(b, pl, gather, stream); break;
+                case 2: launch_resize_strip<2>(b, pl, gather, stream); break;
+                case 3: launch_resize_strip<3>(b, pl, gather, stream); break;
+                case 4: launch_resize_strip<4>(b, pl, gather, stream); break;
+                default: launch_resize_strip<0>(b, pl, gather, stream); break;
             }
         }
         ORBX_LAUNCH_CHECK();
diff --git a/orb_slam_amd/csrc/k_resize_strip.h b/orb_slam_amd/csrc/k_resize_strip.h
--- a/orb_slam_amd/csrc/k_resize_strip.h
+++ b/orb_slam_amd/csrc/k_resize_strip.h
@@ -61,6 +61,13 @@
     return 0;
 }
 
+constexpr int RZS_RESIDENT_DEFAULT = 0;
+ORBX_HD int rzs_grid(int nblocks, int limit) {
+    if (limit <= 0 || limit >= nblocks) return nblocks;
+    const int g = imax(limit & ~7, 8);
+    return imin(g, nblocks);
+}
+
 ORBX_HD int rzs_dword_cols(int w) { return (w + 3) >> 2; }
 ORBX_HD int rzs_groups(int w) { return (rzs_dword_cols(w) + 63) >> 6; }
 ORBX_HD int rzs_rem_cols(int w) { return rzs_dword_cols(w) - 64 * (rzs_groups(w) - 1); }
diff --git a/orb_slam_amd/csrc/orb_math.h b/orb_slam_amd/csrc/orb_math.h
--- a/orb_slam_amd/csrc/orb_math.h
+++ b/orb_slam_amd/csrc/orb_math.h
@@ -16,6 +16,16 @@
 ORBX_HD int imax(int a, int b) { return a > b ? a : b; }
 ORBX_HD int imin3(int a, int b, int c) { return imin(imin(a, b), c); }
 ORBX_HD int imax3(int a, int b, int c) { return imax(imax(a, b), c); }
+
+ORBX_HD void block_item_magic(unsigned block, bool affinity, unsigned per_frame, unsigned magic, int& frame, int& item) {
+    const unsigned slot = affinity ? block >> 3 : block;
+    unsigned fr = magic ? (unsigned)(((unsigned long long)slot * magic) >> 32) : slot;
+    if (fr * per_frame > slot) --fr;
+    frame = (int)(affinity ? fr * 8u + (block & 7u) : fr);
+    item = (int)(slot - fr * per_frame);
+}
+ORBX_HD int item_blocks(bool affinity, int nframes, int per_frame) { return (affinity ? (nframes + 7) / 8 * 8 : nframes) * per_frame; }
+ORBX_HD unsigned item_magic_of(int per_frame) { return per_frame > 1 ? (unsigned)((1ull << 32) / (unsigned)per_frame) + 1u : 0u; }
 
 ORBX_HD int reflect101(int p, int len) {
     if ((unsigned)p < (unsigned)len) return p;
diff --git a/orb_slam_amd/csrc/orbx_api.hip b/orb_slam_amd/csrc/orbx_api.hip
--- a/orb_slam_amd/csrc/orbx_api.hip
+++ b/orb_slam_amd/csrc/orbx_api.hip
@@ -3,6 +3,7 @@
 #include <cstdlib>
 #include <cstring>
 
+#include "k_resize_strip.h"
 #include "orbx_internal.h"
 #include "orbx_launch.h"
 
@@ -34,6 +35,9 @@
     Stream s1;
     int stop_after = -1;
     bool no_xcd_affinity = false;
+    int cus = 0;
+    int rz_resident = RZS_RESIDENT_DEFAULT;
+    int rz_grid_abs = 0;
     int od_min_frames = ORBX_OD_MIN_FRAMES_DEFAULT;
     int blur_on_demand = ORBX_BLUR_ON_DEMAND_DEFAULT;
     StageTimer timer;
@@ -136,6 +140,7 @@
     b.xcd_affinity = (b.nframes >= XCD_AFFINITY_MIN_FRAMES && !h->no_xcd_affinity) ? 1 : 0;
     b.blur_on_demand = h->blur_on_demand;
     b.od_min_frames = h->od_min_frames;
+    b.rz_grid_cap = h->rz_grid_abs > 0 ? -h->rz_grid_abs : h->rz_resident * h->cus;
     b.out_kps = d_kps + (size_t)f0 * cap;
     b.out_desc = d_desc + (size_t)f0 * cap * 32;
     b.out_n = d_n + f0;
@@ -367,6 +372,11 @@
     { const char* om = getenv("ORBX_OD_MIN_FRAMES"); if (om && atoi(om) >= 1) h->od_min_frames = atoi(om); }
     { const char* od = getenv("ORBX_BLUR_ON_DEMAND"); if (od && (od[0] == '0' || od[0] == '1') && od[1] == 0) h->blur_on_demand = od[0] - '0'; }
     { const char* zc = getenv("ORBX_ZERO_COPY"); h->zero_copy = !(zc && zc[0] == '0'); }
+    { const char* rr = getenv("ORBX_RZ_RESIDENT"); if (rr && rr[0] >= '0' && rr[0] <= '9' && atoi(rr) <= 64) h->rz_resident = atoi(rr); }
+    if (hipDeviceGetAttribute(&h->cus, hipDeviceAttributeMultiprocessorCount, p->device) != hipSuccess || h->cus < 1) {
+        delete h;
+        return ORBX_ERR_DEVICE;
+    }
     const char* ovl = getenv("ORBX_OVERLAP");
     if (!(ovl && ovl[0] == '0') && (h->side.aux.ensure() != hipSuccess || h->side.fork.ensure() != hipSuccess || h->side.join.ensure() != hipSuccess)) {
         delete h;
@@ -691,6 +701,24 @@
     StripChoice sc;
     *form = resize_form(h->last, h->hg, level, sc);
     *rows_out = sc.rows_out;
+    return ORBX_OK;
+}
+
+int orbx_debug_resize_grid(const orbx_extractor* h, int level, int* blocks, int* virtual_blocks) {
+    if (!h || !h->have_last || !blocks || !virtual_blocks || level < 1 || level >= h->hg.g.nlevels) return ORBX_ERR_ARG;
+    const PyramidPlan& pp = h->last_plan.pyr;
+    for (int i = 0; i < pp.n; i++)
+        if (pp.launch[i].variant >= PV_TILED0 && pp.launch[i].index == level) {
+            *blocks = pp.launch[i].grid;
+            *virtual_blocks = pp.launch[i].nblocks;
+            return ORBX_OK;
+        }
+    return ORBX_ERR_ARG;
+}
+
+int orbx_debug_set_resize_grid(orbx_extractor* h, int blocks) {
+    if (!h || blocks < 0) return ORBX_ERR_ARG;
+    h->rz_grid_abs = blocks;
     return ORBX_OK;
 }
 
diff --git a/orb_slam_amd/csrc/orbx_device.h b/orb_slam_amd/csrc/orbx_device.h
--- a/orb_slam_amd/csrc/orbx_device.h
+++ b/orb_slam_amd/csrc/orbx_device.h
@@ -57,11 +57,9 @@
     item = (int)(slot - fr * per_frame);
     return frame < b.nframes;
 }
-static inline int frame_item_blocks(const Batch& b, int per_frame) {
-    return (b.xcd_affinity ? (b.nframes + 7) / 8 * 8 : b.nframes) * per_frame;
-}
+static inline int frame_item_blocks(const Batch& b, int per_frame) { return item_blocks(b.xcd_affinity != 0, b.nframes, per_frame); }
 static inline unsigned frame_item_magic_of(int per_frame) {
-    return per_frame > 1 ? (unsigned)((1ull << 32) / (unsigned)per_frame) + 1u : 0u;
+    return item_magic_of(per_frame);
 }
 
 typedef int rec16_t __attribute__((ext_vector_type(16)));
diff --git a/orb_slam_amd/csrc/orbx_internal.h b/orb_slam_amd/csrc/orbx_internal.h
--- a/orb_slam_amd/csrc/orbx_internal.h
+++ b/orb_slam_amd/csrc/orbx_internal.h
@@ -221,6 +221,7 @@
     int xcd_affinity;
     int od_min_frames;
     int blur_on_demand;
+    int rz_grid_cap;
     const ImgSrc* img_tab;
     unsigned long long img_tab_bits;
     long long img_tab_min_stride;
diff --git a/orb_slam_amd/csrc/orbx_launch.h b/orb_slam_amd/csrc/orbx_launch.h
--- a/orb_slam_amd/csrc/orbx_launch.h
+++ b/orb_slam_amd/csrc/orbx_launch.h
@@ -38,7 +38,7 @@
 
 struct StagePlan { int id = -1; unsigned flags = 0; unsigned long long mask = 0; };
 inline StagePlan stage_plan(int id, unsigned flags = 0) { StagePlan s; s.id = id; s.flags = flags; s.mask = 1ull << id; return s; }
-struct PyramidLaunch { int variant, index; StripChoice sc; };
+struct PyramidLaunch { int variant, index; StripChoice sc; int grid, nblocks; };
 struct PyramidPlan { int n = 0; PyramidLaunch launch[MAX_LEVELS]; };
 struct LaunchPlan {
     StagePlan st[VS_COUNT];
```
